# wuji3/visiondk

Measured on AMD Instinct MI355X. Metric: images/sec fwd+bwd+optimizer step (ViT-B/16, bs=256 per GPU), higher is better.
Workload: dtype fp16; 1 GPU; ViT-B/16 ICT, synthetic ImageNet-1k 224x224, random-init weights (reference re-init), per-GPU batch 256, CE label_smoothing 0.05, SGD 0.006/0.937/5e-4, clip 10, EMA on rank 0; global_batch=256, parallelism=dp1

## Files before the change

visiondk_amd/csrc/attention.hip:

```cpp
#include <hip/hip_runtime.h>
#include <stdlib.h>
#include "vdk_device.h"
#include "vdk_host.h"

#define A_HD 64
#define A_RP 72
#define A_FWD_KC 256
#define A_BWD_QC 256

__device__ __forceinline__ void a_stage_rows(bf16_t* dst, const bf16_t* __restrict__ src, long ld, int row0, int nvalid_total,
                                             int ntile) {
  for (int id = threadIdx.x; id < ntile * 8; id += 256) {
    int r = id >> 3, ch = id & 7;
    u32x4 v = {0u, 0u, 0u, 0u};
    if (row0 + r < nvalid_total) v = *(const u32x4*)(src + (long)(row0 + r) * ld + ch * 8);
    *(u32x4*)(dst + r * A_RP + ch * 8) = v;
  }
}
__device__ __forceinline__ void a_load_frags(s16x8 (&f)[4], const bf16_t* __restrict__ src, long ld, int row, int nvalid, int hi) {
#pragma unroll
  for (int ks = 0; ks < 4; ++ks) {
    s16x8 v = {0, 0, 0, 0, 0, 0, 0, 0};
    if (row < nvalid) v = *(const s16x8*)(src + (long)row * ld + ks * 16 + hi * 8);
    f[ks] = v;
// ... 182 lines not shown
    for (int r = 0; r < 16; ++r) { g0[r] = 0.f; g1[r] = 0.f; }
    for (int c = 0; c < nchunk; ++c) {
      const int key0 = c * A_FWD_KC;
      int nk = N - key0; if (nk > A_FWD_KC) nk = A_FWD_KC;
      const int nkp = (nk + 31) / 32 * 32;
      if (nchunk > 1 || rd == 0) {
        __syncthreads();
        a_stage_rows(Ks, kb, ld, key0, N, nkp);
        a_stage_rows(Vs, vb, ld, key0, N, nkp);
        __syncthreads();
      }
      if (active) {
        for (int kt = 0; kt < nkp / 32; ++kt) {
          f32x16 st = a_mma_rows(Ks + (kt * 32 + l31) * A_RP + hi * 8, qf);
          f32x16 dp = a_mma_rows(Vs + (kt * 32 + l31) * A_RP + hi * 8, dof);
          float ds[16];
#pragma unroll
          for (int r = 0; r < 16; ++r) {
            const int key = key0 + kt * 32 + (r & 3) + 8 * (r >> 2) + 4 * hi;
            const float p = (key < N && qrow < N) ? fast_exp2(fmaf(st[r], scale2, -mylse2)) : 0.f;
            ds[r] = p * (dp[r] - dsum);
          }
          s16x8 df[2];
          a_pack_b(ds, df);
#pragma unroll
          for (int s = 0; s < 2; ++s) {
            s16x8 a0 = a_load_T(Ks, kt * 32, 0, s, hi, lane);
            s16x8 a1 = a_load_T(Ks, kt * 32, 32, s, hi, lane);
            g0 = __builtin_amdgcn_mfma_f32_32x32x16_bf16(a0, df[s], g0, 0, 0, 0);
            g1 = __builtin_amdgcn_mfma_f32_32x32x16_bf16(a1, df[s], g1, 0, 0, 0);
          }
        }
      }
    }
    if (active && qrow < N) {
      bf16_t* drow = dq + ((long)b * N + qrow) * lddq + h * A_HD;
#pragma unroll
      for (int g = 0; g < 4; ++g) {
        const int d = 8 * g + 4 * hi;
        *(u32x2*)(drow + d) = (u32x2){pack_bf2(g0[4 * g] * scale, g0[4 * g + 1] * scale), pack_bf2(g0[4 * g + 2] * scale, g0[4 * g + 3] * scale)};
        *(u32x2*)(drow + 32 + d) = (u32x2){pack_bf2(g1[4 * g] * scale, g1[4 * g + 1] * scale), pack_bf2(g1[4 * g + 2] * scale, g1[4 * g + 3] * scale)};
      }
    }
  }
}

__global__ __launch_bounds__(256) void attn_bwd_dkv_kernel(const bf16_t* __restrict__ q, const bf16_t* __restrict__ k,
                                                           const bf16_t* __restrict__ v, long ld, const bf16_t* __restrict__ dout,
                                                           long ldo, const float* __restrict__ lse, const float* __restrict__ dvec,
                                                           bf16_t* __restrict__ dk, bf16_t* __restrict__ dv, long lddkv, int N, int H,
                                                           float scale) {
  __shared__ __attribute__((aligned(16))) bf16_t Qs[A_BWD_QC * A_RP];
  __shared__ __attribute__((aligned(16))) bf16_t Os[A_BWD_QC * A_RP];
  __shared__ __attribute__((aligned(16))) float lse_s[A_BWD_QC];
  __shared__ __attribute__((aligned(16))) float dv_s[A_BWD_QC];
  const int b = blockIdx.x / H, h = blockIdx.x % H;
  const int lane = threadIdx.x & 63, w = threadIdx.x >> 6, hi = lane >> 5, l31 = lane & 31;
  const bf16_t* qb = q + (long)b * N * ld + h * A_HD;
  const bf16_t* kb = k + (long)b * N * ld + h * A_HD;
  const bf16_t* vb = v + (long)b * N * ld + h * A_HD;
  const bf16_t* dob = dout + (long)b * N * ldo + h * A_HD;
  const float* lse_b = lse + ((long)b * H + h) * N;
  const float* dvec_b = dvec + ((long)b * H + h) * N;
  const int nkt = (N + 31) / 32, nchunk = (N + A_BWD_QC - 1) / A_BWD_QC, rounds = (nkt + 3) / 4;
  for (int rd = 0; rd < rounds; ++rd) {
    const int kt = rd * 4 + w;
    const bool active = kt < nkt;
    const int krow = kt * 32 + l31;
    s16x8 kf[4], vf[4];
    a_load_frags(kf, kb, ld, active ? krow : N, N, hi);
    a_load_frags(vf, vb, ld, active ? krow : N, N, hi);
    f32x16 gk0, gk1, gv0, gv1;
#pragma unroll
    for (int r = 0; r < 16; ++r) { gk0[r] = 0.f; gk1[r] = 0.f; gv0[r] = 0.f; gv1[r] = 0.f; }
    for (int c = 0; c < nchunk; ++c) {
      const int q0 = c * A_BWD_QC;
      int nq = N - q0; if (nq > A_BWD_QC) nq = A_BWD_QC;
      const int nqp = (nq + 31) / 32 * 32;
      if (nchunk > 1 || rd == 0) {
        __syncthreads();
        a_stage_rows(Qs, qb, ld, q0, N, nqp);
        a_stage_rows(Os, dob, ldo, q0, N, nqp);
        for (int i = threadIdx.x; i < nqp; i += 256) {
          lse_s[i] = (q0 + i < N) ? lse_b[q0 + i] * VDK_LOG2E : 0.f;
          dv_s[i] = (q0 + i < N) ? dvec_b[q0 + i] : 0.f;
        }
        __syncthreads();
      }
      if (active) {
        for (int qt = 0; qt < nqp / 32; ++qt) {
          f32x16 st = a_mma_rows(Qs + (qt * 32 + l31) * A_RP + hi * 8, kf);
          f32x16 dp = a_mma_rows(Os + (qt * 32 + l31) * A_RP + hi * 8, vf);
          float p[16], ds[16];
#pragma unroll
          for (int g = 0; g < 4; ++g) {
            f32x4 lv = *(const f32x4*)(lse_s + qt * 32 + 8 * g + 4 * hi);
            f32x4 dvv = *(const f32x4*)(dv_s + qt * 32 + 8 * g + 4 * hi);
#pragma unroll
            for (int e = 0; e < 4; ++e) {
              const int r = 4 * g + e;
              const int qq = q0 + qt * 32 + 8 * g + 4 * hi + e;
              const float pv = (qq < N && krow < N) ? fast_exp2(fmaf(st[r], scale * VDK_LOG2E, -lv[e])) : 0.f;
              p[r] = pv;
              ds[r] = pv * (dp[r] - dvv[e]);
            }
          }
          s16x8 pf[2], df[2];
          a_pack_b(p, pf);
          a_pack_b(ds, df);
#pragma unroll
          for (int s = 0; s < 2; ++s) {
            s16x8 ao0 = a_load_T(Os, qt * 32, 0, s, hi, lane);
            s16x8 ao1 = a_load_T(Os, qt * 32, 32, s, hi, lane);
            gv0 = __builtin_amdgcn_mfma_f32_32x32x16_bf16(ao0, pf[s], gv0, 0, 0, 0);
            gv1 = __builtin_amdgcn_mfma_f32_32x32x16_bf16(ao1, pf[s], gv1, 0, 0, 0);
            s16x8 aq0 = a_load_T(Qs, qt * 32, 0, s, hi, lane);
            s16x8 aq1 = a_load_T(Qs, qt * 32, 32, s, hi, lane);
            gk0 = __builtin_amdgcn_mfma_f32_32x32x16_bf16(aq0, df[s], gk0, 0, 0, 0);
            gk1 = __builtin_amdgcn_mfma_f32_32x32x16_bf16(aq1, df[s], gk1, 0, 0, 0);
          }
        }
      }
    }
    if (active && krow < N) {
      bf16_t* krow_p = dk + ((long)b * N + krow) * lddkv + h * A_HD;
      bf16_t* vrow_p = dv + ((long)b * N + krow) * lddkv + h * A_HD;
#pragma unroll
      for (int g = 0; g < 4; ++g) {
        const int d = 8 * g + 4 * hi;
        *(u32x2*)(krow_p + d) = (u32x2){pack_bf2(gk0[4 * g] * scale, gk0[4 * g + 1] * scale), pack_bf2(gk0[4 * g + 2] * scale, gk0[4 * g + 3] * scale)};
        *(u32x2*)(krow_p + 32 + d) = (u32x2){pack_bf2(gk1[4 * g] * scale, gk1[4 * g + 1] * scale), pack_bf2(gk1[4 * g + 2] * scale, gk1[4 * g + 3] * scale)};
        *(u32x2*)(vrow_p + d) = (u32x2){pack_bf2(gv0[4 * g], gv0[4 * g + 1]), pack_bf2(gv0[4 * g + 2], gv0[4 * g + 3])};
        *(u32x2*)(vrow_p + 32 + d) = (u32x2){pack_bf2(gv1[4 * g], gv1[4 * g + 1]), pack_bf2(gv1[4 * g + 2], gv1[4 * g + 3])};
      }
    }
  }
}

int vdk_attention_small_fwd(const void* qkv, int64_t ld, void* o, int64_t ldo, float* lse, int32_t B, int32_t N, int32_t H, float scale, int opf, void* stream);
int vdk_attention_small_bwd(const void* qkv, int64_t ld, const void* o, const void* dout, int64_t ldo, const float* lse, void* dqkv, int64_t ldd, float* dvec, int32_t B, int32_t N,
                            int32_t H, float scale, int opf, void* stream);
int vdk_attention_long_fwd(const void* qkv, int64_t ld, void* o, int64_t ldo, float* lse, int32_t B, int32_t N, int32_t H, float scale, int opf, void* stream);
int vdk_attention_long_bwd(const void* qkv, int64_t ld, const void* o, const void* dout, int64_t ldo, const float* lse, void* dqkv, int64_t ldd, float* dvec, int32_t B, int32_t N,
                           int32_t H, float scale, int opf, void* stream);
static thread_local int g_attn_legacy = -1;
static bool attn_legacy() {
  if (g_attn_legacy >= 0) return g_attn_legacy == 1;
  const char* e = getenv("VDK_ATTN_LEGACY");
  return e && e[0] == '1';
}

void vdk_attention_small_want_colsum(float*);
int vdk_attention_small_colsum_produced();
static int attn_long_min() {
  const char* e = getenv("VDK_ATTN_LONG_MIN");
  return e ? atoi(e) : 1 << 30;
}
static bool attn_long_bwd_off() {
  static const bool off = getenv("VDK_ATTN_LONG_BWD") && getenv("VDK_ATTN_LONG_BWD")[0] == '0';
  return off;
}

extern "C" {

int vdk_attention_fwd_dt(const void*, int64_t, void*, int64_t, float*, int32_t, int32_t, int32_t, int32_t, float, int32_t, void*);
int vdk_attention_bwd_dt(const void*, int64_t, const void*, const void*, int64_t, const float*, void*, int64_t, float*, int32_t, int32_t, int32_t, int32_t, float, int32_t, void*);
int vdk_attention_force_legacy(int32_t on) { g_attn_legacy = on < 0 ? -1 : (on ? 1 : 0); return VDK_OK; }

int vdk_attention_fwd(const void* qkv, int64_t ld, void* o, int64_t ldo, float* lse, int32_t B, int32_t N, int32_t H,
                      int32_t head_dim, float scale, void* stream) {
  return vdk_attention_fwd_dt(qkv, ld, o, ldo, lse, B, N, H, head_dim, scale, VDK_BF16, stream);
}
int vdk_attention_fwd_dt(const void* qkv, int64_t ld, void* o, int64_t ldo, float* lse, int32_t B, int32_t N, int32_t H,
                         int32_t head_dim, float scale, int32_t dtype, void* stream) {
  if (!qkv || !o || B <= 0 || N <= 0 || H <= 0 || (dtype != VDK_BF16 && dtype != VDK_F16)) return vdk_fail(VDK_EINVAL, "vdk_attention_fwd: bad argument");
  const int opf = dtype == VDK_F16 ? VDK_OPF_F16 : VDK_OPF_BF16;
  if (head_dim != A_HD) return vdk_fail(VDK_EUNSUPPORTED, "vdk_attention_fwd: head_dim must be 64");
  if ((ld & 7) || (ldo & 7)) return vdk_fail(VDK_EINVAL, "vdk_attention_fwd: ld % 8");
  if (N <= 256 && N < attn_long_min() && !attn_legacy()) {
    const int rc = vdk_attention_small_fwd(qkv, ld, o, ldo, lse, B, N, H, scale, opf, stream);
    if (rc != VDK_EUNSUPPORTED) return rc ? rc : vdk_check_launch("vdk_attention_fwd");
  }
  if ((N > 256 || N >= attn_long_min()) && !attn_legacy()) {
    const int rc = vdk_attention_long_fwd(qkv, ld, o, ldo, lse, B, N, H, scale, opf, stream);
    return rc ? rc : vdk_check_launch("vdk_attention_fwd");
  }
  if (opf) return vdk_fail(VDK_EUNSUPPORTED, "vdk_attention_fwd: the flash-style kernels of round 1 (vdk_attention_force_legacy) are bf16 only");
  const bf16_t* base = (const bf16_t*)qkv;
  const long D = (long)H * A_HD;
  int grid = B * H;
  int cap = 512;
  if (const char* e = getenv("VDK_ATTN_GRID")) { const int v = atoi(e); if (v > 0) cap = v; }
  if (N <= A_FWD_KC && grid > cap) grid = cap;
  hipLaunchKernelGGL(attn_fwd_kernel, dim3((unsigned)grid), dim3(256), 0, (hipStream_t)stream, base, base + D, base + 2 * D,
                     (long)ld, (bf16_t*)o, (long)ldo, lse, (int)N, (int)H, scale, (int)(B * H));
  return vdk_check_launch("vdk_attention_fwd");
}

int vdk_attention_bwd_cs(const void* qkv, int64_t ld, const void* o, const void* dout, int64_t ldo, const float* lse, void* dqkv, int64_t lddqkv, float* dvec, int32_t B, int32_t N,
                         int32_t H, int32_t head_dim, float scale, int32_t dtype, float* cspart, int32_t* produced, void* stream_) {
  vdk_attention_small_want_colsum(cspart);
  const int rc = vdk_attention_bwd_dt(qkv, ld, o, dout, ldo, lse, dqkv, lddqkv, dvec, B, N, H, head_dim, scale, dtype, stream_);
  if (produced) *produced = rc == VDK_OK ? vdk_attention_small_colsum_produced() : 0;
  vdk_attention_small_want_colsum(nullptr);
  return rc;
}
int vdk_attention_bwd(const void* qkv, int64_t ld, const void* o, const void* dout, int64_t ldo, const float* lse, void* dqkv,
                      int64_t lddqkv, float* dvec, int32_t B, int32_t N, int32_t H, int32_t head_dim, float scale, void* stream_) {
  return vdk_attention_bwd_dt(qkv, ld, o, dout, ldo, lse, dqkv, lddqkv, dvec, B, N, H, head_dim, scale, VDK_BF16, stream_);
}
int vdk_attention_bwd_dt(const void* qkv, int64_t ld, const void* o, const void* dout, int64_t ldo, const float* lse, void* dqkv,
                         int64_t lddqkv, float* dvec, int32_t B, int32_t N, int32_t H, int32_t head_dim, float scale, int32_t dtype, void* stream_) {
  hipStream_t stream = (hipStream_t)stream_;
  if (!qkv || !o || !dout || !lse || !dqkv || !dvec || B <= 0 || N <= 0 || H <= 0 || (dtype != VDK_BF16 && dtype != VDK_F16)) return vdk_fail(VDK_EINVAL, "vdk_attention_bwd: bad argument");
  const int opf = dtype == VDK_F16 ? VDK_OPF_F16 : VDK_OPF_BF16;
  if (head_dim != A_HD) return vdk_fail(VDK_EUNSUPPORTED, "vdk_attention_bwd: head_dim must be 64");
  if ((ld & 7) || (ldo & 7) || (lddqkv & 7)) return vdk_fail(VDK_EINVAL, "vdk_attention_bwd: ld % 8");
  if (N <= 224 && N < attn_long_min() && !attn_legacy()) {
    const int rc = vdk_attention_small_bwd(qkv, ld, o, dout, ldo, lse, dqkv, lddqkv, dvec, B, N, H, scale, opf, stream_);
    if (rc != VDK_EUNSUPPORTED) return rc ? rc : vdk_check_launch("vdk_attention_bwd");
  }
  if ((N > 224 || N >= attn_long_min()) && !attn_legacy() && !attn_long_bwd_off()) {
    const int rc = vdk_attention_long_bwd(qkv, ld, o, dout, ldo, lse, dqkv, lddqkv, dvec, B, N, H, scale, opf, stream_);
    return rc ? rc : vdk_check_launch("vdk_attention_bwd");
  }
  if (opf) return vdk_fail(VDK_EUNSUPPORTED, "vdk_attention_bwd: the flash-style kernels of round 1 are bf16 only");
  const bf16_t* base = (const bf16_t*)qkv;
  bf16_t* dbase = (bf16_t*)dqkv;
  const long D = (long)H * A_HD;
  hipLaunchKernelGGL(attn_bwd_dq_kernel, dim3((unsigned)(B * H)), dim3(256), 0, stream, base, base + D, base + 2 * D, (long)ld,
                     (const bf16_t*)o, (const bf16_t*)dout, (long)ldo, lse, dbase, (long)lddqkv, dvec, (int)N, (int)H, scale);
  hipLaunchKernelGGL(attn_bwd_dkv_kernel, dim3((unsigned)(B * H)), dim3(256), 0, stream, base, base + D, base + 2 * D, (long)ld,
                     (const bf16_t*)dout, (long)ldo, lse, (const float*)dvec, dbase + D, dbase + 2 * D, (long)lddqkv, (int)N, (int)H,
                     scale);
  return vdk_check_launch("vdk_attention_bwd");
}

}
```

visiondk_amd/csrc/attention_small.hip:

```cpp
#include <hip/hip_runtime.h>
#include <stdlib.h>
#include "vdk_device.h"
#include "vdk_host.h"

#include "vdk_attn_tile.h"


template <int NKT, int OF = 0>
__global__ __launch_bounds__(256, (NKT <= 7 ? 2 : 1)) void attn_s_fwd_kernel(const bf16_t* __restrict__ q, const bf16_t* __restrict__ k, const bf16_t* __restrict__ v, long ld,
                                                                              bf16_t* __restrict__ o, long ldo, float* __restrict__ lse, int N, int H, float scale, int nitems) {
  VDK_DYN_LDS(smem);
  const int tid = threadIdx.x, lane = tid & 63, hi = lane >> 5, l31 = lane & 31;
  const int w = __builtin_amdgcn_readfirstlane(tid >> 6);
  const int R8 = (N + 7) & ~7;
  unsigned char* const Qs = smem;
  unsigned char* const Ks = smem + R8 * AS_ROW;
  unsigned char* const Vs = smem + 2 * R8 * AS_ROW;
  for (int i = tid * 16; i < (32 * NKT - R8) * AS_ROW; i += 256 * 16) *(u32x4*)(Vs + R8 * AS_ROW + i) = (u32x4){0u, 0u, 0u, 0u};
  const int nqt = (N + 31) >> 5;
  const float scale2 = scale * VDK_LOG2E;
  const AsLane al = as_lane(lane);
  for (int item = blockIdx.x; item < nitems; item += gridDim.x) {
    const int b = item / H, h = item - b * H;
    const long off = (long)b * N * ld + h * 64;
    __syncthreads();
    as_dma_rows(Qs, q + off, ld, N, R8, w, 4, lane);
    as_dma_rows(Ks, k + off, ld, N, R8, w, 4, lane);
    as_dma_rows(Vs, v + off, ld, N, R8, w, 4, lane);
    __builtin_amdgcn_s_waitcnt(0x0F70);
    __syncthreads();
    for (int qt = w; qt < nqt; qt += 4) {
      const int qrow = qt * 32 + l31;
      s16x8 qf[4];
#pragma unroll
      for (int ks = 0; ks < 4; ++ks) qf[ks] = as_row_frag(Qs, qrow, ks, hi);
      f32x16 st[NKT];
#pragma unroll
      for (int kt = 0; kt < NKT; ++kt) {
        st[kt] = as_zero16();
#pragma unroll
        for (int ks = 0; ks < 4; ++ks) st[kt] = vdk_mfma32<OF>(as_row_frag_l(Ks + kt * 32 * AS_ROW, al, ks), qf[ks], st[kt]);
      }
      if (N & 31) {
#pragma unroll
        for (int r = 0; r < 16; ++r)
          if ((NKT - 1) * 32 + (r & 3) + 8 * (r >> 2) + 4 * hi >= N) st[NKT - 1][r] = -INFINITY;
      }
      float m = -INFINITY;
#pragma unroll
      for (int kt = 0; kt < NKT; ++kt)
#pragma unroll
        for (int r = 0; r < 16; ++r) m = fmaxf(m, st[kt][r]);
      m = fmaxf(m, __shfl_xor(m, 32));
      const float m2 = m * scale2;
      float l = 0.f;
#pragma unroll
      for (int kt = 0; kt < NKT; ++kt)
#pragma unroll
        for (int r = 0; r < 16; ++r) { const float p = fast_exp2(fmaf(st[kt][r], scale2, -m2)); st[kt][r] = p; l += p; }
      l += __shfl_xor(l, 32);
      const float inv = 1.0f / l;
      f32x16 o0 = as_zero16(), o1 = as_zero16();
#pragma unroll
      for (int kt = 0; kt < NKT; ++kt) {
        f32x16 pn;
#pragma unroll
        for (int r = 0; r < 16; ++r) pn[r] = st[kt][r] * inv;
        s16x8 pf[2];
        as_pack_b<OF>(pn, pf);
#pragma unroll
        for (int s = 0; s < 2; ++s) {
          o0 = vdk_mfma32<OF>(as_tr_frag_l(Vs + (kt * 32 + 16 * s) * AS_ROW, al, 0), pf[s], o0);
          o1 = vdk_mfma32<OF>(as_tr_frag_l(Vs + (kt * 32 + 16 * s) * AS_ROW, al, 1), pf[s], o1);
        }
      }
      as_store_tile<OF>(Qs + qt * 32 * AS_ROW, o0, o1, 1.0f, o + (long)b * N * ldo + h * 64, ldo, qt * 32, N, lane);
      if (lse && hi == 0 && qrow < N) lse[((long)b * H + h) * N + qrow] = (m2 + log2f(l)) * 0.6931471805599453f;
    }
  }
}

#define A5_PITCH 72
#ifndef A5_KVREG
#define A5_KVREG 1
#endif
#ifndef A5_SWAP
#define A5_SWAP 1
#endif
#ifndef A5_KP
#define A5_KP 1
#endif
#define A5_QPITCH 144
template <int NKT, int OF>
__global__ __launch_bounds__(512) void attn_s_bwd5_kernel(const bf16_t* __restrict__ q, const bf16_t* __restrict__ k, const bf16_t* __restrict__ v, long ld,
                                                          const bf16_t* __restrict__ o, const bf16_t* __restrict__ dout, long ldo, const float* __restrict__ lse,
                                                          bf16_t* __restrict__ dq, bf16_t* __restrict__ dk, bf16_t* __restrict__ dv, long ldd, int N, int H, float scale,
                                                          int nitems, int dbg ,
                                                          float* __restrict__ cspart ) {
  VDK_DYN_LDS(smem);
  const int tid = threadIdx.x, lane = tid & 63, hi = lane >> 5, l31 = lane & 31;
  const int w = __builtin_amdgcn_readfirstlane(tid >> 6);
  constexpr int NP = 32 * NKT;
  constexpr int NPC = (NP * 8 + 511) / 512;
  constexpr int DSB = NP * A5_PITCH;
  unsigned char* const QO = smem;
  unsigned char* const Kall = smem + 3 * 8192;
  unsigned char* const Kt = Kall + w * 4096;
  unsigned char* const Vt = Kall + NKT * 4096 + w * 4096;
  unsigned char* const Ds = Kall + 2 * NKT * 4096;
  unsigned char* const DQs = Ds + 2 * DSB;
  float* const lse2 = (float*)(DQs + NP * A5_QPITCH);
  float* const Dv = lse2 + NP;
  float* const CSs = Dv + NP;
  constexpr int nt = NKT;
  const float scale2 = scale * VDK_LOG2E;
  const bool ragged = (N & 31) != 0;
  const AsLane al = as_lane(lane);
  const bool keyw = w < nt;
  const int db = w >> 1, qb = w & 1;
  const int a16 = lane & 15, g4 = lane >> 4;
  const int trow = 8 * g4 + (a16 >> 2);
  const int ds_off = trow * A5_PITCH + qb * 32 + 8 * (a16 & 3);
  int kt_off[2];
#pragma unroll
  for (int h2 = 0; h2 < 2; ++h2) {
    const int r = trow + 4 * h2, byte = 32 * db + 8 * (a16 & 3);
    kt_off[h2] = r * AS_ROW + (((byte >> 4) ^ as_f(r)) << 4) + (byte & 8);
  }
  auto request_tile = [&](int j, int buf, long off, long offo, int lane_) {
    const int q0 = j * 32, part = w & 3;
    if (w < 4) as_dma_rows_raw(QO + buf * 8192, q + off + (long)q0 * ld, ld, N - q0, 32, part, 4, lane_);
    else as_dma_rows_raw(QO + buf * 8192 + 4096, dout + offo + (long)q0 * ldo, ldo, N - q0, 32, part, 4, lane_);
  };
  auto request_item = [&](long off, long offo, int lane_) {
    request_tile(0, 0, off, offo, lane_);
    if (nt > 1) request_tile(1, 1, off, offo, lane_);
    if (keyw) {
      as_dma_rows_raw(Kt, k + off + (long)(w * 32) * ld, ld, N - w * 32, 32, 0, 1, lane_);
      as_dma_rows_raw(Vt, v + off + (long)(w * 32) * ld, ld, N - w * 32, 32, 0, 1, lane_);
    }
  };
  u32x4 d_a[NPC], d_c[NPC];
  float lse_r = 0.f;
  auto d_issue = [&](long offo, long lrow, int tid_) {
#pragma unroll
    for (int p = 0; p < NPC; ++p) {
      const int id = tid_ + 512 * p, row = id >> 3, cp = id & 7;
      d_a[p] = (u32x4){0u, 0u, 0u, 0u}; d_c[p] = (u32x4){0u, 0u, 0u, 0u};
      if (row < N && !(dbg & 4)) { d_a[p] = *(const u32x4*)(dout + offo + (long)row * ldo + cp * 8); d_c[p] = *(const u32x4*)(o + offo + (long)row * ldo + cp * 8); }
    }
    lse_r = tid_ < N ? lse[lrow + tid_] : 0.f;
  };
  auto d_finish = [&]() {
#pragma unroll
    for (int p = 0; p < NPC; ++p) {
      const int id = tid + 512 * p, row = id >> 3, cp = id & 7;
      float d = 0.f;
#pragma unroll
      for (int e = 0; e < 4; ++e) { d = fmaf(op_lo<OF>(d_a[p][e]), op_lo<OF>(d_c[p][e]), d); d = fmaf(op_hi<OF>(d_a[p][e]), op_hi<OF>(d_c[p][e]), d); }
      d += __shfl_xor(d, 1); d += __shfl_xor(d, 2); d += __shfl_xor(d, 4);
      if (row < NP && cp == 0) Dv[row] = row < N ? d : 0.f;
    }
    if (tid < NP) lse2[tid] = lse_r * VDK_LOG2E;
  };
  int pb = -1, ph = 0;
  auto cs_flush = [&]() {
    if (tid < 192) {
      const int which = tid >> 6, col = tid & 63, nw = which == 0 ? 8 : nt;
      float t = 0.f;
      for (int ww = 0; ww < nw; ++ww) t += CSs[(which * 8 + ww) * 64 + col];
      cspart[(((long)pb * 3 + which) * H + ph) * 64 + col] = t;
    }
  };
  unsigned char* const St = Ds + w * 4096;
  if ((int)blockIdx.x < nitems) {
    const int b0 = blockIdx.x / H, h0 = blockIdx.x - b0 * H;
    request_item((long)b0 * N * ld + h0 * 64, (long)b0 * N * ldo + h0 * 64, lane);
    d_issue((long)b0 * N * ldo + h0 * 64, ((long)b0 * H + h0) * N, tid);
  }
  for (int item = blockIdx.x; item < nitems; item += gridDim.x) {
    const int b = item / H, h = item - b * H;
    const long off = (long)b * N * ld + h * 64, offo = (long)b * N * ldo + h * 64;
    d_finish();
    f32x16 gk0 = as_zero16(), gk1 = as_zero16(), gv0 = as_zero16(), gv1 = as_zero16();
    __builtin_amdgcn_s_waitcnt(0x0F70);
    __syncthreads();
    if (cspart && pb >= 0) cs_flush();
    s16x8 kfr[4], vfr[4];
#if A5_KVREG
    if (keyw) {
#pragma unroll
      for (int ks = 0; ks < 4; ++ks) { kfr[ks] = as_row_frag_l(Kt, al, ks); vfr[ks] = as_row_frag_l(Vt, al, ks); }
    }
#endif
    auto key_phase = [&](int j) {
      const int q0 = j * 32, buf = j % 3, dbuf = j & 1;
      const unsigned char* Qs = QO + buf * 8192;
      const unsigned char* Os = Qs + 4096;
      unsigned char* const Dsj = Ds + dbuf * DSB;
      if (j + 2 < nt) request_tile(j + 2, (j + 2) % 3, off, offo, lane);
      if (keyw && !(dbg & 1)) {
        f32x16 st = as_zero16(), dp = as_zero16();
        f32x16 pv, ds;
        s16x8 pf[2], df[2];
        const bool edge = ragged && j == nt - 1;
#if A5_KP == 0
#pragma unroll
        for (int ks = 0; ks < 4; ++ks) {
          st = vdk_mfma32<OF>(as_row_frag_l(Qs, al, ks), as_row_frag_l(Kt, al, ks), st);
          dp = vdk_mfma32<OF>(as_row_frag_l(Os, al, ks), as_row_frag_l(Vt, al, ks), dp);
        }
#pragma unroll
        for (int g = 0; g < 4; ++g) {
          const f32x4 lv = *(const f32x4*)(lse2 + q0 + 8 * g + 4 * hi);
          const f32x4 dd = *(const f32x4*)(Dv + q0 + 8 * g + 4 * hi);
#pragma unroll
          for (int e = 0; e < 4; ++e) {
            const int r = 4 * g + e;
            float p = fast_exp2(fmaf(st[r], scale2, -lv[e]));
            if (edge && q0 + 8 * g + 4 * hi + e >= N) p = 0.f;
            pv[r] = p;
            ds[r] = p * (dp[r] - dd[e]);
          }
        }
        as_pack_b<OF>(pv, pf);
        as_pack_b<OF>(ds, df);
#pragma unroll
        for (int s2 = 0; s2 < 2; ++s2) {
          gv0 = vdk_mfma32<OF>(as_tr_frag_l(Os + 16 * s2 * AS_ROW, al, 0), pf[s2], gv0);
          gv1 = vdk_mfma32<OF>(as_tr_frag_l(Os + 16 * s2 * AS_ROW, al, 1), pf[s2], gv1);
          gk0 = vdk_mfma32<OF>(as_tr_frag_l(Qs + 16 * s2 * AS_ROW, al, 0), df[s2], gk0);
          gk1 = vdk_mfma32<OF>(as_tr_frag_l(Qs + 16 * s2 * AS_ROW, al, 1), df[s2], gk1);
        }
#else
#define A5_SB() __builtin_amdgcn_sched_barrier(0)
#ifdef VDK_EMU
#define A5_PIN(x) ((void)0)
#else
#define A5_PIN(x) asm volatile("" : "+v"(x))
#endif
        s16x8 qf[4], of_[4], kf[4], vf[4];
#pragma unroll
        for (int ks = 0; ks < 4; ++ks) { qf[ks] = as_row_frag_l(Qs, al, ks); kf[ks] = A5_KVREG ? kfr[ks] : as_row_frag_l(Kt, al, ks); }
#pragma unroll
        for (int ks = 0; ks < 4; ++ks) st = vdk_mfma32<OF>(qf[ks], kf[ks], st);
#pragma unroll
        for (int ks = 0; ks < 4; ++ks) { of_[ks] = as_row_frag_l(Os, al, ks); vf[ks] = A5_KVREG ? vfr[ks] : as_row_frag_l(Vt, al, ks); }
        A5_SB();
#pragma unroll
        for (int g = 0; g < 4; ++g) {
          dp = vdk_mfma32<OF>(of_[g], vf[g], dp);
          const f32x4 lv = *(const f32x4*)(lse2 + q0 + 8 * g + 4 * hi);
#pragma unroll
          for (int e = 0; e < 4; ++e) pv[4 * g + e] = fast_exp2(fmaf(st[4 * g + e], scale2, -lv[e]));
          A5_SB();
        }
        if (edge) {
#pragma unroll
          for (int r = 0; r < 16; ++r)
            if (q0 + 8 * (r >> 2) + 4 * hi + (r & 3) >= N) pv[r] = 0.f;
        }
        as_pack_b<OF>(pv, pf);
        A5_SB();
#pragma unroll
        for (int s2 = 0; s2 < 2; ++s2)
#pragma unroll
          for (int dh = 0; dh < 2; ++dh) {
            const s16x8 tf = as_tr_frag_l(Os + 16 * s2 * AS_ROW, al, dh);
            if (dh == 0) gv0 = vdk_mfma32<OF>(tf, pf[s2], gv0); else gv1 = vdk_mfma32<OF>(tf, pf[s2], gv1);
            const int g = 2 * s2 + dh;
            const f32x4 dd = *(const f32x4*)(Dv + q0 + 8 * g + 4 * hi);
#pragma unroll
            for (int e = 0; e < 4; ++e) { ds[4 * g + e] = pv[4 * g + e] * (dp[4 * g + e] - dd[e]); A5_PIN(ds[4 * g + e]); }
            A5_SB();
          }
        as_pack_b<OF>(ds, df);
#pragma unroll
        for (int s2 = 0; s2 < 2; ++s2) {
          gk0 = vdk_mfma32<OF>(as_tr_frag_l(Qs + 16 * s2 * AS_ROW, al, 0), df[s2], gk0);
          gk1 = vdk_mfma32<OF>(as_tr_frag_l(Qs + 16 * s2 * AS_ROW, al, 1), df[s2], gk1);
        }
#undef A5_SB
#undef A5_PIN
#endif
        const bool kval = w * 32 + l31 < N;
        unsigned char* const drow = Dsj + (w * 32 + l31) * A5_PITCH + 8 * hi;
#pragma unroll
        for (int s2 = 0; s2 < 2; ++s2) {
          u32x4 u = *(const u32x4*)&df[s2];
          if (!kval) u = (u32x4){0u, 0u, 0u, 0u};
          *(u32x2*)(drow + 32 * s2) = (u32x2){u[0], u[1]};
          *(u32x2*)(drow + 32 * s2 + 16) = (u32x2){u[2], u[3]};
        }
      }
    };
    auto dq_phase = [&](int j) {
      const int q0 = j * 32, dbuf = j & 1;
      unsigned char* const Dsj = Ds + dbuf * DSB;
      f32x4 acc = {0.f, 0.f, 0.f, 0.f};
      if (!(dbg & 2))
#pragma unroll
      for (int t = 0; t < NKT; ++t) {
        const unsigned char* bp = Dsj + t * 32 * A5_PITCH + ds_off;
        const s16x4 lo = __builtin_amdgcn_ds_read_tr16_b64_v4i16(VDK_LDS_S16X4(bp));
        const s16x4 up = __builtin_amdgcn_ds_read_tr16_b64_v4i16(VDK_LDS_S16X4(bp + 4 * A5_PITCH));
        const s16x8 bfrag = {lo[0], lo[1], lo[2], lo[3], up[0], up[1], up[2], up[3]};
        const s16x4 klo = __builtin_amdgcn_ds_read_tr16_b64_v4i16(VDK_LDS_S16X4(Kall + t * 4096 + kt_off[0]));
        const s16x4 kup = __builtin_amdgcn_ds_read_tr16_b64_v4i16(VDK_LDS_S16X4(Kall + t * 4096 + kt_off[1]));
        acc = vdk_mfma16<OF>((s16x8){klo[0], klo[1], klo[2], klo[3], kup[0], kup[1], kup[2], kup[3]}, bfrag, acc);
      }
      *(u32x2*)(DQs + (q0 + 16 * qb + a16) * A5_QPITCH + 32 * db + 8 * g4) = (u32x2){pack_op2<OF>(acc[0] * scale, acc[1] * scale), pack_op2<OF>(acc[2] * scale, acc[3] * scale)};
    };
    key_phase(0);
#pragma unroll 1
    for (int j = 0; j < nt; ++j) {
      if (j + 2 < nt) __builtin_amdgcn_s_waitcnt(0x0F71); else __builtin_amdgcn_s_waitcnt(0x0F70);
      __syncthreads();
      const bool keyfirst = A5_SWAP && w < 4;
      if (keyfirst && j + 1 < nt) key_phase(j + 1);
      dq_phase(j);
      if (!keyfirst && j + 1 < nt) key_phase(j + 1);
    }
    __syncthreads();
    int ln = lane, td = tid;
#ifndef VDK_EMU
    asm volatile("" : "+v"(ln), "+v"(td));
#endif
    const int lane = ln, tid = td, l31 = ln & 31, hi = ln >> 5;
    if (item + (int)gridDim.x < nitems) {
      const int nb = (item + (int)gridDim.x) / H, nh = (item + (int)gridDim.x) - nb * H;
      request_item((long)nb * N * ld + nh * 64, (long)nb * N * ldo + nh * 64, lane);
      d_issue((long)nb * N * ldo + nh * 64, ((long)nb * H + nh) * N, tid);
    }
    if (dbg & 8) continue;
    if (!cspart) {
      if (keyw) {
        as_store_tile<OF>(St, gk0, gk1, scale, dk + (long)b * N * ldd + h * 64, ldd, w * 32, N, lane);
        as_store_tile<OF>(St, gv0, gv1, 1.0f, dv + (long)b * N * ldd + h * 64, ldd, w * 32, N, lane);
      }
#pragma unroll
      for (int p = 0; p < NPC; ++p) {
        const int id = tid + 512 * p, row = id >> 3, cp = id & 7;
        if (row < N) *(u32x4*)(dq + (long)b * N * ldd + h * 64 + (long)row * ldd + cp * 8) = *(const u32x4*)(DQs + row * A5_QPITCH + cp * 16);
      }
      continue;
    }
    auto cs_add = [&](float (&cs)[8], const u32x4& v) {
#pragma unroll
      for (int e = 0; e < 4; ++e) { cs[2 * e] += op_lo<OF>(v[e]); cs[2 * e + 1] += op_hi<OF>(v[e]); }
    };
    auto cs_put = [&](float (&cs)[8], int which) {
#pragma unroll
      for (int e = 0; e < 8; ++e) { float t = cs[e]; t += __shfl_xor(t, 8); t += __shfl_xor(t, 16); t += __shfl_xor(t, 32); cs[e] = t; }
      if (lane < 8) {
        float* dst = CSs + (which * 8 + w) * 64 + lane * 8;
        *(f32x4*)dst = (f32x4){cs[0], cs[1], cs[2], cs[3]}; *(f32x4*)(dst + 4) = (f32x4){cs[4], cs[5], cs[6], cs[7]};
      }
    };
    if (keyw) {
#pragma unroll
      for (int which = 1; which <= 2; ++which) {
        float cs[8] = {0.f, 0.f, 0.f, 0.f, 0.f, 0.f, 0.f, 0.f};
        bf16_t* const dst = (which == 1 ? dk : dv) + (long)b * N * ldd + h * 64;
        const f32x16& x0 = which == 1 ? gk0 : gv0; const f32x16& x1 = which == 1 ? gk1 : gv1;
        const float mul = which == 1 ? scale : 1.0f;
        const int row0 = w * 32;
        if (row0 + l31 < N) {
#pragma unroll
          for (int g = 0; g < 4; ++g) {
            const int ch = g ^ (l31 & 7), ch1 = (4 + g) ^ (l31 & 7);
            *(u32x2*)(St + l31 * AS_ROW + (ch << 4) + 8 * hi) = (u32x2){pack_op2<OF>(x0[4 * g] * mul, x0[4 * g + 1] * mul), pack_op2<OF>(x0[4 * g + 2] * mul, x0[4 * g + 3] * mul)};
            *(u32x2*)(St + l31 * AS_ROW + (ch1 << 4) + 8 * hi) = (u32x2){pack_op2<OF>(x1[4 * g] * mul, x1[4 * g + 1] * mul), pack_op2<OF>(x1[4 * g + 2] * mul, x1[4 * g + 3] * mul)};
          }
        }
        VDK_WAVE_LDS_SYNC();
#pragma unroll
        for (int p = 0; p < 4; ++p) {
          const int r = 8 * p + (lane >> 3), cp = lane & 7;
          if (row0 + r < N) {
            const u32x4 v = *(const u32x4*)(St + r * AS_ROW + ((cp ^ (r & 7)) << 4));
            *(u32x4*)(dst + (long)(row0 + r) * ldd + cp * 8) = v;
            cs_add(cs, v);
          }
        }
        VDK_WAVE_LDS_SYNC();
        cs_put(cs, which);
      }
    }
    {
      float cs[8] = {0.f, 0.f, 0.f, 0.f, 0.f, 0.f, 0.f, 0.f};
#pragma unroll
      for (int p = 0; p < NPC; ++p) {
        const int id = tid + 512 * p, row = id >> 3, cp = id & 7;
        if (row < N) {
          const u32x4 v = *(const u32x4*)(DQs + row * A5_QPITCH + cp * 16);
          *(u32x4*)(dq + (long)b * N * ldd + h * 64 + (long)row * ldd + cp * 8) = v;
          cs_add(cs, v);
        }
      }
      cs_put(cs, 0);
    }
    pb = b; ph = h;
  }
  if (cspart && pb >= 0) { __syncthreads(); cs_flush(); }
}

template <int NKT, int OF>
static int launch_fwd(const bf16_t* base, long D, long ld, bf16_t* o, long ldo, float* lse, int B, int N, int H, float scale, int grid, hipStream_t s) {
  const int R8 = (N + 7) & ~7;
  const size_t lds = (size_t)(2 * R8 + 32 * NKT) * AS_ROW;
  if (hipFuncSetAttribute((const void*)attn_s_fwd_kernel<NKT, OF>, hipFuncAttributeMaxDynamicSharedMemorySize, (int)lds) != hipSuccess)
    return vdk_fail(VDK_ELAUNCH, "vdk_attention_fwd: LDS attribute");
  hipLaunchKernelGGL((attn_s_fwd_kernel<NKT, OF>), dim3((unsigned)grid), dim3(256), lds, s, base, base + D, base + 2 * D, ld, o, ldo, lse, N, H, scale, B * H);
  return VDK_OK;
}
static thread_local float* t_cspart = nullptr;
static thread_local int t_cs_produced = 0;
void vdk_attention_small_want_colsum(float* cspart) { t_cspart = cspart; t_cs_produced = 0; }
int vdk_attention_small_colsum_produced() { return t_cs_produced; }
template <int NKT, int OF>
static int launch_bwd5(const bf16_t* base, long D, long ld, const bf16_t* o, const bf16_t* dout, long ldo, const float* lse, bf16_t* dbase, long ldd, int B, int N, int H,
                       float scale, int grid, hipStream_t s) {
  const size_t lds = 3 * 8192 + 2 * (size_t)NKT * 4096 + 2 * (size_t)(32 * NKT) * A5_PITCH + (size_t)(32 * NKT) * A5_QPITCH + (size_t)NKT * 32 * 8 + 3 * 8 * 64 * 4;
  float* const cspart = t_cspart;
  if (cspart) t_cs_produced = 1;
  const char* edbg = getenv("VDK_ATTN5_DBG");
  const int dbg = edbg ? atoi(edbg) : 0;
  if (hipFuncSetAttribute((const void*)attn_s_bwd5_kernel<NKT, OF>, hipFuncAttributeMaxDynamicSharedMemorySize, (int)lds) != hipSuccess)
    return vdk_fail(VDK_ELAUNCH, "vdk_attention_bwd: LDS attribute");
  hipLaunchKernelGGL((attn_s_bwd5_kernel<NKT, OF>), dim3((unsigned)grid), dim3(512), lds, s, base, base + D, base + 2 * D, ld, o, dout, ldo, lse, dbase, dbase + D, dbase + 2 * D,
                     ldd, N, H, scale, B * H, dbg, cspart);
  return VDK_OK;
}
static int grid_cap(int dflt) {
  if (const char* e = getenv("VDK_ATTN_GRID")) { const int v = atoi(e); if (v > 0) return v; }
  return dflt;
}

int vdk_attention_small_fwd(const void* qkv, int64_t ld, void* o, int64_t ldo, float* lse, int32_t B, int32_t N, int32_t H, float scale, int opf, void* stream) {
  const int nkt = (N + 31) / 32;
  if (nkt < 1 || nkt > 8) return VDK_EUNSUPPORTED;
  const bf16_t* base = (const bf16_t*)qkv;
  const long D = (long)H * 64;
  int grid = B * H;
  const int cap = grid_cap(512);
  if (grid > cap) grid = cap;
  hipStream_t s = (hipStream_t)stream;
  switch (nkt) {
#define FW(n) case n: return opf ? launch_fwd<n, VDK_OPF_F16>(base, D, ld, (bf16_t*)o, ldo, lse, B, N, H, scale, grid, s) : launch_fwd<n, 0>(base, D, ld, (bf16_t*)o, ldo, lse, B, N, H, scale, grid, s);
    FW(1) FW(2) FW(3) FW(4) FW(5) FW(6) FW(7)
    default: return opf ? launch_fwd<8, VDK_OPF_F16>(base, D, ld, (bf16_t*)o, ldo, lse, B, N, H, scale, grid, s) : launch_fwd<8, 0>(base, D, ld, (bf16_t*)o, ldo, lse, B, N, H, scale, grid, s);
#undef FW
  }
}

int vdk_attention_small_bwd(const void* qkv, int64_t ld, const void* o, const void* dout, int64_t ldo, const float* lse, void* dqkv, int64_t ldd, float* dvec, int32_t B, int32_t N,
                            int32_t H, float scale, int opf, void* stream) {
  const int nkt = (N + 31) / 32;
  if (nkt < 1 || nkt > 7) return VDK_EUNSUPPORTED;
  const bf16_t* base = (const bf16_t*)qkv;
  const long D = (long)H * 64;
  int grid = B * H;
  const int cap = grid_cap(256);
  if (grid > cap) grid = cap;
  hipStream_t s = (hipStream_t)stream;
  switch (nkt) {
#define B5(n) case n: return opf ? launch_bwd5<n, VDK_OPF_F16>(base, D, ld, (const bf16_t*)o, (const bf16_t*)dout, ldo, lse, (bf16_t*)dqkv, ldd, B, N, H, scale, grid, s) \
                                 : launch_bwd5<n, 0>(base, D, ld, (const bf16_t*)o, (const bf16_t*)dout, ldo, lse, (bf16_t*)dqkv, ldd, B, N, H, scale, grid, s);
    B5(1) B5(2) B5(3) B5(4) B5(5) B5(6)
    default: return opf ? launch_bwd5<7, VDK_OPF_F16>(base, D, ld, (const bf16_t*)o, (const bf16_t*)dout, ldo, lse, (bf16_t*)dqkv, ldd, B, N, H, scale, grid, s)
                        : launch_bwd5<7, 0>(base, D, ld, (const bf16_t*)o, (const bf16_t*)dout, ldo, lse, (bf16_t*)dqkv, ldd, B, N, H, scale, grid, s);
#undef B5
  }
}
```

visiondk_amd/csrc/gemm.hip:

```cpp
#include <hip/hip_runtime.h>
#ifndef VDK_EMU_NO_HIP_EXT
#include <hip/hip_ext.h>
#endif
#include <cstdlib>
#include "vdk_device.h"
#include "vdk_host.h"
#include "vdk_gemm.h"
#include "vdk_gemm_epilogue.h"

#define G_BM 128
#define G_BN 128
#define G_BK 64
#define G_PITCH 72
#define G_CP 132

__device__ __forceinline__ void g_load_tile(u32x4 (&r)[4], const bf16_t* __restrict__ base, long ld, int row0,
                                            int nrows, int k0, int kend) {
#pragma unroll
  for (int j = 0; j < 4; ++j) {
    int id = threadIdx.x + 256 * j;
    int row = id >> 3, ch = id & 7;
    int grow = row0 + row, k = k0 + ch * 8;
    u32x4 v = {0u, 0u, 0u, 0u};
    if (grow < nrows && k < kend) v = *(const u32x4*)(base + (long)grow * ld + k);
// ... 426 lines not shown
      if (cs_ >= te) break;
      if (ce_ == cs_) continue;
      if (ncontrib == 2 && pp == sk_pos) continue;
      const float* src = p.slabs + ((long)pp * 2 + (cs_ >= tb ? 0 : 1)) * WGF + w * 8192 + lane * 2;
#pragma unroll
      for (int i = 0; i < 4; ++i)
#pragma unroll
        for (int j = 0; j < 2; ++j)
#pragma unroll
          for (int g = 0; g < 8; ++g) {
            const unsigned long long v = VDK_AGENT_LD_U64(src + ((i * 2 + j) * 8 + g) * 128);
            acc[i][j][2 * g] += __uint_as_float((unsigned)v); acc[i][j][2 * g + 1] += __uint_as_float((unsigned)(v >> 32));
          }
    }
  } else if (SK) {
    if (tid == 0) {
      if (sk_st[2] < nwg / (int)gridDim.x) sk_st[2] += 1;
      else sk_st[0] += nk;
    }
  }

  float* slab = (float*)(smem + w * 16384);
  const int ncol = n0 + wc * 64 + (lane & 7) * 8;
  float bias8[8], ocs8[8];
#pragma unroll
  for (int e = 0; e < 8; ++e) { bias8[e] = 0.f; ocs8[e] = 0.f; }
  if ((E != E_GENERIC) && (E & E_BIAS) && ncol < p.N) {
    f32x4 b0v = *(const f32x4*)(p.bias + ncol), b1v = *(const f32x4*)(p.bias + ncol + 4);
#pragma unroll
    for (int e = 0; e < 4; ++e) { bias8[e] = b0v[e]; bias8[4 + e] = b1v[e]; }
  }
  float q8_unused = 0.f;
#pragma unroll
  for (int half = 0; half < 2; ++half) {
#pragma unroll
    for (int rt = 0; rt < 2; ++rt)
#pragma unroll
      for (int ct = 0; ct < 2; ++ct)
#pragma unroll
        for (int r = 0; r < 16; ++r)
          slab[(rt * 32 + (r & 3) + 8 * (r >> 2) + 4 * hi) * 64 + ct * 32 + l31] = acc[half * 2 + rt][ct][r];
    __builtin_amdgcn_wave_barrier();
    if (E != E_GENERIC) {
      h_epilogue_half<E>(p, slab, lane, (long)m0 + wr * 128 + half * 64, ncol, z, bias8, ocs8, q8_unused);
    } else {
#pragma unroll
      for (int pass = 0; pass < 8; ++pass) {
        const int row = pass * 8 + (lane >> 3), cc = (lane & 7) * 8;
        const long mi = (long)m0 + wr * 128 + half * 64 + row;
        const int n = n0 + wc * 64 + cc;
        if (mi < p.M && n < p.N) {
          float v[8];
          f32x4 x0 = *(const f32x4*)(slab + row * 64 + cc), x1 = *(const f32x4*)(slab + row * 64 + cc + 4);
#pragma unroll
          for (int e = 0; e < 4; ++e) { v[e] = x0[e]; v[4 + e] = x1[e]; }
          g_epilogue_store8(p, mi, n, v, z);
        }
      }
    }
    __builtin_amdgcn_wave_barrier();
  }
  if ((E != E_GENERIC) && (E & E_OCS)) {
#pragma unroll
    for (int e = 0; e < 8; ++e) {
      float v = ocs8[e];
      v += __shfl_xor(v, 8); v += __shfl_xor(v, 16); v += __shfl_xor(v, 32);
      ocs8[e] = v;
    }
    if (lane < 8 && ncol < p.N) {
      float* dst = p.ocs_part + ((long)tm * 2 + wr) * p.N + ncol;
      *(f32x4*)dst = (f32x4){ocs8[0], ocs8[1], ocs8[2], ocs8[3]};
      *(f32x4*)(dst + 4) = (f32x4){ocs8[4], ocs8[5], ocs8[6], ocs8[7]};
    }
  }
  if (!SK && p.dbg && tid == 0) {
    __builtin_amdgcn_s_waitcnt(0x0F70);
    unsigned long long* o = p.dbg + ((size_t)blockIdx.y * gridDim.x + blockIdx.x) * 4;
    o[0] = t_start; o[1] = t_landed; o[2] = t_main; o[3] = __builtin_readcyclecounter();
  }
  } while (SK);
#undef H_REG
#undef H_ISSUE_A
#undef H_ISSUE_B
#undef H_FRAG_A
#undef H_FRAG_B
}

template <int OF = 0>
__global__ __launch_bounds__(256) void splitk_reduce_kernel(const float* __restrict__ slabs, int S, long n4 ,
                                                            long mn, float alpha, float* __restrict__ outf,
                                                            bf16_t* __restrict__ outb) {
  long i = (long)blockIdx.x * 256 + threadIdx.x;
  if (i >= n4) return;
  f32x4 s = *(const f32x4*)(slabs + i * 4);
  for (int k = 1; k < S; ++k) {
    f32x4 t = *(const f32x4*)(slabs + (long)k * mn + i * 4);
    s += t;
  }
  s *= alpha;
  if (outf) *(f32x4*)(outf + i * 4) = s;
  if (outb) *(u32x2*)(outb + i * 4) = (u32x2){pack_op2<OF>(s[0], s[1]), pack_op2<OF>(s[2], s[3])};
}

template <int OF = 0>
__global__ __launch_bounds__(256) void transpose_bf16_kernel(const bf16_t* __restrict__ in, long ldi, int R, int Cc,
                                                             bf16_t* __restrict__ out, long ldo, int Rpad, int row_group,
                                                             float* __restrict__ colsum_partial) {
  __shared__ bf16_t tile[64][66];
  const int r0 = blockIdx.x * 64, c0 = blockIdx.y * 64;
  const int tid = threadIdx.x;
  for (int i = 0; i < 8; ++i) {
    int row = i * 8 + (tid >> 5), cw = (tid & 31) * 2;
    int gr = r0 + row, gc = c0 + cw;
    bf16_t v0 = 0, v1 = 0;
    if (gr < R) {
      const long sr = row_group > 0 ? (long)gr + gr / row_group + 1 : (long)gr;
      if (gc + 1 < Cc) { unsigned wv = *(const unsigned*)(in + sr * ldi + gc); v0 = (bf16_t)(wv & 0xffff); v1 = (bf16_t)(wv >> 16); }
      else if (gc < Cc) v0 = in[sr * ldi + gc];
    }
    tile[row][cw] = v0; tile[row][cw + 1] = v1;
  }
  __syncthreads();
  if (colsum_partial && tid < 64 && c0 + tid < Cc) {
    float sacc = 0.f;
    for (int r = 0; r < 64; ++r) sacc += op2f<OF>(tile[r][tid]);
    colsum_partial[(long)blockIdx.x * Cc + c0 + tid] = sacc;
  }
  for (int i = 0; i < 8; ++i) {
    int col = i * 8 + (tid >> 5), rw = (tid & 31) * 2;
    int gc = c0 + col, gr = r0 + rw;
    if (gc < Cc && gr < Rpad) {
      unsigned wv = (unsigned)tile[rw][col] | ((unsigned)tile[rw + 1][col] << 16);
      *(unsigned*)(out + (long)gc * ldo + gr) = wv;
    }
  }
}

#include <vector>
static thread_local std::vector<hipEvent_t> g_prof_ev;
static thread_local std::vector<double> g_prof_flops;
static thread_local double g_prof_bytes = 0.0;
static thread_local size_t g_prof_used = 0;
static thread_local bool g_prof_on = false;
static thread_local void* g_dbg_ptr = nullptr;
static thread_local int g_force_kernel = 0;
static thread_local int g_sk_grid = 0;
static thread_local int g_last_kernel = 0;
static bool w4_enabled_env() {
  static const bool on = !(getenv("VDK_GEMM_W4") && atoi(getenv("VDK_GEMM_W4")) == 0);
  return on;
}
static thread_local int t_tn_half = 0;
void vdk_gemm_tn_prefer_half(int on) { t_tn_half = on; }
static bool w4h_wanted(int E, bool trans, long M, long N, long K) {
  static const int mask = getenv("VDK_GEMM_W4H") ? atoi(getenv("VDK_GEMM_W4H")) : -1;
  if (g_force_kernel == 6) return true;
  if (g_force_kernel == 2 || g_force_kernel == 3 || g_force_kernel == 5 || !w4_enabled_env()) return false;
  if (mask >= 0) {
    if (trans) return (mask & 16) != 0;
    if (E == E_GENERIC) return false;
    if (E & E_GELU) return (mask & 1) != 0;
    if (E & E_DGELU) return (mask & 2) != 0;
    if (E & E_RES) return (mask & 4) != 0;
    return (mask & 8) != 0;
  }
  if (trans) return t_tn_half != 0;
  if (E == E_GENERIC) return false;
  const long tiles = ((M + 255) / 256) * ((N + 255) / 256);
  if (tiles < 128) return true;
  if ((E & E_DGELU) && (E & E_AUXD) && tiles > 256) return false;
  if (E & E_DGELU) return true;
  static const long gelu_k = getenv("VDK_GEMM_W4H_GELU_K") ? atol(getenv("VDK_GEMM_W4H_GELU_K")) : 768;
  if ((E & E_GELU) && gelu_k > 0 && K <= gelu_k) return true;
  if (E & E_GELU) return K <= 768 && (double)tiles / (double)((tiles + 255) / 256 * 256) < 0.8;
  if (E & E_RES) return K < 1536 && tiles <= 256;
  return K <= 1024 && tiles <= 3 * 256;
}
static long narrow_min_m() {
  static const long v = getenv("VDK_GEMM_NARROW_MIN_M") ? atol(getenv("VDK_GEMM_NARROW_MIN_M")) : 65536L;
  return v;
}
static bool w4_enabled() {
  return (w4_enabled_env() || g_force_kernel == 5) && g_force_kernel != 2 && g_force_kernel != 3 && g_force_kernel != 6;
}
#define SK_CNT_BYTES 65536
static int sk_grid() {
  if (g_sk_grid > 0) return g_sk_grid;
  static int cus = 0;
  if (cus == 0) {
    int dev = 0, n = 0;
    if (hipGetDevice(&dev) != hipSuccess || hipDeviceGetAttribute(&n, hipDeviceAttributeMultiprocessorCount, dev) != hipSuccess || n < 8) n = 256;
    cus = n & ~7;
  }
  return cus;
}

#define RC_MARGIN(x) do { int rc_ = (x); if (rc_) return rc_; } while (0)
extern "C" {

int vdk_gemm_a_colsum_rows(int32_t M, int32_t N, int32_t K) {
  const long tiles256 = (long)((M + 255) / 256) * ((N + 255) / 256);
  const bool big = g_force_kernel == 2 || g_force_kernel == 3 || g_force_kernel == 5 || g_force_kernel == 6 || ((g_force_kernel == 0 || g_force_kernel == 4) && (K % 64 == 0) && tiles256 >= 128 && M >= 256 && N >= 256);
  return (big && (K % 64 == 0) && (M % 256 == 0)) ? (M / 256) : 0;
}

int vdk_gemm_c_colsum_rows(int32_t M, int32_t N, int32_t K) {
  const long tiles256 = (long)((M + 255) / 256) * ((N + 255) / 256);
  const long tiles_h = w4_enabled_env() ? (long)((M + 255) / 256) * ((N + 127) / 128) : 0;
  const bool big = g_force_kernel == 2 || g_force_kernel == 3 || g_force_kernel == 5 || g_force_kernel == 6 || ((g_force_kernel == 0 || g_force_kernel == 4) && (K % 64 == 0) && (tiles256 >= 128 || tiles_h >= 128) && M >= 256 && N >= 256);
  return (big && (K % 64 == 0)) ? 2 * ((M + 255) / 256) : 0;
}

int vdk_gemm_force_kernel(int32_t which) { g_force_kernel = which; return VDK_OK; }
int vdk_gemm_last_kernel(void) { return g_last_kernel; }

int vdk_gemm_streamk_workspace_bytes(size_t* bytes) {
  if (!bytes) return vdk_fail(VDK_EINVAL, "vdk_gemm_streamk_workspace_bytes: null");
  *bytes = (size_t)SK_CNT_BYTES + (size_t)sk_grid() * 2 * 65536 * 4;
  return VDK_OK;
}
int vdk_gemm_streamk_grid(int32_t g) {
  if (g < 0 || (g & 7)) return vdk_fail(VDK_EINVAL, "vdk_gemm_streamk_grid: must be a multiple of 8");
  g_sk_grid = g;
  return VDK_OK;
}
int vdk_gemm_debug_stamps(void* device_u64_buffer) { g_dbg_ptr = device_u64_buffer; return VDK_OK; }

int vdk_prof_begin(int32_t max_launches) {
  if (max_launches < 0) return vdk_fail(VDK_EINVAL, "vdk_prof_begin: bad argument");
  while (g_prof_ev.size() < (size_t)max_launches * 2) {
    hipEvent_t e;
    if (hipEventCreate(&e) != hipSuccess) return vdk_fail(VDK_ELAUNCH, "vdk_prof_begin: hipEventCreate failed");
    g_prof_ev.push_back(e);
  }
  g_prof_flops.clear();
  g_prof_bytes = 0.0;
  g_prof_used = 0;
  g_prof_on = true;
  return VDK_OK;
}
int vdk_prof_pause(int32_t paused) { g_prof_on = !paused && !g_prof_ev.empty(); return VDK_OK; }
int vdk_prof_end(double* total_ms, int64_t* launches, double* total_flops) {
  g_prof_on = false;
  double ms = 0.0, fl = 0.0;
  for (size_t i = 0; i + 1 < g_prof_used; i += 2) {
    if (hipEventSynchronize(g_prof_ev[i + 1]) != hipSuccess) return vdk_fail(VDK_ELAUNCH, "vdk_prof_end: event sync failed");
    float t = 0.f;
    if (hipEventElapsedTime(&t, g_prof_ev[i], g_prof_ev[i + 1]) != hipSuccess) return vdk_fail(VDK_ELAUNCH, "vdk_prof_end: elapsed failed");
    ms += t; fl += g_prof_flops[i / 2];
  }
  if (total_ms) *total_ms = ms;
  if (launches) *launches = (int64_t)(g_prof_used / 2);
  if (total_flops) *total_flops = fl;
  return VDK_OK;
}

int vdk_prof_bytes(double* total_bytes) {
  if (!total_bytes) return vdk_fail(VDK_EINVAL, "vdk_prof_bytes: null");
  *total_bytes = g_prof_bytes;
  return VDK_OK;
}

int vdk_gemm_splitk_workspace_bytes(int32_t M, int32_t N, int32_t splitk, size_t* bytes) {
  if (!bytes || M <= 0 || N <= 0 || splitk < 1) return vdk_fail(VDK_EINVAL, "vdk_gemm_splitk_workspace_bytes: bad argument");
  *bytes = splitk > 1 ? (size_t)splitk * M * N * 4 : 0;
  return VDK_OK;
}

int vdk_gemm_bf16_nt(const GemmDesc* d, void* ws, size_t ws_bytes, void* stream_) {
  hipStream_t stream = (hipStream_t)stream_;
  if (!d || !d->A || !d->B || !d->C) return vdk_fail(VDK_EINVAL, "vdk_gemm_bf16_nt: null pointer");
  if (d->M <= 0 || d->N <= 0 || d->K <= 0) return vdk_fail(VDK_EINVAL, "vdk_gemm_bf16_nt: empty problem");
  if ((d->K & 7) || (d->N & 7) || (!d->conv && (d->lda & 7)) || (d->ldb & 7) || (d->ldc & 7))
    return vdk_fail(VDK_EINVAL, "vdk_gemm_bf16_nt: K, N, lda, ldb, ldc must be multiples of 8");
  if (d->ab_dtype == VDK_F16 && !d->conv && d->splitk <= 1 && d->splitk != -1 && d->row_group == 0 && !d->a_colsum && !d->c_colsum && d->a_row_group == 0) {
    double lim = 2147483648.0 - 65536.0;
    if (const char* e = getenv("VDK_GEMM_ROWBLOCK_LIMIT")) { const double v = atof(e); if (v > 0) lim = v; }
    double rowb = (double)d->ldc * (d->c_dtype == VDK_F32 ? 4.0 : 2.0);
    if (d->aux && (double)d->ldaux * 2.0 > rowb) rowb = (double)d->ldaux * 2.0;
    if (d->residual && (double)d->ldr * 4.0 > rowb) rowb = (double)d->ldr * 4.0;
    if (!d->trans && (double)d->lda * 2.0 > rowb) rowb = (double)d->lda * 2.0;
    if (((double)d->M + 256.0) * rowb >= lim) {
      long mb = (long)(lim / rowb) - 256;
      mb = mb / 256 * 256;
      if (mb >= 256) {
        for (long m0 = 0; m0 < d->M; m0 += mb) {
          GemmDesc sub = *d;
          sub.M = (int32_t)((d->M - m0) < mb ? (d->M - m0) : mb);
          sub.A = d->trans ? (const void*)((const bf16_t*)d->A + m0) : (const void*)((const bf16_t*)d->A + m0 * d->lda);
          sub.C = d->c_dtype == VDK_F32 ? (void*)((float*)d->C + m0 * d->ldc) : (void*)((bf16_t*)d->C + m0 * d->ldc);
          if (d->residual) sub.residual = d->residual + m0 * d->ldr;
          if (d->aux) sub.aux = (void*)((bf16_t*)d->aux + m0 * d->ldaux);
          if (d->row_scale) { if (m0 % d->rows_per_scale) return vdk_fail(VDK_EUNSUPPORTED, "vdk_gemm_bf16_nt: row blocks do not align with rows_per_scale"); sub.row_scale = d->row_scale + m0 / d->rows_per_scale; }
          const int rc = vdk_gemm_bf16_nt(&sub, ws, ws_bytes, stream_);
          if (rc) return rc;
        }
        return VDK_OK;
      }
    }
  }
  if (d->conv) {
    const VdkConvGeom* c = d->conv;
    if (c->Cin <= 0 || (c->Cin & 7) || c->KH <= 0 || c->KW <= 0 || c->stride <= 0 || c->pad < 0 || c->OH <= 0 || c->OW <= 0 || c->H <= 0 || c->W <= 0)
      return vdk_fail(VDK_EINVAL, "vdk_gemm_bf16_nt: bad convolution geometry (Cin % 8 == 0)");
    if (!d->trans && (d->K != c->KH * c->KW * c->Cin || (d->M % (c->OH * c->OW))))
      return vdk_fail(VDK_EINVAL, "vdk_gemm_bf16_nt: bad convolution geometry (K == KH*KW*Cin, M == B*OH*OW)");
    if (d->trans && (c->transposed || d->N != c->KH * c->KW * c->Cin || c->rows <= 0 || c->rows >= (1 << 24) || (c->rows % (c->OH * c->OW)) || d->K < c->rows || (d->K % 128) ||
                     d->K - c->rows >= 128 || d->a_row_group != 0))
      return vdk_fail(VDK_EINVAL, "vdk_gemm_bf16_nt: bad weight-gradient geometry (N == KH*KW*Cin, rows == B*OH*OW < 2^24, K == rows rounded up to 128)");
  }
  if (d->ab_dtype != VDK_BF16 && d->ab_dtype != VDK_F16) return vdk_fail(VDK_EINVAL, "vdk_gemm_bf16_nt: ab_dtype must be VDK_BF16 or VDK_F16");
  const int opf = d->ab_dtype == VDK_F16 ? VDK_OPF_F16 : VDK_OPF_BF16;
  if (d->c_dtype != VDK_F32 && d->c_dtype != (opf ? VDK_F16 : VDK_BF16)) return vdk_fail(VDK_EINVAL, "vdk_gemm_bf16_nt: bad c_dtype (VDK_F32, or the operand format)");
  if (opf && (d->a_colsum || d->splitk == -1))
    return vdk_fail(VDK_EUNSUPPORTED, "vdk_gemm_bf16_nt: fp16 operands are served by the four-wave and the 128x128 kernels (no a_colsum, no stream-K)");
  if (d->act < VDK_ACT_NONE || d->act > VDK_ACT_MUL_AUX) return vdk_fail(VDK_EINVAL, "vdk_gemm_bf16_nt: bad act");
  if (((d->act == VDK_ACT_DGELU || d->act == VDK_ACT_GELU_SAVE_GRAD || d->act == VDK_ACT_MUL_AUX) && !d->aux) || (d->aux && (d->ldaux & 7)))
    return vdk_fail(VDK_EINVAL, "vdk_gemm_bf16_nt: bad aux");
  int splitk = d->splitk < 1 ? 1 : d->splitk;
  GemmParams p = {};
  p.A = (const bf16_t*)d->A; p.B = (const bf16_t*)d->B; p.C = d->C;
  p.lda = d->lda; p.ldb = d->ldb; p.ldc = d->ldc;
  p.M = d->M; p.N = d->N; p.K = d->K;
  p.opf = opf;
  p.c_dtype = d->c_dtype == VDK_F32 ? VDK_F32 : VDK_BF16; p.bias = (const float*)d->bias; p.residual = (const float*)d->residual; p.ldr = d->ldr;
  p.act = d->act; p.aux = (bf16_t*)d->aux; p.ldaux = d->ldaux; p.alpha = d->alpha; p.row_group = d->row_group < 0 ? -d->row_group : d->row_group; p.row_shift = d->row_group > 0 ? 1 : 0; p.a_row_group = d->a_row_group;
  p.splitk = splitk; p.slabs = nullptr; p.sk_cnt = nullptr; p.dbg = (unsigned long long*)g_dbg_ptr;
  p.colsum_part = nullptr; p.ocs_part = nullptr;
  p.cscale = d->col_scale;
  p.rscale = d->row_scale; p.rps = d->rows_per_scale;
  if (d->row_scale && (d->rows_per_scale <= 0 || d->c_dtype != VDK_F32 || !d->bias || !d->residual || d->act != VDK_ACT_NONE || d->splitk > 1 || d->trans || d->row_group != 0))
    return vdk_fail(VDK_EUNSUPPORTED, "vdk_gemm_bf16_nt: row_scale goes with rows_per_scale > 0, an fp32 output, a bias, a residual, act NONE and neither split-K, TN nor a row remap");
  if (d->col_scale && (d->c_dtype != VDK_F32 || !d->bias || d->act != VDK_ACT_NONE || d->splitk > 1 || d->trans || d->row_group != 0 || (d->N & 7)))
    return vdk_fail(VDK_EUNSUPPORTED, "vdk_gemm_bf16_nt: col_scale goes with an fp32 output, a bias, act NONE, N % 8 == 0 and neither split-K, TN nor a row remap");
  p.conv_on = d->conv != nullptr;
  if (d->conv) {
    const VdkConvGeom* c = d->conv;
    p.cCin = c->Cin; p.cH = c->H; p.cW = c->W; p.cOH = c->OH; p.cOW = c->OW; p.cKH = c->KH; p.cKW = c->KW; p.cstride = c->stride; p.cpad = c->pad; p.ctrans = c->transposed;
    p.crows = c->rows;
  }
  int kps = d->K;
  if (splitk > 1) {
    if (d->bias || d->residual || d->act != VDK_ACT_NONE || d->row_group != 0) return vdk_fail(VDK_EINVAL, "vdk_gemm_bf16_nt: split-K excludes fused epilogues");
    if (d->ldc != d->N) return vdk_fail(VDK_EINVAL, "vdk_gemm_bf16_nt: split-K needs ldc == N");
    const int kq = (d->K % 128 == 0) ? 128 : G_BK;
    kps = ((d->K + splitk - 1) / splitk + kq - 1) / kq * kq;
    splitk = (d->K + kps - 1) / kps;
    p.splitk = splitk;
    if (splitk > 1) {
      size_t need = (size_t)splitk * d->M * d->N * 4;
      if (!ws || ws_bytes < need) return vdk_fail(VDK_EWORKSPACE, "vdk_gemm_bf16_nt: split-K workspace too small");
      p.slabs = (float*)ws;
    }
  }
  p.k_per_split = kps;
  const int ntn = (d->N + G_BN - 1) / G_BN, ntm = (d->M + G_BM - 1) / G_BM;
  const bool prof = g_prof_on && g_prof_used + 2 <= g_prof_ev.size();
  const long tiles256 = (long)((d->M + 255) / 256) * ((d->N + 255) / 256) * splitk;
  const long tiles_h = (!d->trans && splitk == 1 && !d->a_colsum && w4_enabled_env()) ? (long)((d->M + 255) / 256) * ((d->N + 127) / 128) : 0;
  const bool narrow = !d->conv && !d->trans && g_force_kernel == 0 && w4_enabled_env() && (d->K % 64 == 0) && (kps % 64 == 0) && d->N >= 128 && d->N < 256 && d->M >= narrow_min_m() &&
                      !d->a_colsum && !d->c_colsum && splitk == 1 && vdk_gemm_w4h_serves(p, false);
  const bool big = !d->conv && (narrow || g_force_kernel == 2 || g_force_kernel == 3 || g_force_kernel == 5 || g_force_kernel == 6 || ((g_force_kernel == 0 || g_force_kernel == 4) && (d->K % 64 == 0) && (kps % 64 == 0) && (tiles256 >= 128 || tiles_h >= 128) && d->M >= 256 && d->N >= 256));
  int E = E_GENERIC;
  {
    const bool bias = d->bias != nullptr, res = d->residual != nullptr, f32 = p.c_dtype == VDK_F32, rg = d->row_group != 0;
    const bool plain_alpha = d->alpha == 1.0f;
    if (splitk > 1) E = E_SPLITK;
    else if (plain_alpha && !rg && !res && d->act == VDK_ACT_NONE && !f32) E = bias ? E_BIAS : 0;
    else if (plain_alpha && !rg && !res && d->act == VDK_ACT_GELU && !f32 && bias && d->aux) E = E_BIAS | E_GELU;
    else if (plain_alpha && !rg && !res && d->act == VDK_ACT_DGELU && !f32 && !bias) E = E_DGELU;
    else if (plain_alpha && !rg && !res && d->act == VDK_ACT_GELU_SAVE_GRAD && !f32 && bias) E = E_BIAS | E_GELU | E_AUXD;
    else if (plain_alpha && !rg && !res && d->act == VDK_ACT_MUL_AUX && !f32 && !bias) E = E_DGELU | E_AUXD;
    else if (plain_alpha && !rg && res && d->act == VDK_ACT_NONE && f32 && bias) E = E_BIAS | E_RES | E_F32;
    else if (plain_alpha && rg && res && d->act == VDK_ACT_NONE && f32 && bias) E = E_BIAS | E_RES | E_F32 | E_ROWGRP;
    else if (plain_alpha && !rg && !res && d->act == VDK_ACT_NONE && f32 && !bias) E = E_F32;
    else if (plain_alpha && !rg && !res && d->act == VDK_ACT_NONE && f32 && bias) E = E_BIAS | E_F32;
  }
  dim3 grid256((unsigned)(((d->M + 255) / 256) * ((d->N + 255) / 256)), (unsigned)splitk);
  bool sk = false;
  if (d->splitk == -1 && !d->trans && !d->a_colsum && big && ws && g_force_kernel != 4) {
    const long T = (long)grid256.x, G = sk_grid();
    const long rounds = (T + G - 1) / G;
    static const bool optin = getenv("VDK_GEMM_STREAMK") && atoi(getenv("VDK_GEMM_STREAMK")) > 0;
    const bool worth = optin && T >= G && (double)T / (double)(rounds * G) < 0.94;
    if ((worth || g_force_kernel == 3) && T <= SK_CNT_BYTES / 4 && T * (d->K / 64) >= G && ws_bytes >= (size_t)SK_CNT_BYTES + (size_t)G * 2 * 65536 * 4) {
      sk = true;
      p.sk_cnt = (int*)ws; p.slabs = (float*)((char*)ws + SK_CNT_BYTES);
      grid256 = dim3((unsigned)G, 1u);
    }
  }
#define VDK_GEMM_LAUNCH(KERN, GRID, BLOCK)                                                                                                   \
  do {                                                                                                                                       \
    if (prof) hipExtLaunchKernelGGL(KERN, GRID, BLOCK, 0, stream, g_prof_ev[g_prof_used], g_prof_ev[g_prof_used + 1], 0, p);                 \
    else hipLaunchKernelGGL(KERN, GRID, BLOCK, 0, stream, p);                                                                                \
  } while (0)
#define LAUNCH256X(TNF, EE, CSF)                                                                                         \
  do {                                                                                                                   \
    if (opf) {                    \
      void* e0_ = prof ? (void*)g_prof_ev[g_prof_used] : nullptr; void* e1_ = prof ? (void*)g_prof_ev[g_prof_used + 1] : nullptr;                \
      const bool hfirst_ = narrow || w4h_wanted(EE, TNF, p.M, p.N, p.K) || !(w4_enabled() && vdk_gemm_w4_serves(p, TNF));                         \
      if (hfirst_ && vdk_gemm_w4h_serves(p, TNF) && vdk_gemm_w4h_launch_f16(p, TNF, EE, grid256.y, stream, e0_, e1_)) { g_last_kernel = 6; break; }   \
      if (vdk_gemm_w4_serves(p, TNF) && vdk_gemm_w4_launch_f16(p, TNF, EE, grid256.x, grid256.y, stream, e0_, e1_)) { g_last_kernel = 5; break; }     \
      if (vdk_gemm_w4h_serves(p, TNF) && vdk_gemm_w4h_launch_f16(p, TNF, EE, grid256.y, stream, e0_, e1_)) { g_last_kernel = 6; break; }          \
      fp16_unserved = true; break;                                                                                        \
    }                                                                                                                    \
    if (!sk && !(CSF) && (narrow || w4h_wanted(EE, TNF, p.M, p.N, p.K)) && vdk_gemm_w4h_serves(p, TNF) &&                                           \
        vdk_gemm_w4h_launch(p, TNF, EE, grid256.y, stream, prof ? (void*)g_prof_ev[g_prof_used] : nullptr,               \
                            prof ? (void*)g_prof_ev[g_prof_used + 1] : nullptr)) { g_last_kernel = 6; break; }           \
    if (!sk && !(CSF) && w4_enabled() && vdk_gemm_w4_serves(p, TNF) &&                                                   \
        vdk_gemm_w4_launch(p, TNF, EE, grid256.x, grid256.y, stream, prof ? (void*)g_prof_ev[g_prof_used] : nullptr,     \
                           prof ? (void*)g_prof_ev[g_prof_used + 1] : nullptr)) { g_last_kernel = 5; break; }            \
    g_last_kernel = sk ? 3 : 2;                                                                                          \
    if (sk) VDK_GEMM_LAUNCH((gemm256_bf16_kernel<TNF, EE, !TNF, CSF>), grid256, dim3(512));                               \
    else VDK_GEMM_LAUNCH((gemm256_bf16_kernel<TNF, EE, false, CSF>), grid256, dim3(512));                                 \
  } while (0)
#define LAUNCH256(TNF, EE) LAUNCH256X(TNF, EE, false)
#define LAUNCH256CS(EE)                                                                                                  \
  do {                                                                                                                   \
    if (p.colsum_part) VDK_GEMM_LAUNCH((gemm256_bf16_kernel<false, EE, false, true>), grid256, dim3(512));                \
    else LAUNCH256X(false, EE, false);                                                                                   \
  } while (0)
  bool fp16_unserved = false;
  if (d->trans && d->conv) {
    if ((kps % 128) || (d->M & 7) || d->M < 8 || !vdk_gemm_w4_serves(p, true)) return vdk_fail(VDK_EUNSUPPORTED, "vdk_gemm_bf16_nt: this implicit weight gradient is outside the four-wave TN kernel's range");
    void* e0_ = prof ? (void*)g_prof_ev[g_prof_used] : nullptr; void* e1_ = prof ? (void*)g_prof_ev[g_prof_used + 1] : nullptr;
    const int ew_ = E == E_SPLITK ? E_SPLITK : (E == E_F32 ? E_F32 : E_GENERIC);
    if (!(opf ? vdk_gemm_w4_launch_f16(p, true, ew_, grid256.x, grid256.y, stream, e0_, e1_) : vdk_gemm_w4_launch(p, true, ew_, grid256.x, grid256.y, stream, e0_, e1_)))
      return vdk_fail(VDK_EUNSUPPORTED, "vdk_gemm_bf16_nt: implicit weight gradient: no kernel");
    g_last_kernel = 5;
  } else if (d->trans) {
    if ((d->K % 64) || (kps % 64) || (d->M & 7) || d->M < 8 || d->N < 8)
      return vdk_fail(VDK_EUNSUPPORTED, "vdk_gemm_bf16_nt: trans=1 needs K and the split size to be multiples of 64 and M % 8 == 0");
    switch (E) {
      case E_SPLITK: LAUNCH256(true, E_SPLITK); break;
      case E_F32: LAUNCH256(true, E_F32); break;
      case 0: LAUNCH256(true, 0); break;
      default: LAUNCH256(true, E_GENERIC); break;
    }
  } else if (big && (d->K % 64 == 0) && (kps % 64 == 0)) {
    if (d->a_colsum) {
      if (d->M % 256) return vdk_fail(VDK_EUNSUPPORTED, "vdk_gemm_bf16_nt: a_colsum needs M % 256 == 0");
      p.colsum_part = d->a_colsum;
      if (E != 0 && E != E_DGELU && E != E_F32) E = E_GENERIC;
    }
    if (d->c_colsum) {
      if ((E != E_DGELU && E != (E_DGELU | E_AUXD) && E != 0) || d->a_colsum) return vdk_fail(VDK_EUNSUPPORTED, "vdk_gemm_bf16_nt: c_colsum goes with a plain or dGELU bf16 epilogue and without a_colsum");
      p.ocs_part = d->c_colsum;
      E |= E_OCS;
    }
    switch (E) {
      case E_OCS: LAUNCH256(false, E_OCS); break;
      case E_DGELU | E_OCS: LAUNCH256(false, E_DGELU | E_OCS); break;
      case 0: LAUNCH256CS(0); break;
      case E_BIAS: LAUNCH256(false, E_BIAS); break;
      case E_BIAS | E_GELU: LAUNCH256(false, E_BIAS | E_GELU); break;
      case E_DGELU: LAUNCH256CS(E_DGELU); break;
      case E_BIAS | E_GELU | E_AUXD: LAUNCH256(false, E_BIAS | E_GELU | E_AUXD); break;
      case E_DGELU | E_AUXD: LAUNCH256(false, E_DGELU | E_AUXD); break;
      case E_DGELU | E_OCS | E_AUXD: LAUNCH256(false, E_DGELU | E_OCS | E_AUXD); break;
      case E_BIAS | E_RES | E_F32: LAUNCH256(false, E_BIAS | E_RES | E_F32); break;
      case E_BIAS | E_F32: LAUNCH256(false, E_BIAS | E_F32); break;
      case E_BIAS | E_RES | E_F32 | E_ROWGRP: LAUNCH256(false, E_BIAS | E_RES | E_F32 | E_ROWGRP); break;
      case E_SPLITK: LAUNCH256(false, E_SPLITK); break;
      case E_F32: LAUNCH256CS(E_F32); break;
      default: LAUNCH256CS(E_GENERIC); break;
    }
  }
#undef LAUNCH256CS
#undef LAUNCH256X
#undef LAUNCH256
  else if (d->a_colsum || d->c_colsum)
    return vdk_fail(VDK_EUNSUPPORTED, "vdk_gemm_bf16_nt: a_colsum / c_colsum are by-products of the 256x256 NT kernel only (see vdk_gemm_a_colsum_rows)");
  else if (d->conv) {
    g_last_kernel = 1;
    if (opf) VDK_GEMM_LAUNCH((gemm_bf16_nt_kernel<true, VDK_OPF_F16>), dim3((unsigned)(ntn * ntm), (unsigned)splitk), dim3(256));
    else VDK_GEMM_LAUNCH(gemm_bf16_nt_kernel<true>, dim3((unsigned)(ntn * ntm), (unsigned)splitk), dim3(256));
  } else {
    g_last_kernel = 1;
    if (opf) VDK_GEMM_LAUNCH((gemm_bf16_nt_kernel<false, VDK_OPF_F16>), dim3((unsigned)(ntn * ntm), (unsigned)splitk), dim3(256));
    else VDK_GEMM_LAUNCH(gemm_bf16_nt_kernel<false>, dim3((unsigned)(ntn * ntm), (unsigned)splitk), dim3(256));
  }
  if (fp16_unserved) {
    if (d->trans) return vdk_fail(VDK_EUNSUPPORTED, "vdk_gemm_bf16_nt: this fp16 TN problem is outside the four-wave kernels' range");
    g_last_kernel = 1;
    VDK_GEMM_LAUNCH((gemm_bf16_nt_kernel<false, VDK_OPF_F16>), dim3((unsigned)(ntn * ntm), (unsigned)splitk), dim3(256));
  }
  if (prof) {
    g_prof_flops.push_back(2.0 * d->M * d->N * d->K);
    {
      const double mn = (double)d->M * d->N;
      double b = ((double)d->M * d->K + (double)d->N * d->K) * 2.0 + mn * (p.c_dtype == VDK_F32 ? 4.0 : 2.0);
      if (d->residual) b += mn * 4.0;
      if (d->aux) b += mn * 2.0;
      if (d->bias) b += d->N * 4.0;
      if (d->splitk > 1) b += 2.0 * d->splitk * mn * 4.0;
      g_prof_bytes += b;
    }
    g_prof_used += 2;
  }
  if (splitk > 1) {
    long mn = (long)d->M * d->N, n4 = mn / 4;
    if (opf) hipLaunchKernelGGL(splitk_reduce_kernel<VDK_OPF_F16>, dim3((unsigned)((n4 + 255) / 256)), dim3(256), 0, stream, (const float*)p.slabs, splitk, n4, mn, d->alpha,
                                p.c_dtype == VDK_F32 ? (float*)d->C : (float*)nullptr, p.c_dtype == VDK_BF16 ? (bf16_t*)d->C : (bf16_t*)nullptr);
    else
    hipLaunchKernelGGL(splitk_reduce_kernel<0>, dim3((unsigned)((n4 + 255) / 256)), dim3(256), 0, stream,
                       (const float*)p.slabs, splitk, n4, mn, d->alpha,
                       p.c_dtype == VDK_F32 ? (float*)d->C : (float*)nullptr,
                       p.c_dtype == VDK_BF16 ? (bf16_t*)d->C : (bf16_t*)nullptr);
  }
  return vdk_check_launch("vdk_gemm_bf16_nt");
}

int vdk_margin_cos_pass(const VdkMarginHead* h, int32_t pass, const void* fbt, int64_t ld_f, const void* wb, int64_t ld_w, int32_t B, int32_t Bp, int32_t C, int32_t Cp, int32_t K,
                        const int64_t* labels, const float* gt, float* stats, float* tlogit, const float* rowstat, float label_smoothing, float grad_scale, void* dcos,
                        int64_t lddc, void* stream_) {
  hipStream_t stream = (hipStream_t)stream_;
  if (!h || !fbt || !wb || !labels || B <= 0 || Bp < B || C <= 0 || Cp < C || (pass != 1 && pass != 2)) return vdk_fail(VDK_EINVAL, "vdk_margin_cos_pass: bad argument");
  if ((pass == 1 && (!stats || !tlogit)) || (pass == 2 && (!rowstat || !dcos))) return vdk_fail(VDK_EINVAL, "vdk_margin_cos_pass: missing buffer for this pass");
  if ((K % 64) || (Bp & 7) || (Cp & 7) || (ld_f & 7) || (ld_w & 7) || (pass == 2 && (lddc & 7)) || Bp < 8 || Cp < 256)
    return VDK_EUNSUPPORTED;
  GemmParams p = {};
  p.A = (const bf16_t*)fbt; p.B = (const bf16_t*)wb; p.C = dcos; p.lda = ld_f; p.ldb = ld_w; p.ldc = lddc; p.M = Bp; p.N = Cp; p.K = K; p.c_dtype = VDK_BF16;
  p.alpha = 1.0f; p.splitk = 1; p.k_per_split = K;
  RC_MARGIN(fill_params(h, &p.me.P));
  p.me.labels = (const long long*)labels; p.me.gt = gt; p.me.stats = stats; p.me.nslice = (Cp + 63) / 64; p.me.tlogit = tlogit; p.me.rowstat = rowstat;
  p.me.smoothing = label_smoothing; p.me.gscale = grad_scale; p.me.epsc = label_smoothing / (float)C; p.me.B = B; p.me.C = C;
  const dim3 grid((unsigned)(((Bp + 255) / 256) * ((Cp + 255) / 256)), 1u);
  g_last_kernel = 2;
  if (w4_enabled() && vdk_gemm_w4_serves(p, true) && vdk_gemm_w4_launch(p, true, pass == 1 ? E_MSTAT : E_MGRAD, grid.x, 1u, stream, nullptr, nullptr)) g_last_kernel = 5;
  else if (pass == 1) hipLaunchKernelGGL((gemm256_bf16_kernel<true, E_MSTAT, false, false>), grid, dim3(512), 0, stream, p);
  else hipLaunchKernelGGL((gemm256_bf16_kernel<true, E_MGRAD, false, false>), grid, dim3(512), 0, stream, p);
  return vdk_check_launch("vdk_margin_cos_pass");
}

int vdk_transpose_bf16(const void* in, int64_t ldi, int32_t R, int32_t Cc, void* out, int64_t ldo, int32_t Rpad,
                       int32_t in_row_group, float* colsum_partial, void* stream) {
  return vdk_transpose_16(in, ldi, R, Cc, out, ldo, Rpad, in_row_group, colsum_partial, VDK_OPF_BF16, stream);
}

}

int vdk_transpose_16(const void* in, int64_t ldi, int32_t R, int32_t Cc, void* out, int64_t ldo, int32_t Rpad, int32_t in_row_group, float* colsum_partial, int opf,
                     void* stream) {
  if (!in || !out || R < 0 || Cc <= 0 || Rpad < R || (Rpad & 1) || ldo < Rpad || (ldi & 1) || (ldo & 1))
    return vdk_fail(VDK_EINVAL, "vdk_transpose_bf16: bad argument");
  if (Rpad == 0) return VDK_OK;
  const dim3 grid((unsigned)((Rpad + 63) / 64), (unsigned)((Cc + 63) / 64));
  if (opf) hipLaunchKernelGGL(transpose_bf16_kernel<VDK_OPF_F16>, grid, dim3(256), 0, (hipStream_t)stream, (const bf16_t*)in, (long)ldi, (int)R, (int)Cc, (bf16_t*)out,
                              (long)ldo, (int)Rpad, (int)in_row_group, colsum_partial);
  else hipLaunchKernelGGL(transpose_bf16_kernel<0>, grid, dim3(256), 0, (hipStream_t)stream, (const bf16_t*)in, (long)ldi, (int)R, (int)Cc, (bf16_t*)out, (long)ldo,
                          (int)Rpad, (int)in_row_group, colsum_partial);
  return vdk_check_launch("vdk_transpose_bf16");
}
```

visiondk_amd/csrc/gemm_w4.hip:

```cpp
#include <hip/hip_runtime.h>
#ifndef VDK_EMU_NO_HIP_EXT
#include <hip/hip_ext.h>
#endif
#include "vdk_device.h"
#include "vdk_host.h"
#include <atomic>
#include <string.h>
#include <stdlib.h>
#include "vdk_gemm.h"
#include "vdk_gemm_epilogue.h"

#ifndef VDK_W4_OF
#define VDK_W4_OF 0
#endif
#if VDK_W4_OF == 0
#define W4_SYM(name) name
#else
#define W4_SYM(name) name##_f16
#endif

#define W4_REGION 16384
#define W4_TILEBUF 65536
#define W4_STAGE 131072
#define W4_SMEM 163840
// ... 72 lines not shown
  d.ldb = ldb;
  d.conv = 0;
  if (!TN) {
    d.rs = w4_make_rsrc(base, (unsigned)extent * ldb);
    const unsigned i = (unsigned)lane >> 3, cp = (unsigned)lane & 7u;
    d.voff0 = i * ldb + ((cp ^ (i >> 1)) << 4);
    d.voff1 = i * ldb + ((cp ^ (4u + (i >> 1))) << 4);
    d.wave_off = (unsigned)__builtin_amdgcn_readfirstlane((int)(((unsigned)(w >> 1) * blk + (unsigned)(w & 1) * 32u) * ldb));
    d.sub_stride = 64u * ldb;
    d.piece_stride = 8u * ldb;
    d.kbeg = (unsigned)kbeg * 2u;
    d.kstep = 128u;
  } else {
    d.rs = w4_make_rsrc(base, (unsigned)K * ldb);
    const unsigned kr = (unsigned)lane >> 4, cp = (unsigned)lane & 15u, c = cp ^ (4u * (kr & 3u));
    d.voff0 = d.voff1 = kr * ldb + ((c >> 3) * blk + (c & 7u) * 8u) * 2u;
    d.wave_off = (unsigned)__builtin_amdgcn_readfirstlane((int)((unsigned)w * 16u * ldb));
    d.sub_stride = 128u;
    d.piece_stride = 4u * ldb;
    d.kbeg = (unsigned)kbeg * ldb;
    d.kstep = 64u * ldb;
  }
}
template <bool TN>
__device__ __forceinline__ unsigned w4_tile_base(const W4Dma& d, int origin) {
  return (TN ? (unsigned)origin * 2u : (unsigned)origin * d.ldb) + d.wave_off;
}
__device__ __forceinline__ void w4_piece(const W4Dma& d, unsigned char* dst, int sub, int j, unsigned so0) {
  if (d.conv) {
    const unsigned rr = so0 + d.w16 + 4u * (unsigned)j + d.kr;
    unsigned voff = W4_OOB;
    if (rr < (unsigned)d.crows && d.cok[sub]) {
      int b, rem, oy, ox;
      w4_divmod(rr, d.cHW, d.inv_hw, b, rem);
      w4_divmod((unsigned)rem, d.cOW, d.inv_w, oy, ox);
      const int iy = oy * d.cstride + d.cy[sub], ix = ox * d.cstride + d.cx[sub];
      if ((unsigned)iy < (unsigned)d.cH && (unsigned)ix < (unsigned)d.cW) voff = (unsigned)(((b * d.cH + iy) * d.cW + ix) * d.cCin) * 2u + d.cib[sub];
    }
    W4_DMA16(d.rs, voff, dst, 0u);
    return;
  }
  const unsigned so = so0 + (unsigned)sub * d.sub_stride + (unsigned)j * d.piece_stride;
  W4_DMA16(d.rs, (j & 1) ? d.voff1 : d.voff0, dst, so);
}
__device__ __forceinline__ void w4_region(const W4Dma& d, unsigned char* region, int sub, int w, unsigned so0) {
#pragma unroll
  for (int j = 0; j < 4; ++j) w4_piece(d, region + (4 * w + j) * 1024, sub, j, so0);
}

template <bool TN>
struct W4Frag { unsigned a[TN ? 2 : 4], b[TN ? 2 : 4]; };

template <bool TN>
__device__ __forceinline__ void w4_frag_init(W4Frag<TN>& f, int wr, int wc, int lane) {
  const unsigned l31 = lane & 31, hi = lane >> 5;
  if (!TN) {
#pragma unroll
    for (int ks = 0; ks < 4; ++ks) {
      const unsigned ch = ((unsigned)(ks * 2) + hi) ^ ((l31 >> 1) & 7u);
      f.a[ks] = ((unsigned)wr * 64u + l31) * 128u + ch * 16u;
      f.b[ks] = ((unsigned)wc * 64u + l31) * 128u + ch * 16u;
    }
  } else {
    const unsigned s = lane & 15, chalf = (lane >> 4) & 1, t1 = hi * 8u + (s >> 2);
#pragma unroll
    for (int rt = 0; rt < 2; ++rt) {
      const unsigned ca = (unsigned)wr * 64u + (unsigned)rt * 32u + 16u * chalf + 4u * (s & 3u);
      const unsigned cb = (unsigned)wc * 64u + (unsigned)rt * 32u + 16u * chalf + 4u * (s & 3u);
      f.a[rt] = t1 * 256u + (((ca >> 3) ^ (4u * (t1 & 3u))) * 16u) + ((ca >> 2) & 1u) * 8u;
      f.b[rt] = t1 * 256u + (((cb >> 3) ^ (4u * (t1 & 3u))) * 16u) + ((cb >> 2) & 1u) * 8u;
    }
  }
}
template <bool TN>
__device__ __forceinline__ s16x8 w4_frag(const unsigned char* region, const unsigned* off, int rt, int ks) {
  if (!TN) {
    return *(const s16x8*)(region + off[ks] + rt * 4096);
  } else {
    const unsigned char* p1 = region + off[rt] + ks * 4096;
    s16x4 lo = __builtin_amdgcn_ds_read_tr16_b64_v4i16(VDK_LDS_S16X4(p1));
    s16x4 up = __builtin_amdgcn_ds_read_tr16_b64_v4i16(VDK_LDS_S16X4(p1 + 1024));
    s16x8 r = {lo[0], lo[1], lo[2], lo[3], up[0], up[1], up[2], up[3]};
    return r;
  }
}

template <bool TN, bool RD, bool FIRST, int OF>
__device__ __forceinline__ void w4_phase(f32x16 (&c00), f32x16 (&c01), f32x16 (&c10), f32x16 (&c11), const s16x8 (&X)[2][4], const s16x8 (&Y)[2][4],
                                         const unsigned char* rd_region, const unsigned* rd_off, s16x8 (&RDST)[2][4],
                                         const W4Dma& dma, unsigned char* is_region, int is_sub, unsigned so0, int w) {
  const f32x16 zero = {0.f, 0.f, 0.f, 0.f, 0.f, 0.f, 0.f, 0.f, 0.f, 0.f, 0.f, 0.f, 0.f, 0.f, 0.f, 0.f};
#pragma unroll
  for (int ks = 0; ks < 4; ++ks) {
    c00 = vdk_mfma32<OF>(Y[0][ks], X[0][ks], (FIRST && ks == 0) ? zero : c00);
    if (RD) RDST[0][ks] = w4_frag<TN>(rd_region, rd_off, 0, ks);
    c01 = vdk_mfma32<OF>(Y[1][ks], X[0][ks], (FIRST && ks == 0) ? zero : c01);
    if (RD) RDST[1][ks] = w4_frag<TN>(rd_region, rd_off, 1, ks);
    c10 = vdk_mfma32<OF>(Y[0][ks], X[1][ks], (FIRST && ks == 0) ? zero : c10);
    w4_piece(dma, is_region + (4 * w + ks) * 1024, is_sub, ks, so0);
    c11 = vdk_mfma32<OF>(Y[1][ks], X[1][ks], (FIRST && ks == 0) ? zero : c11);
  }
#ifndef VDK_EMU
#pragma unroll
  for (int ks = 0; ks < 4; ++ks) {
    __builtin_amdgcn_sched_group_barrier(0x008, 1, 0);
    if (RD) __builtin_amdgcn_sched_group_barrier(0x100, TN ? 2 : 1, 0);
    __builtin_amdgcn_sched_group_barrier(0x008, 1, 0);
    if (RD) __builtin_amdgcn_sched_group_barrier(0x100, TN ? 2 : 1, 0);
    __builtin_amdgcn_sched_group_barrier(0x008, 1, 0);
    __builtin_amdgcn_sched_group_barrier(0x004, 2, 0);
    __builtin_amdgcn_sched_group_barrier(0x008, 1, 0);
  }
#endif
}

template <int V>
__device__ __forceinline__ void w4_phase_end() {
  __builtin_amdgcn_sched_barrier(0);
  if constexpr (V >= 0) W4_WAIT_VM(V);
  W4_WAIT_LGKM0();
}
template <bool TN, int CUR, int VM, bool FIRST, bool NEXT, int OF>
__device__ __forceinline__ void w4_ktile(unsigned char* smem, const W4Frag<TN>& F, const W4Dma& da, const W4Dma& db, unsigned soa, unsigned sob, int w, f32x16 (&acc)[4][4],
                                         s16x8 (&A0)[2][4], s16x8 (&A1)[2][4], s16x8 (&B0)[2][4], s16x8 (&B1)[2][4], s16x8 (&B0N)[2][4]) {
  unsigned char* const buf = smem + CUR * W4_TILEBUF;
  unsigned char* const nbuf = smem + (CUR ^ 1) * W4_TILEBUF;
  W4_BAR();
  w4_phase<TN, true, FIRST, OF>(acc[0][0], acc[0][1], acc[1][0], acc[1][1], A0, B0, buf + W4_RB1, F.b, B1, da, buf + W4_RA0, 0, soa, w);
  w4_phase_end<VM>();
  W4_BAR();
  w4_phase<TN, true, FIRST, OF>(acc[0][2], acc[0][3], acc[1][2], acc[1][3], A0, B1, buf + W4_RA1, F.a, A1, db, buf + W4_RB0, 0, sob, w);
  w4_phase_end<VM>();
  W4_BAR();
  w4_phase<TN, NEXT, FIRST, OF>(acc[2][2], acc[2][3], acc[3][2], acc[3][3], A1, B1, nbuf + W4_RA0, F.a, A0, db, buf + W4_RB1, 1, sob, w);
  w4_phase_end<VM>();
  W4_BAR();
  w4_phase<TN, NEXT, FIRST, OF>(acc[2][0], acc[2][1], acc[3][0], acc[3][1], A1, B0, nbuf + W4_RB0, F.b, B0N, da, buf + W4_RA1, 1, soa, w);
  w4_phase_end<VM>();
}

#ifdef VDK_EMU
#define W4_EPI_SYNC() VDK_WAVE_LDS_SYNC()
#else
#define W4_EPI_SYNC() do { __builtin_amdgcn_s_waitcnt(0xC07F); VDK_WAVE_LDS_SYNC(); } while (0)
#endif
template <int E, int NCT, int DEEP, int OF>
__device__ __forceinline__ void w4_epilogue(const GemmParams& p, unsigned char* stage, f32x16 (&acc)[4][NCT], int lane, int wr, int wc, int m0, int n0, int z, int tm, unsigned long long (&ts)[5],
                                            const u32x4* auxpre = nullptr ) {
  constexpr int NCH = NCT * 4;
  constexpr int RPP = 64 / NCH;
  constexpr int NPS = 32 / RPP;
  constexpr int ROWB = NCT * 64;
  constexpr int EB = E & ~E_AUXD;
  constexpr bool FAST = (E == 0 || E == E_BIAS || EB == (E_BIAS | E_GELU) || EB == E_DGELU || EB == (E_DGELU | E_OCS) || E == E_OCS);
  const int l31 = lane & 31, hi = lane >> 5;
  const int mrow0 = m0 + wr * 128, ncol0 = n0 + wc * (NCT * 32);
  const int swz_w = NCT == 4 ? (l31 & 15) : ((l31 >> 1) & 7);
  if constexpr (FAST) {
    const int rrow = lane / NCH, rc = lane % NCH;
    const int ncol = ncol0 + rc * 8;
    const bool nok = ncol < p.N;
    float bias[NCT][4][4];
    if (E & E_BIAS) {
#pragma unroll
      for (int ct = 0; ct < NCT; ++ct)
#pragma unroll
        for (int g = 0; g < 4; ++g) {
          const int n = ncol0 + ct * 32 + 8 * g + 4 * hi;
          f32x4 b = {0.f, 0.f, 0.f, 0.f};
          if (n < p.N) b = *(const f32x4*)(p.bias + n);
#pragma unroll
          for (int e = 0; e < 4; ++e) bias[ct][g][e] = b[e];
        }
    }
    float ocs[8];
#pragma unroll
    for (int e = 0; e < 8; ++e) ocs[e] = 0.f;
    unsigned char* const wbase = stage + l31 * ROWB + hi * 8;
    const unsigned lane_out = nok ? (unsigned)rrow * (unsigned)p.ldc * 2u + (unsigned)ncol * 2u : W4_OOB;
    const unsigned lane_aux = nok ? (unsigned)rrow * (unsigned)p.ldaux * 2u + (unsigned)ncol * 2u : W4_OOB;
    const __amdgpu_buffer_rsrc_t rs_out = __builtin_amdgcn_make_buffer_rsrc(p.C, 0, (int)((unsigned)p.M * (unsigned)p.ldc * 2u), 0x00020000);
    const __amdgpu_buffer_rsrc_t rs_aux = __builtin_amdgcn_make_buffer_rsrc((E & (E_GELU | E_DGELU)) ? (void*)p.aux : p.C, 0,
                                                                            (int)((unsigned)p.M * (unsigned)((E & (E_GELU | E_DGELU)) ? p.ldaux : p.ldc) * 2u), 0x00020000);
    auto rows_out = [&](const __amdgpu_buffer_rsrc_t& rs, unsigned lane_off, unsigned ldbytes, int rt, bool with_ocs) {
      W4_EPI_SYNC();
      const unsigned srow = (unsigned)(mrow0 + rt * 32) * ldbytes;
      u32x4 d[NPS];
#pragma unroll
      for (int ps = 0; ps < NPS; ++ps) {
        const int row = ps * RPP + rrow;
        d[ps] = *(const u32x4*)(stage + row * ROWB + ((rc ^ (NCT == 4 ? (row & 15) : ((row >> 1) & 7))) << 4));
      }
      if (with_ocs) {
#pragma unroll
        for (int ps = 0; ps < NPS; ++ps)
#pragma unroll
          for (int e = 0; e < 4; ++e) { ocs[2 * e] += op_lo<OF>(d[ps][e]); ocs[2 * e + 1] += op_hi<OF>(d[ps][e]); }
      }
#pragma unroll
      for (int ps = 0; ps < NPS; ++ps)
        __builtin_amdgcn_raw_buffer_store_b128(d[ps], rs, lane_off + (srow + (unsigned)(ps * RPP) * ldbytes), 0, W4_STORE_POLICY);
      W4_EPI_SYNC();
    };
    if constexpr (DEEP >= 0) W4_WAIT_VM(DEEP);
    if (p.dbg) ts[0] = __builtin_readcyclecounter();
    u32x4 auxrows[NPS];
    auto aux_request = [&](int rt_) {
      const unsigned srow = (unsigned)(mrow0 + rt_ * 32) * (unsigned)p.ldaux * 2u;
#pragma unroll
      for (int ps = 0; ps < NPS; ++ps)
        auxrows[ps] = __builtin_amdgcn_raw_buffer_load_b128(rs_aux, lane_aux, srow + (unsigned)(ps * RPP) * (unsigned)p.ldaux * 2u, 0);
    };
    if (E & E_DGELU) {
      if (auxpre) {
#pragma unroll
        for (int ps = 0; ps < NPS; ++ps) auxrows[ps] = auxpre[ps];
      } else aux_request(0);
    }
#pragma unroll
    for (int rt = 0; rt < 4; ++rt) {
      if (p.dbg && rt > 0) ts[rt] = __builtin_readcyclecounter();
#ifndef VDK_EMU
      __builtin_amdgcn_sched_barrier(0);
#endif
      u32x2 held[NCT][4];
      if (E & E_DGELU) {
        if (!W4_EPI_AHEAD && rt > 0) aux_request(rt);
#pragma unroll
        for (int ps = 0; ps < NPS; ++ps) {
          const int row = ps * RPP + rrow;
          *(u32x4*)(stage + row * ROWB + ((rc ^ (NCT == 4 ? (row & 15) : ((row >> 1) & 7))) << 4)) = auxrows[ps];
        }
        if (W4_EPI_AHEAD && rt < 3) aux_request(rt + 1);
        W4_EPI_SYNC();
      }
#pragma unroll
      for (int ct = 0; ct < NCT; ++ct)
#pragma unroll
        for (int g = 0; g < 4; ++g) {
          unsigned char* const wp = wbase + (((ct * 4 + g) ^ swz_w) << 4);
          float v[4];
          if (E & E_DGELU) {
            const u32x2 u = *(const u32x2*)wp;
            if (E & E_AUXD) {
              v[0] = acc[rt][ct][4 * g + 0] * h_lo(u[0]); v[1] = acc[rt][ct][4 * g + 1] * h_hi(u[0]);
              v[2] = acc[rt][ct][4 * g + 2] * h_lo(u[1]); v[3] = acc[rt][ct][4 * g + 3] * h_hi(u[1]);
            } else {
              const vdk_f32x2 d0 = gelu_grad_f2((vdk_f32x2){op_lo<OF>(u[0]), op_hi<OF>(u[0])}), d1 = gelu_grad_f2((vdk_f32x2){op_lo<OF>(u[1]), op_hi<OF>(u[1])});
              v[0] = acc[rt][ct][4 * g + 0] * d0[0]; v[1] = acc[rt][ct][4 * g + 1] * d0[1];
              v[2] = acc[rt][ct][4 * g + 2] * d1[0]; v[3] = acc[rt][ct][4 * g + 3] * d1[1];
            }
          } else {
#pragma unroll
            for (int e = 0; e < 4; ++e) v[e] = (E & E_BIAS) ? acc[rt][ct][4 * g + e] + bias[ct][g][e] : acc[rt][ct][4 * g + e];
          }
          if ((E & E_GELU) && (E & E_AUXD)) {
            vdk_f32x2 g0, g1, d0, d1;
            gelu_both_f2((vdk_f32x2){v[0], v[1]}, g0, d0); gelu_both_f2((vdk_f32x2){v[2], v[3]}, g1, d1);
            *(u32x2*)wp = (u32x2){pack_h2(d0[0], d0[1]), pack_h2(d1[0], d1[1])};
            held[ct][g] = (u32x2){pack_op2<OF>(g0[0], g0[1]), pack_op2<OF>(g1[0], g1[1])};
          } else
          *(u32x2*)wp = (u32x2){pack_op2<OF>(v[0], v[1]), pack_op2<OF>(v[2], v[3])};
          if ((E & E_GELU) && !(E & E_AUXD)) {
            const vdk_f32x2 g0 = gelu_f2((vdk_f32x2){v[0], v[1]}), g1 = gelu_f2((vdk_f32x2){v[2], v[3]});
            held[ct][g] = (u32x2){pack_op2<OF>(g0[0], g0[1]), pack_op2<OF>(g1[0], g1[1])};
          }
#ifndef VDK_EMU
          if ((E & (E_GELU | E_DGELU)) && g == 3) __builtin_amdgcn_sched_barrier(0);
#endif
        }
      if (E & E_GELU) {
        rows_out(rs_aux, lane_aux, (unsigned)p.ldaux * 2u, rt, false);
#pragma unroll
        for (int ct = 0; ct < NCT; ++ct)
#pragma unroll
          for (int g = 0; g < 4; ++g) *(u32x2*)(wbase + (((ct * 4 + g) ^ swz_w) << 4)) = held[ct][g];
      }
      rows_out(rs_out, lane_out, (unsigned)p.ldc * 2u, rt, (E & E_OCS) != 0);
    }
    if (E & E_OCS) {
#pragma unroll
      for (int e = 0; e < 8; ++e) {
        float s = ocs[e];
        if (NCT == 2) s += __shfl_xor(s, 8);
        s += __shfl_xor(s, 16); s += __shfl_xor(s, 32);
        ocs[e] = s;
      }
      if (lane < NCH && nok) {
        float* dst = p.ocs_part + ((long)tm * 2 + wr) * p.N + ncol;
        *(f32x4*)dst = (f32x4){ocs[0], ocs[1], ocs[2], ocs[3]};
        *(f32x4*)(dst + 4) = (f32x4){ocs[4], ocs[5], ocs[6], ocs[7]};
      }
    }
  } else if constexpr (E == (E_BIAS | E_RES | E_F32) || E == (E_BIAS | E_F32)) {
    constexpr bool RES = (E & E_RES) != 0;
    float* const slab = (float*)stage;
    const int rrow = lane >> 4, rc = lane & 15;
    const __amdgpu_buffer_rsrc_t rs_out = __builtin_amdgcn_make_buffer_rsrc(p.C, 0, (int)((unsigned)p.M * (unsigned)p.ldc * 4u), 0x00020000);
    const __amdgpu_buffer_rsrc_t rs_res = __builtin_amdgcn_make_buffer_rsrc(RES ? (void*)p.residual : p.C, 0, (int)((unsigned)p.M * (unsigned)(RES ? p.ldr : p.ldc) * 4u), 0x00020000);
    if constexpr (DEEP >= 0) W4_WAIT_VM(DEEP);
    if (p.dbg) ts[0] = __builtin_readcyclecounter();
    constexpr int NCP = NCT / 2, NB = NCP * 4;
    unsigned lane_out[NCP], lane_res[NCP];
    f32x4 bias4[NCP], cs4[NCP];
    const bool csc = p.cscale != nullptr;
#pragma unroll
    for (int cp = 0; cp < NCP; ++cp) {
      const int ncol = ncol0 + cp * 64 + rc * 4;
      const bool nok = ncol < p.N;
      lane_out[cp] = nok ? (unsigned)rrow * (unsigned)p.ldc * 4u + (unsigned)ncol * 4u : W4_OOB;
      lane_res[cp] = (RES && nok) ? (unsigned)rrow * (unsigned)p.ldr * 4u + (unsigned)ncol * 4u : W4_OOB;
      bias4[cp] = (f32x4){0.f, 0.f, 0.f, 0.f};
      cs4[cp] = (f32x4){1.f, 1.f, 1.f, 1.f};
      if (nok) bias4[cp] = *(const f32x4*)(p.bias + ncol);
      if (nok && csc) cs4[cp] = *(const f32x4*)(p.cscale + ncol);
    }
    u32x4 rn[8];
    auto res_request = [&](int b) {
      const int cp_ = b >> 2, rt_ = b & 3;
      const unsigned srow_r = (unsigned)(mrow0 + rt_ * 32) * (unsigned)p.ldr * 4u;
#pragma unroll
      for (int ps = 0; ps < 8; ++ps) rn[ps] = __builtin_amdgcn_raw_buffer_load_b128(rs_res, lane_res[cp_], srow_r + (unsigned)(ps * 4) * (unsigned)p.ldr * 4u, 0);
    };
    if (RES) res_request(0);
#pragma unroll
    for (int b = 0; b < NB; ++b) {
      const int cp = b >> 2, rt = b & 3;
      const unsigned srow_o = (unsigned)(mrow0 + rt * 32) * (unsigned)p.ldc * 4u;
      if (RES && !W4_EPI_AHEAD && b > 0) res_request(b);
      f32x4 r[8];
#pragma unroll
      for (int ps = 0; ps < 8; ++ps)
        r[ps] = RES ? (f32x4){__uint_as_float(rn[ps][0]), __uint_as_float(rn[ps][1]), __uint_as_float(rn[ps][2]), __uint_as_float(rn[ps][3])} : (f32x4){0.f, 0.f, 0.f, 0.f};
      if (RES && W4_EPI_AHEAD && b + 1 < NB) res_request(b + 1);
#pragma unroll
      for (int ctl = 0; ctl < 2; ++ctl)
#pragma unroll
        for (int g = 0; g < 4; ++g) {
          const f32x16& a = acc[rt][cp * 2 + ctl];
          *(f32x4*)(slab + l31 * 64 + (((ctl * 8 + 2 * g + hi) ^ (l31 & 15)) << 2)) = (f32x4){a[4 * g], a[4 * g + 1], a[4 * g + 2], a[4 * g + 3]};
        }
      W4_EPI_SYNC();
      f32x4 d[8];
#pragma unroll
      for (int ps = 0; ps < 8; ++ps) {
        const int row = ps * 4 + rrow;
        d[ps] = *(const f32x4*)(slab + row * 64 + ((rc ^ (row & 15)) << 2));
      }
      if (csc) {
#pragma unroll
        for (int ps = 0; ps < 8; ++ps) d[ps] = d[ps] * cs4[cp];
      }
      if (RES && p.rscale) {
#pragma unroll
        for (int ps = 0; ps < 8; ++ps) {
          int row = mrow0 + rt * 32 + ps * 4 + rrow;
          row = row < p.M ? row : p.M - 1;
          const float f = p.rscale[row / p.rps];
          d[ps] = (d[ps] + bias4[cp]) * f + r[ps];
        }
      } else
#pragma unroll
      for (int ps = 0; ps < 8; ++ps) d[ps] = RES ? (d[ps] + bias4[cp]) + r[ps] : d[ps] + bias4[cp];
#pragma unroll
      for (int ps = 0; ps < 8; ++ps) {
        const u32x4 o = {__float_as_uint(d[ps][0]), __float_as_uint(d[ps][1]), __float_as_uint(d[ps][2]), __float_as_uint(d[ps][3])};
// ... 413 lines not shown
}
int g_w4_force_band_cw = -1;
extern "C" int vdk_gemm_force_band_cw(int32_t cw) { g_w4_force_band_cw = cw; return VDK_OK; }
#else
extern int g_w4_force_band_cw;
#endif
static int w4_cus() { return vdk_gemm_w4_cus(); }

#define W4_LAUNCH(TNF, EE)                                                                                                                    \
  do {                                                                                                                                        \
    if (persist) {                                                                                                                            \
      if (ev0 || ev1) hipExtLaunchKernelGGL((gemm_w4_kernel<TNF, EE, true, VDK_W4_OF>), pgrid, dim3(256), 0, stream, (hipEvent_t)ev0, (hipEvent_t)ev1, 0, p);   \
      else hipLaunchKernelGGL((gemm_w4_kernel<TNF, EE, true, VDK_W4_OF>), pgrid, dim3(256), 0, stream, p);                                               \
    } else {                                                                                                                                  \
      if (ev0 || ev1) hipExtLaunchKernelGGL((gemm_w4_kernel<TNF, EE, false, VDK_W4_OF>), grid, dim3(256), 0, stream, (hipEvent_t)ev0, (hipEvent_t)ev1, 0, p);   \
      else hipLaunchKernelGGL((gemm_w4_kernel<TNF, EE, false, VDK_W4_OF>), grid, dim3(256), 0, stream, p);                                               \
    }                                                                                                                                         \
    return true;                                                                                                                              \
  } while (0)

static bool w4_launch_one(const GemmParams& p, bool trans, int E, unsigned tiles, unsigned splitk, hipStream_t stream, void* ev0, void* ev1);

bool W4_SYM(vdk_gemm_w4_launch)(const GemmParams& p, bool trans, int E, unsigned tiles, unsigned splitk, void* stream_, void* ev0, void* ev1) {
  hipStream_t stream = (hipStream_t)stream_;
  const unsigned G = (unsigned)w4_cus();
  const bool split_on = getenv("VDK_GEMM_W4_SPLIT") && atoi(getenv("VDK_GEMM_W4_SPLIT")) == 1;
  const int split_min_k = getenv("VDK_GEMM_W4_SPLIT_K") ? atoi(getenv("VDK_GEMM_W4_SPLIT_K")) : 1536;
  if (split_on && !trans && splitk == 1 && tiles > G && p.K >= split_min_k && E != E_GENERIC && !(E & (E_ROWGRP | E_MSTAT | E_MGRAD | E_SPLITK))) {
    const unsigned ntn = (unsigned)((p.N + 255) / 256), ntm = (unsigned)((p.M + 255) / 256);
    const unsigned rows1 = (tiles / G) * G / ntn;
    const unsigned rem_tiles = (ntm - rows1) * ntn;
    if (rows1 > 0 && rem_tiles > 0 && 2 * rem_tiles <= G) {
      GemmParams p1 = p, p2 = p;
      const long m1 = (long)rows1 * 256;
      p1.M = (int)m1;
      p2.M = p.M - (int)m1;
      p2.A = p.A + m1 * p.lda;
      p2.C = (char*)p.C + m1 * p.ldc * ((E & E_F32) ? 4 : 2);
      if (p.residual) p2.residual = p.residual + m1 * p.ldr;
      if (p.aux) p2.aux = p.aux + m1 * p.ldaux;
      if (p.ocs_part) p2.ocs_part = p.ocs_part + (size_t)rows1 * 2 * p.N;
      if (vdk_gemm_w4h_serves(p2, false)) {
        w4_launch_one(p1, false, E, rows1 * ntn, 1u, stream, ev0, nullptr);
        return W4_SYM(vdk_gemm_w4h_launch)(p2, false, E, 1u, stream_, nullptr, ev1);
      }
    }
  }
  return w4_launch_one(p, trans, E, tiles, splitk, stream, ev0, ev1);
}

static int w4_band_cw(const GemmParams& p, bool trans, unsigned tiles, unsigned G, int tile_n) {
  if (g_w4_force_band_cw >= 0) return (trans || p.conv_on) ? 0 : g_w4_force_band_cw;
  static const bool on = [] { const char* e = getenv("VDK_GEMM_BANDS"); return !(e && e[0] == '0'); }();
  if (!on || trans || p.conv_on) return 0;
  const double bbytes = (double)p.N * p.K * 2.0, abytes = (double)p.M * p.K * 2.0;
  if (bbytes <= 2.0e6) return 0;
  const int ntn = (p.N + tile_n - 1) / tile_n;
  int nb = (int)((bbytes + 2.0e6 - 1.0) / 2.0e6); if (nb > ntn) nb = ntn;
  const double rounds = (double)tiles / (double)G;
  if (nb < 2 || 8.0 * bbytes * (rounds - 1.0) <= (nb - 1) * abytes) return 0;
  return (ntn + nb - 1) / nb;
}
static bool w4_sk_xcd() { static const bool v = [] { const char* e = getenv("VDK_GEMM_SK_XCD"); return !(e && e[0] == '0'); }(); return v; }
static bool w4_launch_one(const GemmParams& p_, bool trans, int E, unsigned tiles, unsigned splitk, hipStream_t stream, void* ev0, void* ev1) {
  GemmParams p = p_;
  p.sk_xcd = (splitk > 1 && E == E_SPLITK && w4_sk_xcd()) ? 1 : 0;
  p.band_cw = splitk == 1 ? w4_band_cw(p, trans, tiles, (unsigned)w4_cus(), 256) : 0;
  const unsigned items = tiles * splitk;
  const dim3 grid = p.sk_xcd ? dim3(8u * ((items + 7u) / 8u), 1u) : dim3(tiles, splitk);
  const unsigned G = (unsigned)w4_cus();
  const bool persist = splitk == 1 && tiles > G;
  const dim3 pgrid(G, 1u);
  p.stagger = 0; p.stagger_lo = 0;
  if (persist) {
    int pct = 75, all = 0;
    if (const char* e = getenv("VDK_GEMM_W4_STAGGER")) { pct = atoi(e); all = strstr(e, "all") != nullptr; }
    if (pct > 0) {
      const int nk = p.K / 64;
      int epi = 6000;
      if (E != E_GENERIC && (E & E_GELU)) epi = 20000; else if (E != E_GENERIC && (E & E_DGELU)) epi = 20000; else if (E == E_GENERIC || (E & (E_RES | E_F32))) epi = 25000;
      p.stagger = (int)((long)(nk * 2300 + epi) * pct / 100);
      p.stagger_lo = all;
    }
  }
  if (trans) {
    switch (E) {
      case E_SPLITK: W4_LAUNCH(true, E_SPLITK);
      case E_F32: W4_LAUNCH(true, E_F32);
      case 0: W4_LAUNCH(true, 0);
      case E_MSTAT: W4_LAUNCH(true, E_MSTAT);
      case E_MGRAD: W4_LAUNCH(true, E_MGRAD);
      default: W4_LAUNCH(true, E_GENERIC);
    }
  }
  switch (E) {
    case 0: W4_LAUNCH(false, 0);
    case E_OCS: W4_LAUNCH(false, E_OCS);
    case E_DGELU | E_OCS: W4_LAUNCH(false, E_DGELU | E_OCS);
    case E_BIAS: W4_LAUNCH(false, E_BIAS);
    case E_BIAS | E_GELU: W4_LAUNCH(false, E_BIAS | E_GELU);
    case E_DGELU: W4_LAUNCH(false, E_DGELU);
    case E_BIAS | E_GELU | E_AUXD: W4_LAUNCH(false, E_BIAS | E_GELU | E_AUXD);
    case E_DGELU | E_AUXD: W4_LAUNCH(false, E_DGELU | E_AUXD);
    case E_DGELU | E_OCS | E_AUXD: W4_LAUNCH(false, E_DGELU | E_OCS | E_AUXD);
    case E_BIAS | E_RES | E_F32: W4_LAUNCH(false, E_BIAS | E_RES | E_F32);
    case E_BIAS | E_F32: W4_LAUNCH(false, E_BIAS | E_F32);
    case E_BIAS | E_RES | E_F32 | E_ROWGRP: W4_LAUNCH(false, E_BIAS | E_RES | E_F32 | E_ROWGRP);
    case E_SPLITK: W4_LAUNCH(false, E_SPLITK);
    case E_F32: W4_LAUNCH(false, E_F32);
    default: W4_LAUNCH(false, E_GENERIC);
  }
  return false;
}

#define W4H_LAUNCH(TNF, EE)                                                                                                             \
  do {                                                                                                                                  \
    if (ev0 || ev1) hipExtLaunchKernelGGL((gemm_w4h_kernel<TNF, EE, VDK_W4_OF>), grid, dim3(256), 0, stream, (hipEvent_t)ev0, (hipEvent_t)ev1, 0, p);     \
    else hipLaunchKernelGGL((gemm_w4h_kernel<TNF, EE, VDK_W4_OF>), grid, dim3(256), 0, stream, p);                                                 \
    return true;                                                                                                                        \
  } while (0)

bool W4_SYM(vdk_gemm_w4h_launch)(const GemmParams& p_, bool trans, int E, unsigned splitk, void* stream_, void* ev0, void* ev1) {
  hipStream_t stream = (hipStream_t)stream_;
  GemmParams p = p_;
  const dim3 grid((unsigned)(((p.M + 255) / 256) * ((p.N + 127) / 128)), splitk);
  p.band_cw = splitk == 1 ? w4_band_cw(p, trans, grid.x, 2u * (unsigned)w4_cus(), 128) : 0;
  {
    static const int stag_pct = getenv("VDK_GEMM_W4H_STAGGER") ? atoi(getenv("VDK_GEMM_W4H_STAGGER")) : 0;
    const int cus = w4_cus();
    const int nk = (p.k_per_split < p.K ? p.k_per_split : p.K) / 64;
    int epi = 7000;
    if (E != E_GENERIC && (E & E_GELU)) epi = 20000; else if (E != E_GENERIC && (E & E_DGELU)) epi = 30000; else if (E == E_GENERIC || (E & (E_RES | E_F32 | E_SPLITK))) epi = 30000;
    p.stagger_lo = cus;
    p.stagger = ((int)grid.x >= 2 * cus && splitk == 1) ? (int)((long)(4000 + nk * 2400 + epi) / 2 * stag_pct / 100) : 0;
  }
  if (trans) {
    switch (E) {
      case E_SPLITK: W4H_LAUNCH(true, E_SPLITK);
      case E_F32: W4H_LAUNCH(true, E_F32);
      case 0: W4H_LAUNCH(true, 0);
      default: W4H_LAUNCH(true, E_GENERIC);
    }
  }
  switch (E) {
    case 0: W4H_LAUNCH(false, 0);
    case E_OCS: W4H_LAUNCH(false, E_OCS);
    case E_DGELU | E_OCS: W4H_LAUNCH(false, E_DGELU | E_OCS);
    case E_BIAS: W4H_LAUNCH(false, E_BIAS);
    case E_BIAS | E_GELU: W4H_LAUNCH(false, E_BIAS | E_GELU);
    case E_DGELU: W4H_LAUNCH(false, E_DGELU);
    case E_BIAS | E_GELU | E_AUXD: W4H_LAUNCH(false, E_BIAS | E_GELU | E_AUXD);
    case E_DGELU | E_AUXD: W4H_LAUNCH(false, E_DGELU | E_AUXD);
    case E_DGELU | E_OCS | E_AUXD: W4H_LAUNCH(false, E_DGELU | E_OCS | E_AUXD);
    case E_BIAS | E_RES | E_F32: W4H_LAUNCH(false, E_BIAS | E_RES | E_F32);
    case E_BIAS | E_F32: W4H_LAUNCH(false, E_BIAS | E_F32);
    case E_BIAS | E_RES | E_F32 | E_ROWGRP: W4H_LAUNCH(false, E_BIAS | E_RES | E_F32 | E_ROWGRP);
    case E_SPLITK: W4H_LAUNCH(false, E_SPLITK);
    case E_F32: W4H_LAUNCH(false, E_F32);
    default: W4H_LAUNCH(false, E_GENERIC);
  }
  return false;
}
```

visiondk_amd/csrc/vdk_attn_tile.h:

```cpp
#pragma once
#include <hip/hip_runtime.h>
#include "vdk_device.h"

#define AS_ROW 128

__device__ __forceinline__ int as_f(int r) { return (((r >> 1) & 1) << 2) | ((r >> 2) & 3); }

__device__ __forceinline__ void as_dma_rows(unsigned char* arr, const bf16_t* __restrict__ src, long ld, int N, int R8, int w, int nw, int lane) {
  for (int j = w; j < (R8 >> 3); j += nw) {
    const int row = 8 * j + (lane >> 3);
    const int c = (lane & 7) ^ as_f(row);
    const int srow = row < N ? row : N - 1;
    const bf16_t* g = src + (long)srow * ld + c * 8;
    __builtin_amdgcn_global_load_lds(VDK_GLOBAL_PTR(g), VDK_LDS_PTR(arr + j * 1024), 16, 0, 0);
  }
}
__device__ __forceinline__ void as_dma16_raw(const bf16_t* g, unsigned char* lds_dst) {
#ifdef VDK_EMU
  __builtin_amdgcn_global_load_lds(VDK_GLOBAL_PTR(g), VDK_LDS_PTR(lds_dst), 16, 0, 0);
#else
  const unsigned dst = (unsigned)__builtin_amdgcn_readfirstlane((int)(unsigned)(unsigned long long)VDK_LDS_PTR(lds_dst));
  asm volatile("s_mov_b32 m0, %1\n\ts_nop 0\n\tglobal_load_lds_dwordx4 %0, off" ::"v"(g), "s"(dst) : "memory");
#endif
}
__device__ __forceinline__ void as_dma_rows_raw(unsigned char* arr, const bf16_t* __restrict__ src, long ld, int N, int R8, int w, int nw, int lane) {
  for (int j = w; j < (R8 >> 3); j += nw) {
    const int row = 8 * j + (lane >> 3);
    const int c = (lane & 7) ^ as_f(row);
    const int srow = row < N ? row : N - 1;
    as_dma16_raw(src + (long)srow * ld + c * 8, arr + j * 1024);
  }
}
__device__ __forceinline__ s16x8 as_row_frag(const unsigned char* arr, int row, int ks, int hi) {
  return *(const s16x8*)(arr + row * AS_ROW + (((2 * ks + hi) ^ as_f(row)) << 4));
}
__device__ __forceinline__ s16x8 as_tr_frag(const unsigned char* arr, int t1, int d0, int lane) {
  const int s = lane & 15, chalf = (lane >> 4) & 1, hi = lane >> 5;
  const int r1 = t1 + 4 * hi + (s >> 2), r2 = r1 + 8;
  const int byte = 2 * d0 + 32 * chalf + 8 * (s & 3);
  const unsigned char* p1 = arr + r1 * AS_ROW + (((byte >> 4) ^ as_f(r1)) << 4) + (byte & 8);
  const unsigned char* p2 = arr + r2 * AS_ROW + (((byte >> 4) ^ as_f(r2)) << 4) + (byte & 8);
  s16x4 lo = __builtin_amdgcn_ds_read_tr16_b64_v4i16(VDK_LDS_S16X4(p1));
  s16x4 up = __builtin_amdgcn_ds_read_tr16_b64_v4i16(VDK_LDS_S16X4(p2));
  s16x8 r = {lo[0], lo[1], lo[2], lo[3], up[0], up[1], up[2], up[3]};
  return r;
}
struct AsLane { int row[4]; int tr[2][2]; };
__device__ __forceinline__ AsLane as_lane(int lane) {
  AsLane a;
  const int l31 = lane & 31, hi = lane >> 5;
#pragma unroll
  for (int ks = 0; ks < 4; ++ks) a.row[ks] = l31 * AS_ROW + (((2 * ks + hi) ^ as_f(l31)) << 4);
  const int s = lane & 15, chalf = (lane >> 4) & 1;
  const int r1 = 4 * hi + (s >> 2), r2 = r1 + 8;
#pragma unroll
  for (int dh = 0; dh < 2; ++dh) {
    const int byte = 64 * dh + 32 * chalf + 8 * (s & 3);
    a.tr[dh][0] = r1 * AS_ROW + (((byte >> 4) ^ as_f(r1)) << 4) + (byte & 8);
    a.tr[dh][1] = r2 * AS_ROW + (((byte >> 4) ^ as_f(r2)) << 4) + (byte & 8);
  }
  return a;
}
__device__ __forceinline__ s16x8 as_row_frag_l(const unsigned char* tile, const AsLane& a, int ks) { return *(const s16x8*)(tile + a.row[ks]); }
__device__ __forceinline__ s16x8 as_tr_frag_l(const unsigned char* tile, const AsLane& a, int dh) {
  s16x4 lo = __builtin_amdgcn_ds_read_tr16_b64_v4i16(VDK_LDS_S16X4(tile + a.tr[dh][0]));
  s16x4 up = __builtin_amdgcn_ds_read_tr16_b64_v4i16(VDK_LDS_S16X4(tile + a.tr[dh][1]));
  s16x8 r = {lo[0], lo[1], lo[2], lo[3], up[0], up[1], up[2], up[3]};
  return r;
}
__device__ __forceinline__ f32x16 as_zero16() {
  f32x16 z;
#pragma unroll
  for (int r = 0; r < 16; ++r) z[r] = 0.f;
  return z;
}
template <int OF = 0>
__device__ __forceinline__ void as_pack_b(const f32x16& p, s16x8 (&f)[2]) {
#pragma unroll
  for (int s = 0; s < 2; ++s) {
    u32x4 u = {pack_op2<OF>(p[8 * s + 0], p[8 * s + 1]), pack_op2<OF>(p[8 * s + 2], p[8 * s + 3]), pack_op2<OF>(p[8 * s + 4], p[8 * s + 5]), pack_op2<OF>(p[8 * s + 6], p[8 * s + 7])};
    f[s] = *(s16x8*)&u;
  }
}
template <int OF = 0>
__device__ __forceinline__ void as_store_tile(unsigned char* tile, const f32x16& x0, const f32x16& x1, float mul, bf16_t* __restrict__ dst, long ld, int row0, int N,
                                              int lane) {
  const int l31 = lane & 31, hi = lane >> 5;
  if (row0 + l31 < N) {
#pragma unroll
    for (int g = 0; g < 4; ++g) {
      const int ch = g ^ (l31 & 7), ch1 = (4 + g) ^ (l31 & 7);
      *(u32x2*)(tile + l31 * AS_ROW + (ch << 4) + 8 * hi) = (u32x2){pack_op2<OF>(x0[4 * g] * mul, x0[4 * g + 1] * mul), pack_op2<OF>(x0[4 * g + 2] * mul, x0[4 * g + 3] * mul)};
      *(u32x2*)(tile + l31 * AS_ROW + (ch1 << 4) + 8 * hi) = (u32x2){pack_op2<OF>(x1[4 * g] * mul, x1[4 * g + 1] * mul), pack_op2<OF>(x1[4 * g + 2] * mul, x1[4 * g + 3] * mul)};
    }
  }
  VDK_WAVE_LDS_SYNC();
#pragma unroll
  for (int p = 0; p < 4; ++p) {
    const int r = 8 * p + (lane >> 3), cp = lane & 7;
    if (row0 + r < N) {
      const u32x4 v = *(const u32x4*)(tile + r * AS_ROW + ((cp ^ (r & 7)) << 4));
      *(u32x4*)(dst + (long)(row0 + r) * ld + cp * 8) = v;
    }
  }
  VDK_WAVE_LDS_SYNC();
}
```

visiondk_amd/csrc/vdk_gemm.h:

```cpp
#pragma once
#include "visiondk.h"
#include "vdk_device.h"
#include "vdk_margin.h"

typedef VdkGemmDesc GemmDesc;

struct GemmParams {
  const bf16_t* A; const bf16_t* B; void* C;
  long lda, ldb, ldc;
  int M, N, K;
  int c_dtype;
  const float* bias;
  const float* residual; long ldr;
  int act;
  bf16_t* aux; long ldaux;
  float alpha;
  int row_group;
  int row_shift;
  int a_row_group;
  int splitk; int k_per_split;
  float* slabs;
  int* sk_cnt;
  float* ocs_part;
  float* colsum_part;
  int conv_on, cCin, cH, cW, cOH, cOW, cKH, cKW, cstride, cpad, ctrans;
  int crows;
  unsigned char* q8; long ldq8; const float* q8_scale; float* q8_amax; int q8_fmt;
  MarginEpi me;
  unsigned long long* dbg;
  int band_cw;
  int sk_xcd;
  int stagger, stagger_lo;
  int opf;
  const float* cscale;
  const float* rscale; int rps;
};

extern "C" int vdk_gemm_bf16_nt(const VdkGemmDesc* d, void* ws, size_t ws_bytes, void* stream);
extern "C" int vdk_transpose_bf16(const void* in, int64_t ldi, int32_t R, int32_t C, void* out, int64_t ldo, int32_t Rpad, int32_t in_row_group, float* colsum_partial, void* stream);
void vdk_gemm_tn_prefer_half(int on);
int vdk_transpose_16(const void* in, int64_t ldi, int32_t R, int32_t C, void* out, int64_t ldo, int32_t Rpad, int32_t in_row_group, float* colsum_partial, int opf, void* stream);

bool vdk_gemm_w4_serves(const GemmParams& p, bool trans);
bool vdk_gemm_w4_launch(const GemmParams& p, bool trans, int E, unsigned tiles, unsigned splitk, void* stream, void* ev0, void* ev1);
bool vdk_gemm_w4h_serves(const GemmParams& p, bool trans);
bool vdk_gemm_w4h_launch(const GemmParams& p, bool trans, int E, unsigned splitk, void* stream, void* ev0, void* ev1);
bool vdk_gemm_w4_launch_f16(const GemmParams& p, bool trans, int E, unsigned tiles, unsigned splitk, void* stream, void* ev0, void* ev1);
bool vdk_gemm_w4h_launch_f16(const GemmParams& p, bool trans, int E, unsigned splitk, void* stream, void* ev0, void* ev1);
int vdk_gemm_w4_cus();
```

visiondk_amd/csrc/vdk_gemm_epilogue.h:

```cpp
#pragma once
#include "vdk_gemm.h"

template <int OF = 0>
__device__ __forceinline__ void g_epilogue_store8(const GemmParams& p, long mi, int n, float (&v)[8], int z) {
    const long m = p.row_group > 0 ? mi + (mi / p.row_group + 1) * p.row_shift : mi;
    const long mr = p.row_group > 0 ? mi % p.row_group + p.row_shift : mi;
    if (p.splitk > 1) {
      float* dst = p.slabs + ((long)z * p.M + mi) * p.N + n;
      *(f32x4*)dst = (f32x4){v[0], v[1], v[2], v[3]};
      *(f32x4*)(dst + 4) = (f32x4){v[4], v[5], v[6], v[7]};
      return;
    }
    if (p.alpha != 1.0f) {
#pragma unroll
      for (int e = 0; e < 8; ++e) v[e] *= p.alpha;
    }
    if (p.cscale) {
      f32x4 c0 = *(const f32x4*)(p.cscale + n), c1 = *(const f32x4*)(p.cscale + n + 4);
#pragma unroll
      for (int e = 0; e < 4; ++e) { v[e] *= c0[e]; v[4 + e] *= c1[e]; }
    }
    if (p.bias) {
      f32x4 b0 = *(const f32x4*)(p.bias + n), b1 = *(const f32x4*)(p.bias + n + 4);
#pragma unroll
      for (int e = 0; e < 4; ++e) { v[e] += b0[e]; v[4 + e] += b1[e]; }
    }
    if (p.act == VDK_ACT_GELU) {
      if (p.aux) {
        u32x4 u = {pack_op2<OF>(v[0], v[1]), pack_op2<OF>(v[2], v[3]), pack_op2<OF>(v[4], v[5]), pack_op2<OF>(v[6], v[7])};
        *(u32x4*)(p.aux + m * p.ldaux + n) = u;
      }
#pragma unroll
      for (int e = 0; e < 4; ++e) { const vdk_f32x2 g2 = gelu_f2((vdk_f32x2){v[2 * e], v[2 * e + 1]}); v[2 * e] = g2[0]; v[2 * e + 1] = g2[1]; }
    } else if (p.act == VDK_ACT_DGELU) {
      u32x4 u = *(const u32x4*)(p.aux + m * p.ldaux + n);
#pragma unroll
      for (int e = 0; e < 4; ++e) {
        const vdk_f32x2 d2 = gelu_grad_f2((vdk_f32x2){op_lo<OF>(u[e]), op_hi<OF>(u[e])});
        v[2 * e] *= d2[0];
        v[2 * e + 1] *= d2[1];
      }
    } else if (p.act == VDK_ACT_GELU_SAVE_GRAD) {
      float d[8];
#pragma unroll
      for (int e = 0; e < 8; ++e) gelu_both_f(v[e], v[e], d[e]);
      *(u32x4*)(p.aux + m * p.ldaux + n) = (u32x4){pack_h2(d[0], d[1]), pack_h2(d[2], d[3]), pack_h2(d[4], d[5]), pack_h2(d[6], d[7])};
    } else if (p.act == VDK_ACT_MUL_AUX) {
      u32x4 u = *(const u32x4*)(p.aux + m * p.ldaux + n);
#pragma unroll
      for (int e = 0; e < 4; ++e) { v[2 * e] *= h_lo(u[e]); v[2 * e + 1] *= h_hi(u[e]); }
    }
    if (p.rscale) {
      const float f = p.rscale[mi / p.rps];
#pragma unroll
      for (int e = 0; e < 8; ++e) v[e] *= f;
    }
    if (p.residual) {
      const float* rs = p.residual + mr * p.ldr + n;
      f32x4 r0 = *(const f32x4*)rs, r1 = *(const f32x4*)(rs + 4);
#pragma unroll
      for (int e = 0; e < 4; ++e) { v[e] += r0[e]; v[4 + e] += r1[e]; }
    }
    if (p.c_dtype == VDK_F32) {
      float* dst = (float*)p.C + m * p.ldc + n;
      *(f32x4*)dst = (f32x4){v[0], v[1], v[2], v[3]};
      *(f32x4*)(dst + 4) = (f32x4){v[4], v[5], v[6], v[7]};
    } else {
      u32x4 o = {pack_op2<OF>(v[0], v[1]), pack_op2<OF>(v[2], v[3]), pack_op2<OF>(v[4], v[5]), pack_op2<OF>(v[6], v[7])};
      *(u32x4*)((bf16_t*)p.C + m * p.ldc + n) = o;
    }
}


#define E_BIAS 1
#define E_GELU 2
#define E_DGELU 4
#define E_RES 8
#define E_F32 16
#define E_SPLITK 32
#define E_ROWGRP 64
#define E_OCS 128
#define E_MSTAT 256
#define E_MGRAD 512
#define E_Q8 1024
#define E_AUXD 2048
#define E_GENERIC 0x1000

template <int E, int NPS = 8 , bool SWZ = false, int OF = 0 >
__device__ __forceinline__ void h_epilogue_half(const GemmParams& p, const float* slab, int lane, long mbase ,
                                                int n, int z, const float (&bias8)[8], float (&ocs)[8], float& q8am) {
  const int rsub = lane >> 3, cc = (lane & 7) * 8;
  if (E & E_MSTAT) {
    const MarginEpi& me = p.me;
#pragma unroll
    for (int ps = 0; ps < NPS; ++ps) {
      const long mi = mbase + ps * 8 + rsub;
      const bool rok = mi < me.B;
      const int row = ps * 8 + rsub, sw = SWZ ? (row & 15) : 0;
      f32x4 x0 = *(const f32x4*)(slab + row * 64 + (((cc >> 2) ^ sw) << 2)), x1 = *(const f32x4*)(slab + row * 64 + ((((cc >> 2) + 1) ^ sw) << 2));
      float v[8] = {x0[0], x0[1], x0[2], x0[3], x1[0], x1[1], x1[2], x1[3]};
      MarginP P = me.P;
      long yt = -1; RowCtx R; R.thr = 0.f; R.final_gt = 0.f; R.dfinal = 1.f;
      if (rok) { margin_row_params(P, (int)mi); yt = me.labels[mi]; R = margin_row_ctx(P, me.gt ? me.gt[mi] : 0.f); }
      float m = -3.0e38f, sl = 0.f, lg[8];
#pragma unroll
      for (int e = 0; e < 8; ++e) {
        lg[e] = -3.0e38f;
        if (rok && n + e < me.C) {
          float jc; margin_eval(P, R, v[e], (long)(n + e) == yt, lg[e], jc);
          sl += lg[e]; m = fmaxf(m, lg[e]);
          if ((long)(n + e) == yt) me.tlogit[mi] = lg[e];
        }
      }
      float se = 0.f;
#pragma unroll
      for (int e = 0; e < 8; ++e) se += (lg[e] > -1.0e38f) ? vdk_vexp(lg[e] - m) : 0.f;
#pragma unroll
      for (int off = 1; off < 8; off <<= 1) {
        const float m2 = __shfl_xor(m, off), s2 = __shfl_xor(se, off);
        sl += __shfl_xor(sl, off);
        const float M = fmaxf(m, m2);
        se = se * vdk_vexp(m - M) + s2 * vdk_vexp(m2 - M);
        m = M;
      }
      if (rok && (lane & 7) == 0 && n < p.N) *(f32x4*)(me.stats + ((long)mi * me.nslice + (n >> 6)) * 4) = (f32x4){m, se, sl, 0.f};
    }
    return;
  }
  if (n >= p.N) return;
  long mo[NPS], mr[NPS];
  bool ok[NPS];
#pragma unroll
  for (int ps = 0; ps < NPS; ++ps) {
    const long mi = mbase + ps * 8 + rsub;
    ok[ps] = mi < p.M;
    mo[ps] = (E & E_ROWGRP) ? mi + (mi / p.row_group + 1) * p.row_shift : mi;
    mr[ps] = (E & E_ROWGRP) ? mi % p.row_group + p.row_shift : mi;
  }
  f32x4 r0[NPS], r1[NPS];
  u32x4 ux[NPS];
  float q8s = 1.0f, q8lim = 448.0f;
  if (E & E_Q8) { q8s = p.q8_scale ? p.q8_scale[0] : 1.0f; q8lim = p.q8_fmt == 0 ? 448.0f : 57344.0f; }
  if (E & E_RES) {
#pragma unroll
    for (int ps = 0; ps < NPS; ++ps)
      if (ok[ps]) { const float* rs = p.residual + mr[ps] * p.ldr + n; r0[ps] = *(const f32x4*)rs; r1[ps] = *(const f32x4*)(rs + 4); }
  }
  if (E & E_DGELU) {
#pragma unroll
    for (int ps = 0; ps < NPS; ++ps)
      if (ok[ps]) ux[ps] = *(const u32x4*)(p.aux + mo[ps] * p.ldaux + n);
  }
#pragma unroll
  for (int ps = 0; ps < NPS; ++ps) {
    if (!ok[ps]) continue;
    const int row = ps * 8 + rsub, sw = SWZ ? (row & 15) : 0;
    float v[8];
    f32x4 x0 = *(const f32x4*)(slab + row * 64 + (((cc >> 2) ^ sw) << 2)), x1 = *(const f32x4*)(slab + row * 64 + ((((cc >> 2) + 1) ^ sw) << 2));
#pragma unroll
    for (int e = 0; e < 4; ++e) { v[e] = x0[e]; v[4 + e] = x1[e]; }
    if (E & E_SPLITK) {
      float* dst = p.slabs + ((long)z * p.M + (mbase + row)) * p.N + n;
      *(f32x4*)dst = x0; *(f32x4*)(dst + 4) = x1;
      continue;
    }
    if ((E & E_F32) && p.cscale) {
      const f32x4 c0 = *(const f32x4*)(p.cscale + n), c1 = *(const f32x4*)(p.cscale + n + 4);
#pragma unroll
      for (int e = 0; e < 4; ++e) { v[e] *= c0[e]; v[4 + e] *= c1[e]; }
    }
    if (E & E_BIAS) {
#pragma unroll
      for (int e = 0; e < 8; ++e) v[e] += bias8[e];
    }
    if ((E & E_GELU) && (E & E_AUXD)) {
      float dv[8];
#pragma unroll
      for (int e = 0; e < 8; ++e) gelu_both_f(v[e], v[e], dv[e]);
      *(u32x4*)(p.aux + mo[ps] * p.ldaux + n) = (u32x4){pack_h2(dv[0], dv[1]), pack_h2(dv[2], dv[3]), pack_h2(dv[4], dv[5]), pack_h2(dv[6], dv[7])};
    } else if (E & E_GELU) {
      *(u32x4*)(p.aux + mo[ps] * p.ldaux + n) = (u32x4){pack_op2<OF>(v[0], v[1]), pack_op2<OF>(v[2], v[3]), pack_op2<OF>(v[4], v[5]), pack_op2<OF>(v[6], v[7])};
#pragma unroll
      for (int e = 0; e < 4; ++e) { const vdk_f32x2 g2 = gelu_f2((vdk_f32x2){v[2 * e], v[2 * e + 1]}); v[2 * e] = g2[0]; v[2 * e + 1] = g2[1]; }
    }
    if ((E & E_DGELU) && (E & E_AUXD)) {
#pragma unroll
      for (int e = 0; e < 4; ++e) { v[2 * e] *= h_lo(ux[ps][e]); v[2 * e + 1] *= h_hi(ux[ps][e]); }
    } else if (E & E_DGELU) {
#pragma unroll
      for (int e = 0; e < 4; ++e) { const vdk_f32x2 d2 = gelu_grad_f2((vdk_f32x2){op_lo<OF>(ux[ps][e]), op_hi<OF>(ux[ps][e])}); v[2 * e] *= d2[0]; v[2 * e + 1] *= d2[1]; }
    }
    if (E & E_RES) {
      if (p.rscale) {
        const float f = p.rscale[(mbase + row) / p.rps];
#pragma unroll
        for (int e = 0; e < 8; ++e) v[e] *= f;
      }
#pragma unroll
      for (int e = 0; e < 4; ++e) { v[e] += r0[ps][e]; v[4 + e] += r1[ps][e]; }
    }
    if (E & E_MGRAD) {
      const MarginEpi& me = p.me;
      const long mi = mbase + row;
      if (mi < me.B) {
        MarginP P = me.P; margin_row_params(P, (int)mi);
        const long yt = me.labels[mi];
        const RowCtx R = margin_row_ctx(P, me.gt ? me.gt[mi] : 0.f);
        const float M = me.rowstat[2 * mi], inv = me.rowstat[2 * mi + 1];
#pragma unroll
        for (int e = 0; e < 8; ++e) {
          float lgv, jc; margin_eval(P, R, v[e], (long)(n + e) == yt, lgv, jc);
          float gd = vdk_vexp(lgv - M) * inv - me.epsc;
          if ((long)(n + e) == yt) gd -= (1.0f - me.smoothing);
          v[e] = (n + e < me.C) ? gd * me.gscale * jc : 0.f;
        }
      } else {
#pragma unroll
        for (int e = 0; e < 8; ++e) v[e] = 0.f;
      }
    }
    if (E & E_F32) {
      float* dst = (float*)p.C + mo[ps] * p.ldc + n;
      *(f32x4*)dst = (f32x4){v[0], v[1], v[2], v[3]};
      *(f32x4*)(dst + 4) = (f32x4){v[4], v[5], v[6], v[7]};
    } else {
      const u32x4 o = {pack_op2<OF>(v[0], v[1]), pack_op2<OF>(v[2], v[3]), pack_op2<OF>(v[4], v[5]), pack_op2<OF>(v[6], v[7])};
      *(u32x4*)((bf16_t*)p.C + mo[ps] * p.ldc + n) = o;
      if (E & E_OCS) {
#pragma unroll
        for (int e = 0; e < 4; ++e) { ocs[2 * e] += op_lo<OF>(o[e]); ocs[2 * e + 1] += op_hi<OF>(o[e]); }
      }
      if (E & E_Q8) {
        float c[8];
#pragma unroll
        for (int e = 0; e < 4; ++e) {
          const float a = op_lo<OF>(o[e]), b = op_hi<OF>(o[e]);
          q8am = fmaxf(q8am, fmaxf(fabsf(a), fabsf(b)));
          c[2 * e] = fminf(fmaxf(a * q8s, -q8lim), q8lim); c[2 * e + 1] = fminf(fmaxf(b * q8s, -q8lim), q8lim);
        }
// ... 14 lines not shown
```

visiondk_amd/csrc/vit_engine.hip:

```cpp
#include <hip/hip_runtime.h>
#include <stdlib.h>
#include <stdio.h>
#include <string.h>
#include "vdk_device.h"
#include "vdk_host.h"
#include "vdk_gemm.h"

extern "C" {
int vdk_layernorm_fwd(const float*, int64_t, int32_t, int32_t, const float*, const float*, float, void*, int64_t, int32_t, float*, float*, void*);
int vdk_layernorm_bwd_workspace_bytes(int32_t, int32_t, size_t*);
int vdk_layernorm_bwd(const void*, int64_t, int32_t, const float*, int64_t, const float*, const float*, const float*, const float*, int64_t,
                      int32_t, int32_t, float*, int64_t, void*, int64_t, float*, float*, void*, size_t, void*);
int vdk_reduce_rows_f32(const float*, int64_t, int32_t, int64_t, float*, float, void*);
int vdk_colsum_bf16_workspace_bytes(int32_t, int32_t, size_t*);
int vdk_colsum_bf16(const void*, int64_t, int32_t, int32_t, float*, void*, size_t, void*);
int vdk_attention_fwd(const void*, int64_t, void*, int64_t, float*, int32_t, int32_t, int32_t, int32_t, float, void*);
int vdk_attention_bwd(const void*, int64_t, const void*, const void*, int64_t, const float*, void*, int64_t, float*, int32_t, int32_t, int32_t,
                      int32_t, float, void*);
int vdk_attention_fwd_dt(const void*, int64_t, void*, int64_t, float*, int32_t, int32_t, int32_t, int32_t, float, int32_t, void*);
int vdk_attention_bwd_dt(const void*, int64_t, const void*, const void*, int64_t, const float*, void*, int64_t, float*, int32_t, int32_t, int32_t, int32_t, float, int32_t, void*);
int vdk_attention_bwd_cs(const void*, int64_t, const void*, const void*, int64_t, const float*, void*, int64_t, float*, int32_t, int32_t, int32_t, int32_t, float, int32_t, float*, int32_t*,
                         void*);
int vdk_patchify_bf16(const float*, int32_t, int32_t, int32_t, int32_t, int32_t, void*, int32_t, void*);
int vdk_cls_rows(float*, int64_t, int32_t, int32_t, const float*, const float*, void*);
int vdk_cast_f32_bf16(const float*, void*, int64_t, void*);
int vdk_transpose_cast_f32_bf16(const float*, int64_t, int32_t, int32_t, void*, int64_t, int32_t, void*);
int vdk_gemm_f32_nt(const VdkGemmF32Desc*, void*);
int vdk_gemm_a_colsum_rows(int32_t, int32_t, int32_t);
int vdk_softmax_rows_f32(float*, int64_t, int64_t, int32_t, float, void*);
int vdk_patchify_f32(const float*, int32_t, int32_t, int32_t, int32_t, int32_t, float*, void*);
int vdk_quant_fp8(const void*, int32_t, int64_t, const float*, void*, int32_t, float*, void*);
int vdk_fp8_scale_update(float*, float*, float*, int32_t, int32_t, float, void*);
int vdk_gemm_fp8_nt(const VdkGemmDesc*, int32_t, int32_t, const float*, const float*, void*);
int vdk_gemm_fp8_nt_q8(const VdkGemmDesc*, int32_t, int32_t, const float*, const float*, void*, int64_t, int32_t, const float*, float*, void*);
int vdk_layernorm_fwd_q8(const float*, int64_t, int32_t, int32_t, const float*, const float*, float, void*, int64_t, float*, float*, void*, int64_t, int32_t, const float*, float*, void*);
}


static thread_local int t_opf = VDK_OPF_BF16;
#define DT16 (t_opf ? VDK_F16 : VDK_BF16)
static bool gelu_saved_grad() {
  static const int v = [] { const char* e = getenv("VDK_VIT_GELU_SAVED_GRAD"); return e ? atoi(e) : -1; }();
  return v < 0 ? t_opf != 0 : v != 0;
}
#define ACT_FC1 (gelu_saved_grad() ? VDK_ACT_GELU_SAVE_GRAD : VDK_ACT_GELU)
#define ACT_DFC2 (gelu_saved_grad() ? VDK_ACT_MUL_AUX : VDK_ACT_DGELU)

static inline int64_t up(int64_t x, int64_t a) { return (x + a - 1) / a * a; }

struct VitDims {
  int B, img, ps, Cin, D, L, H, M, C, Cp, np, N, T, Kraw, Kpe, Tp, Bp, cls, pre , fp8, opf ;
  float eps;
};
static int vit_dims(const VdkVitConfig* c, VitDims* d) {
  if (!c) return vdk_fail(VDK_EINVAL, "vit: null config");
  d->B = c->batch; d->img = c->img_size; d->ps = c->patch_size; d->Cin = c->in_chans; d->D = c->dim; d->L = c->depth;
  d->H = c->heads; d->M = c->mlp_dim; d->C = c->num_classes; d->eps = c->ln_eps;
  if (d->B <= 0 || d->img <= 0 || d->ps <= 0 || d->img % d->ps || d->Cin <= 0 || d->D <= 0 || d->L <= 0 || d->H <= 0 || d->M <= 0 || d->C < 0)
    return vdk_fail(VDK_EINVAL, "vit: bad config value");
  if (d->D != d->H * 64) return vdk_fail(VDK_EUNSUPPORTED, "vit: head_dim must be 64 (dim == 64 * heads)");
  if ((d->D & 7) || (d->M & 7)) return vdk_fail(VDK_EUNSUPPORTED, "vit: dim and mlp_dim must be multiples of 8");
  d->Kraw = d->Cin * d->ps * d->ps;
  d->Kpe = (int)up(d->Kraw, 8);
  d->np = (d->img / d->ps) * (d->img / d->ps);
  d->cls = c->no_class_token ? 0 : 1;
  d->pre = c->pre_norm ? 1 : 0;
  if (d->pre && c->fp8) return vdk_fail(VDK_EUNSUPPORTED, "vit: pre_norm and the fp8 mode are not combined");
  if (!d->cls && d->C > 0) return vdk_fail(VDK_EUNSUPPORTED, "vit: no_class_token is feature mode only (num_classes == 0)");
  d->N = d->np + d->cls;
  d->T = d->B * d->N;
  d->Cp = (int)up(d->C, 8);
  d->Tp = (int)up(d->T, 64);
  d->Bp = (int)up(d->B, 64);
  d->fp8 = c->fp8;
  if (d->fp8 < 0 || d->fp8 > 2) return vdk_fail(VDK_EINVAL, "vit: fp8 must be 0, 1 or 2");
  if (c->operand != VDK_BF16 && c->operand != VDK_F16) return vdk_fail(VDK_EINVAL, "vit: operand must be VDK_BF16 or VDK_F16");
  d->opf = c->operand == VDK_F16 ? VDK_OPF_F16 : VDK_OPF_BF16;
  if (d->opf && d->fp8) return vdk_fail(VDK_EUNSUPPORTED, "vit: the fp8 mode goes with bf16 operands");
  if (d->fp8 && (d->D < 256 || (d->D % 128) || (d->M % 128))) return vdk_fail(VDK_EUNSUPPORTED, "vit: the fp8 mode needs dim >= 256, dim and mlp_dim % 128 == 0");
  return VDK_OK;
}

struct PEntry { char name[64]; int64_t off, numel; int64_t shape[4]; int ndim; };
struct PLayout {
  int64_t cls, pos, pe_w, pe_b, npre_w, npre_b, norm_w, norm_b, head_w, head_b, total;
  struct Blk { int64_t n1w, n1b, qkv_w, qkv_b, proj_w, proj_b, n2w, n2b, fc1_w, fc1_b, fc2_w, fc2_b; };
  Blk blk[64];
  struct BlkT { int64_t qkv, proj, fc1, fc2; } blkT[64];
  int64_t headT, totalT;
};
static int64_t p_take(int64_t& cur, int64_t n) { int64_t o = cur; cur = up(cur + n, 64); return o; }
static int vit_layout(const VitDims& d, PLayout* p) {
  if (d.L > 64) return vdk_fail(VDK_EUNSUPPORTED, "vit: depth > 64");
  int64_t cur = 0;
  p->cls = d.cls ? p_take(cur, d.D) : 0;
  p->pos = p_take(cur, (int64_t)d.N * d.D);
  p->pe_w = p_take(cur, (int64_t)d.D * d.Kraw);
  p->pe_b = p_take(cur, d.D);
  p->npre_w = p->npre_b = 0;
  if (d.pre) { p->npre_w = p_take(cur, d.D); p->npre_b = p_take(cur, d.D); }
  for (int l = 0; l < d.L; ++l) {
    PLayout::Blk& b = p->blk[l];
    b.n1w = p_take(cur, d.D); b.n1b = p_take(cur, d.D);
    b.qkv_w = p_take(cur, (int64_t)3 * d.D * d.D); b.qkv_b = p_take(cur, 3 * d.D);
    b.proj_w = p_take(cur, (int64_t)d.D * d.D); b.proj_b = p_take(cur, d.D);
    b.n2w = p_take(cur, d.D); b.n2b = p_take(cur, d.D);
    b.fc1_w = p_take(cur, (int64_t)d.M * d.D); b.fc1_b = p_take(cur, d.M);
    b.fc2_w = p_take(cur, (int64_t)d.D * d.M); b.fc2_b = p_take(cur, d.D);
  }
  p->norm_w = p_take(cur, d.D); p->norm_b = p_take(cur, d.D);
  p->head_w = p->head_b = cur;
  if (d.C > 0) {
    p->head_w = p_take(cur, (int64_t)d.Cp * d.D);
    p->head_b = p_take(cur, d.Cp);
  }
  p->total = cur;
  int64_t t = 0;
  for (int l = 0; l < d.L; ++l) {
    p->blkT[l].qkv = p_take(t, (int64_t)d.D * 3 * d.D);
    p->blkT[l].proj = p_take(t, (int64_t)d.D * d.D);
    p->blkT[l].fc1 = p_take(t, (int64_t)d.D * d.M);
    p->blkT[l].fc2 = p_take(t, (int64_t)d.M * d.D);
  }
  p->headT = t;
  if (d.C > 0) p->headT = p_take(t, (int64_t)d.D * d.Cp);
  p->totalT = t;
  return VDK_OK;
}

static void pe_set(PEntry* e, const char* name, int64_t off, int ndim, int64_t s0, int64_t s1 = 1, int64_t s2 = 1, int64_t s3 = 1) {
  snprintf(e->name, sizeof(e->name), "%s", name);
  e->off = off; e->ndim = ndim; e->shape[0] = s0; e->shape[1] = s1; e->shape[2] = s2; e->shape[3] = s3;
  e->numel = s0 * s1 * s2 * s3;
}
static int vit_entry(const VitDims& d, const PLayout& p, int idx, PEntry* e) {
  const int per = 12, nb0 = d.pre ? 5 : 4, ntens = nb0 + per * d.L + (d.C > 0 ? 4 : 2);
  if (!d.cls) { if (idx < 0) return -1; ++idx; }
  if (idx < 0 || idx >= ntens) return -1;
  char nm[64];
  if (idx == 0) { pe_set(e, "cls_token", p.cls, 3, 1, 1, d.D); return 0; }
  if (idx == 1) { pe_set(e, "pos_embed", p.pos, 3, 1, d.N, d.D); return 0; }
  if (idx == 2) { pe_set(e, "patch_embed.proj.weight", p.pe_w, 4, d.D, d.Cin, d.ps, d.ps); return 0; }
  if (idx == 3 && !d.pre) { pe_set(e, "patch_embed.proj.bias", p.pe_b, 1, d.D); return 0; }
  if (idx == 3) { pe_set(e, "norm_pre.weight", p.npre_w, 1, d.D); return 0; }
  if (idx == 4 && d.pre) { pe_set(e, "norm_pre.bias", p.npre_b, 1, d.D); return 0; }
  if (idx < nb0 + per * d.L) {
    int l = (idx - nb0) / per, k = (idx - nb0) % per;
    const PLayout::Blk& b = p.blk[l];
    static const char* suffix[12] = {"norm1.weight", "norm1.bias", "attn.qkv.weight", "attn.qkv.bias", "attn.proj.weight", "attn.proj.bias",
                                     "norm2.weight", "norm2.bias", "mlp.fc1.weight", "mlp.fc1.bias", "mlp.fc2.weight", "mlp.fc2.bias"};
    snprintf(nm, sizeof(nm), "blocks.%d.%s", l, suffix[k]);
    switch (k) {
      case 0: pe_set(e, nm, b.n1w, 1, d.D); break;
      case 1: pe_set(e, nm, b.n1b, 1, d.D); break;
      case 2: pe_set(e, nm, b.qkv_w, 2, 3 * d.D, d.D); break;
      case 3: pe_set(e, nm, b.qkv_b, 1, 3 * d.D); break;
      case 4: pe_set(e, nm, b.proj_w, 2, d.D, d.D); break;
      case 5: pe_set(e, nm, b.proj_b, 1, d.D); break;
      case 6: pe_set(e, nm, b.n2w, 1, d.D); break;
      case 7: pe_set(e, nm, b.n2b, 1, d.D); break;
      case 8: pe_set(e, nm, b.fc1_w, 2, d.M, d.D); break;
      case 9: pe_set(e, nm, b.fc1_b, 1, d.M); break;
      case 10: pe_set(e, nm, b.fc2_w, 2, d.D, d.M); break;
      default: pe_set(e, nm, b.fc2_b, 1, d.D); break;
    }
    return 0;
  }
  int k = idx - nb0 - per * d.L;
  if (k == 0) pe_set(e, "norm.weight", p.norm_w, 1, d.D);
  else if (k == 1) pe_set(e, "norm.bias", p.norm_b, 1, d.D);
  else if (k == 2) pe_set(e, "head.weight", p.head_w, 2, d.C, d.D);
  else pe_set(e, "head.bias", p.head_b, 1, d.C);
  return 0;
}

// ... 329 lines not shown
  RC(vdk_transpose_16(Xa, ldx, rows, in, tB, rows_pad, rows_pad, 0, nullptr, t_opf, s));
  const int sk = wgrad_splitk(out, in, rows_pad);
  RC(gemm(s, tA, rows_pad, tB, rows_pad, dW, in, out, in, rows_pad, VDK_F32, nullptr, nullptr, 0, VDK_ACT_NONE, nullptr, 0, sk, 0, base + w.slabs,
          w.slabs_bytes));
  if (csp) RC(vdk_reduce_rows_f32(csp, out, (rows_pad + 63) / 64, out, db, 1.0f, s));
  return VDK_OK;
}

static bool qkvb_pass(int T, int N, size_t csws_bytes) {
  static const int env = getenv("VDK_VIT_QKVB_PASS") ? atoi(getenv("VDK_VIT_QKVB_PASS")) : -1;
  if (env == 0) return false;
  size_t need = 0;
  if (vdk_colsum_bf16_workspace_bytes(T, N, &need) != VDK_OK || need > csws_bytes) return false;
  return true;
}

static int dgrad_with_bias(hipStream_t s, const WsPlan& w, char* base, const bf16_t* dY, int64_t lddy, const bf16_t* Wt, int64_t ldw, void* dX, int64_t lddx, int rows,
                           int in, int out, int act, void* aux, int64_t ldaux, float* db, int* fused, int slot, VdkReduceJob* jobs, int* njobs,
                           float* dbx = nullptr, int* fusedx = nullptr, int slotx = 0) {
  const int prow = db ? vdk_gemm_a_colsum_rows(rows, in, out) : 0;
  *fused = (db && !t_opf && prow > 0 && (size_t)prow * out * 4 <= w.csws_bytes) ? 1 : 0;
  const int xrow = dbx ? vdk_gemm_c_colsum_rows(rows, in, out) : 0;
  const int fx = (dbx && !*fused && xrow > 0 && (size_t)xrow * in * 4 <= w.csws_bytes) ? 1 : 0;
  if (fusedx) *fusedx = fx;
  float* const part = (float*)(base + w.csws + (size_t)slot * w.csws_bytes);
  float* const partx = (float*)(base + w.csws + (size_t)slotx * w.csws_bytes);
  VdkGemmDesc g = {};
  g.A = dY; g.lda = lddy; g.B = Wt; g.ldb = ldw; g.C = dX; g.ldc = lddx; g.M = rows; g.N = in; g.K = out; g.c_dtype = DT16; g.act = act; g.aux = aux;
  g.ldaux = ldaux; g.alpha = 1.0f; g.splitk = 1; g.ab_dtype = DT16;
  if (*fused) g.a_colsum = part;
  if (fx) g.c_colsum = partx;
  RC(vdk_gemm_bf16_nt(&g, nullptr, 0, s));
  if (*fused) jobs[(*njobs)++] = VdkReduceJob{part, (long)out, prow, (long)out, db, 1.0f};
  if (fx) jobs[(*njobs)++] = VdkReduceJob{partx, (long)in, xrow, (long)in, dbx, 1.0f};
  return VDK_OK;
}

int vdk_vit_backward(const VdkVitConfig* cfg, const void* dlogits, const float* params, const void* wb16, const void* wt16, void* ws,
                     size_t ws_bytes, float* grads, vdk_grad_ready_fn on_ready, void* user, void* stream_, void* side_stream_) {
  hipStream_t s = (hipStream_t)stream_;
  hipStream_t s2 = side_stream_ ? (hipStream_t)side_stream_ : s;
  VitDims d; RC(vit_dims(cfg, &d));
  PLayout p; RC(vit_layout(d, &p));
  WsPlan w; RC(vit_plan(d, &w));
  if (!dlogits || !params || !wb16 || !wt16 || !ws || !grads) return vdk_fail(VDK_EINVAL, "vdk_vit_backward: null pointer");
  if (ws_bytes < w.total) return vdk_fail(VDK_EWORKSPACE, "vdk_vit_backward: workspace too small");
  t_opf = d.opf;
  char* base = (char*)ws;
  const bf16_t* wt = (const bf16_t*)wt16;
  const int T = d.T, D = d.D, M = d.M;
  float* X = (float*)(base + w.X);
  float* stats = (float*)(base + w.stats);
  const size_t XS = (size_t)T * D;
  float* dxa = (float*)(base + w.dxa); float* dxm = (float*)(base + w.dxm);
#define DXAB(l) ((bf16_t*)(base + w.dxab[((l) + 3) % 3]))
#define DXMB(l) ((bf16_t*)(base + w.dxmb[((l) + 2) & 1]))
#define DU(l) ((bf16_t*)(base + w.du[((l) + 2) & 1]))
#define DQKV(l) ((bf16_t*)(base + w.dqkv[((l) + 2) & 1]))
  bf16_t* dsm = (bf16_t*)(base + w.dsm);
  float* dvec = (float*)(base + w.dvec);
  void* lnws = base + w.lnws;
  const size_t EV_SIDE_DONE = 8;
  size_t ev_p = EV_SIDE_DONE + d.L + 4;
  RC(ev_order(0, s, s2));

  bool last_fc2_bias_done = false;
  if (d.C == 0) {
    float* xl = X + (size_t)(2 * d.L) * XS;
    float* meanf = stats + (size_t)d.L * 4 * T; float* rstdf = meanf + T;
    RC(vdk_layernorm_bwd_deferred(dlogits, D, VDK_F32, xl, D, meanf, rstdf, params + p.norm_w, nullptr, 0, T, D, dxa, D, DXAB(d.L - 1), D, grads + p.norm_w,
                                  grads + p.norm_b, lnws, w.lnws_bytes, s, nullptr, nullptr, nullptr, nullptr, t_opf));
    if (on_ready) on_ready(user, p.norm_w, p.total - p.norm_w);
  } else {
    const bf16_t* dl = (const bf16_t*)dlogits;
    bf16_t* hf = (bf16_t*)(base + w.hf);
    RC(linear_wgrad(s, d, w, base, dl, d.Cp, hf, D, d.B, d.Bp, d.Cp, D, grads + p.head_w, grads + p.head_b, 0));
    bf16_t* dhf = (bf16_t*)(base + w.dhf);
    RC(gemm(s, dl, d.Cp, wt + p.headT, d.Cp, dhf, D, d.B, D, d.Cp, DT16, nullptr, nullptr, 0, VDK_ACT_NONE, nullptr, 0, 1, 0, nullptr, 0));
    if (hipMemsetAsync(dxa, 0, XS * 4, s) != hipSuccess || hipMemsetAsync(DXAB(d.L - 1), 0, XS * 2, s) != hipSuccess)
      return vdk_fail(VDK_ELAUNCH, "vdk_vit_backward: memset failed");
    float* xl = X + (size_t)(2 * d.L) * XS;
    float* meanf = stats + (size_t)d.L * 4 * T; float* rstdf = meanf + T;
    if (s2 == s && D <= 1024) {
      VdkReduceJob fj[2];
      RC(vdk_layernorm_bwd_deferred(dhf, D, DT16, xl, (int64_t)d.N * D, meanf, rstdf, params + p.norm_w, nullptr, 0, d.B, D, dxa, (int64_t)d.N * D, DXAB(d.L - 1),
                                    (int64_t)d.N * D, grads + p.norm_w, grads + p.norm_b, lnws, w.lnws_bytes, s, &fj[0], grads + p.blk[d.L - 1].fc2_b, &fj[1]));
      if (fj[0].in) RC(vdk_reduce_rows_batch(fj, 2, s)); else RC(vdk_reduce_rows_batch(fj + 1, 1, s));
      last_fc2_bias_done = true;
    } else
    RC(vdk_layernorm_bwd(dhf, D, DT16, xl, (int64_t)d.N * D, meanf, rstdf, params + p.norm_w, nullptr, 0, d.B, D, dxa, (int64_t)d.N * D, DXAB(d.L - 1),
                         (int64_t)d.N * D, grads + p.norm_w, grads + p.norm_b, lnws, w.lnws_bytes, s));
    if (on_ready) on_ready(user, p.norm_w, p.total - p.norm_w);
  }
  bool fc2_bias_from_norm1 = false, dxab8_ready = false;
  F8 f8; RC(f8_init(cfg, d, p, &f8, (unsigned char*)(base + w.a8), (unsigned char*)(base + w.a8b)));
  for (int l = d.L - 1; l >= 0; --l) {
    const PLayout::Blk& b = p.blk[l];
    float* xin = X + (size_t)(2 * l) * XS; float* xmid = xin + XS;
    float* mean1 = stats + (size_t)l * 4 * T; float* rstd1 = mean1 + T; float* mean2 = rstd1 + T; float* rstd2 = mean2 + T;
    bf16_t* h1 = (bf16_t*)(base + w.h1 + l * w.s_h); bf16_t* qkv = (bf16_t*)(base + w.qkv + l * w.s_qkv);
    float* lse = (float*)(base + w.lse + l * w.s_lse); bf16_t* o = (bf16_t*)(base + w.o + l * w.s_h);
    bf16_t* h2 = (bf16_t*)(base + w.h2 + l * w.s_h); bf16_t* u = (bf16_t*)(base + w.u + l * w.s_u); bf16_t* g = (bf16_t*)(base + w.g + l * w.s_u);
    bf16_t* dxab = DXAB(l); bf16_t* dxmb = DXMB(l); bf16_t* du = DU(l); bf16_t* dqkv = DQKV(l);
    if (s2 != s && l + 2 <= d.L - 1) { hipEvent_t e; RC(ev_get(EV_SIDE_DONE + l + 3, &e)); if (hipStreamWaitEvent(s, e, 0) != hipSuccess) return vdk_fail(VDK_ELAUNCH, "vit: wait failed"); }
    int fz = 0;
    const bool one_stream = (s2 == s);
    VdkReduceJob jobs[8]; int nj = 0;
    char* const lnws0 = base + w.lnws; char* const lnws1 = lnws0 + w.lnws_bytes;
    RC(ev_order(ev_p++, s, s2));
    if (f8.mode) {
      const int sl = 12 * l;
      const bool have_fc2b = one_stream && ((l == d.L - 1) ? last_fc2_bias_done : fc2_bias_from_norm1);
      const bool fq = f8_fused(f8) && (M % 64) == 0;
      const int xrow = one_stream ? 2 * ((T + 255) / 256) : 0;
      const bool fo = xrow > 0 && (size_t)xrow * M * 4 <= w.csws_bytes;
      float* const partx = (float*)(base + w.csws + (size_t)1 * w.csws_bytes);
      RC(gemm8(s, f8, dxab, sl + 8, 1, f8.wt8 + p.blkT[l].fc2, sl + 7, D, du, M, T, M, D, VDK_BF16, nullptr, nullptr, 0, VDK_ACT_DGELU, u, M, dxab8_ready ? f8.a8 : nullptr,
               fq ? sl + 9 : -1, 1, fo ? partx : nullptr));
      if (fo) jobs[nj++] = VdkReduceJob{partx, (long)M, xrow, (long)M, grads + b.fc1_b, 1.0f};
      RC(linear_wgrad(s2, d, w, base, dxab, D, g, M, T, d.Tp, D, M, grads + b.fc2_w, have_fc2b ? nullptr : grads + b.fc2_b, 0));
      RC(gemm8(s, f8, du, sl + 9, 1, f8.wt8 + p.blkT[l].fc1, sl + 6, M, dsm, D, T, D, M, VDK_BF16, nullptr, nullptr, 0, VDK_ACT_NONE, nullptr, 0, fq ? f8.a8b : nullptr));
      RC(linear_wgrad(s2, d, w, base, du, M, h2, D, T, d.Tp, M, D, grads + b.fc1_w, fo ? nullptr : grads + b.fc1_b, 0));
    } else if (one_stream) {
      int fx = 0;
      const bool have_fc2b = (l == d.L - 1) ? last_fc2_bias_done : fc2_bias_from_norm1;
      RC(dgrad_with_bias(s, w, base, dxab, D, wt + p.blkT[l].fc2, D, du, M, T, M, D, ACT_DFC2, u, M, have_fc2b ? nullptr : grads + b.fc2_b, &fz, 0, jobs, &nj,
                         grads + b.fc1_b, &fx, 1));
      RC(linear_wgrad(s2, d, w, base, dxab, D, g, M, T, d.Tp, D, M, grads + b.fc2_w, (fz || have_fc2b) ? nullptr : grads + b.fc2_b, 0));
      if (fx) {
        RC(gemm(s, du, M, wt + p.blkT[l].fc1, M, dsm, D, T, D, M, DT16, nullptr, nullptr, 0, VDK_ACT_NONE, nullptr, 0, 1, 0, nullptr, 0));
        fz = 1;
      } else {
        RC(dgrad_with_bias(s, w, base, du, M, wt + p.blkT[l].fc1, M, dsm, D, T, D, M, VDK_ACT_NONE, nullptr, 0, grads + b.fc1_b, &fz, 1, jobs, &nj));
      }
      RC(linear_wgrad(s2, d, w, base, du, M, h2, D, T, d.Tp, M, D, grads + b.fc1_w, fz ? nullptr : grads + b.fc1_b, 0));
    } else {
      RC(linear_wgrad(s2, d, w, base, dxab, D, g, M, T, d.Tp, D, M, grads + b.fc2_w, grads + b.fc2_b, 0));
      RC(gemm(s, dxab, D, wt + p.blkT[l].fc2, D, du, M, T, M, D, DT16, nullptr, nullptr, 0, ACT_DFC2, u, M, 1, 0, nullptr, 0));
      RC(ev_order(ev_p++, s, s2));
      RC(linear_wgrad(s2, d, w, base, du, M, h2, D, T, d.Tp, M, D, grads + b.fc1_w, grads + b.fc1_b, 0));
      RC(gemm(s, du, M, wt + p.blkT[l].fc1, M, dsm, D, T, D, M, DT16, nullptr, nullptr, 0, VDK_ACT_NONE, nullptr, 0, 1, 0, nullptr, 0));
    }
    const bool ocs_ln = one_stream && D <= 1024;
    static const bool g16_on = !(getenv("VDK_VIT_G16") && atoi(getenv("VDK_VIT_G16")) == 0);
    const bool g16 = g16_on && ocs_ln && !f8.mode && t_opf == VDK_OPF_F16 && D > 512 && D <= 1024;
    const bool lq = f8.mode && f8_fused(f8) && ocs_ln;
    const LnQ8 q8m = {f8.a8, (long)D, f8.sc + 12 * l + 10, f8.amax + 12 * l + 10, 1};
    if (g16) RC(vdk_layernorm_bwd_deferred(dsm, D, DT16, xmid, D, mean2, rstd2, params + b.n2w, nullptr, D, T, D, nullptr, D, dxmb, D, grads + b.n2w, grads + b.n2b, lnws0,
                                           w.lnws_bytes, s, &jobs[nj], grads + b.proj_b, &jobs[nj + 1], nullptr, 0, nullptr, nullptr, 1, dxab));
    else
    RC(vdk_layernorm_bwd_deferred(dsm, D, DT16, xmid, D, mean2, rstd2, params + b.n2w, dxa, D, T, D, dxm, D, dxmb, D, grads + b.n2w, grads + b.n2b, lnws0,
                                  w.lnws_bytes, s, &jobs[nj], ocs_ln ? grads + b.proj_b : nullptr, ocs_ln ? &jobs[nj + 1] : nullptr, lq ? &q8m : nullptr));
    nj += ocs_ln ? 2 : 1;
    RC(ev_order(ev_p++, s, s2));
    if (f8.mode) {
      RC(gemm8(s, f8, dxmb, 12 * l + 10, 1, f8.wt8 + p.blkT[l].proj, 12 * l + 5, D, dsm, D, T, D, D, VDK_BF16, nullptr, nullptr, 0, VDK_ACT_NONE, nullptr, 0, lq ? f8.a8 : nullptr));
      RC(linear_wgrad(s2, d, w, base, dxmb, D, o, D, T, d.Tp, D, D, grads + b.proj_w, ocs_ln ? nullptr : grads + b.proj_b, 0));
    } else if (one_stream && ocs_ln) {
      RC(gemm(s, dxmb, D, wt + p.blkT[l].proj, D, dsm, D, T, D, D, DT16, nullptr, nullptr, 0, VDK_ACT_NONE, nullptr, 0, 1, 0, nullptr, 0));
      RC(linear_wgrad(s2, d, w, base, dxmb, D, o, D, T, d.Tp, D, D, grads + b.proj_w, nullptr, 0));
    } else if (one_stream) {
      RC(dgrad_with_bias(s, w, base, dxmb, D, wt + p.blkT[l].proj, D, dsm, D, T, D, D, VDK_ACT_NONE, nullptr, 0, grads + b.proj_b, &fz, 2, jobs, &nj));
      RC(linear_wgrad(s2, d, w, base, dxmb, D, o, D, T, d.Tp, D, D, grads + b.proj_w, fz ? nullptr : grads + b.proj_b, 0));
    } else {
      RC(linear_wgrad(s2, d, w, base, dxmb, D, o, D, T, d.Tp, D, D, grads + b.proj_w, grads + b.proj_b, 0));
      RC(gemm(s, dxmb, D, wt + p.blkT[l].proj, D, dsm, D, T, D, D, DT16, nullptr, nullptr, 0, VDK_ACT_NONE, nullptr, 0, 1, 0, nullptr, 0));
    }
    int32_t qkvb_done = 0;
    {
      static const bool fuse_on = !(getenv("VDK_VIT_QKVB_ATTN") && atoi(getenv("VDK_VIT_QKVB_ATTN")) == 0);
      float* csp = (fuse_on && !f8.mode && one_stream && (size_t)d.B * 3 * D * 4 <= w.csws_bytes) ? (float*)(base + w.csws + (size_t)3 * w.csws_bytes) : nullptr;
      RC(vdk_attention_bwd_cs(qkv, 3 * D, o, dsm, D, lse, dqkv, 3 * D, dvec, d.B, d.N, d.H, 64, 0.125f, DT16, csp, &qkvb_done, s));
      if (qkvb_done) { jobs[nj] = VdkReduceJob{csp, (long)3 * D, d.B, (long)3 * D, grads + b.qkv_b, 1.0f}; ++nj; }
    }
    RC(ev_order(ev_p++, s, s2));
    if (f8.mode) {
      size_t csneed = 0; vdk_colsum_bf16_workspace_bytes(T, 3 * D, &csneed);
      const bool fcq = f8_fused(f8) && one_stream && csneed <= w.csws_bytes;
      if (fcq) {
        const LnQ8 q8d = {f8.a8, (long)3 * D, f8.sc + 12 * l + 11, f8.amax + 12 * l + 11, 1};
        RC(vdk_colsum_bf16_deferred(dqkv, 3 * D, T, 3 * D, grads + b.qkv_b, base + w.csws + (size_t)2 * w.csws_bytes, w.csws_bytes, s, &jobs[nj], &q8d)); ++nj;
      }
      RC(gemm8(s, f8, dqkv, 12 * l + 11, 1, f8.wt8 + p.blkT[l].qkv, 12 * l + 4, 3 * D, dsm, D, T, D, 3 * D, VDK_BF16, nullptr, nullptr, 0, VDK_ACT_NONE, nullptr, 0,
               fcq ? f8.a8 : nullptr));
      RC(linear_wgrad(s2, d, w, base, dqkv, 3 * D, h1, D, T, d.Tp, 3 * D, D, grads + b.qkv_w, fcq ? nullptr : grads + b.qkv_b, 0));
    } else if (one_stream && (qkvb_done || qkvb_pass(T, 3 * D, w.csws_bytes))) {
      if (!qkvb_done) { RC(vdk_colsum_bf16_deferred(dqkv, 3 * D, T, 3 * D, grads + b.qkv_b, base + w.csws + (size_t)3 * w.csws_bytes, w.csws_bytes, s, &jobs[nj], nullptr, t_opf)); ++nj; }
      RC(gemm(s, dqkv, 3 * D, wt + p.blkT[l].qkv, 3 * D, dsm, D, T, D, 3 * D, DT16, nullptr, nullptr, 0, VDK_ACT_NONE, nullptr, 0, 1, 0, nullptr, 0));
      RC(linear_wgrad(s2, d, w, base, dqkv, 3 * D, h1, D, T, d.Tp, 3 * D, D, grads + b.qkv_w, nullptr, 0));
    } else if (one_stream) {
      RC(dgrad_with_bias(s, w, base, dqkv, 3 * D, wt + p.blkT[l].qkv, 3 * D, dsm, D, T, D, 3 * D, VDK_ACT_NONE, nullptr, 0, grads + b.qkv_b, &fz, 3, jobs, &nj));
      RC(linear_wgrad(s2, d, w, base, dqkv, 3 * D, h1, D, T, d.Tp, 3 * D, D, grads + b.qkv_w, fz ? nullptr : grads + b.qkv_b, 0));
    } else {
      RC(linear_wgrad(s2, d, w, base, dqkv, 3 * D, h1, D, T, d.Tp, 3 * D, D, grads + b.qkv_w, grads + b.qkv_b, 0));
      RC(gemm(s, dqkv, 3 * D, wt + p.blkT[l].qkv, 3 * D, dsm, D, T, D, 3 * D, DT16, nullptr, nullptr, 0, VDK_ACT_NONE, nullptr, 0, 1, 0, nullptr, 0));
    }
    const bool ocs_n1 = ocs_ln && l > 0;
    const bool lq1 = lq && ocs_n1;
    const LnQ8 q8a = {f8.a8, (long)D, f8.sc + 12 * (l - 1) + 8, f8.amax + 12 * (l - 1) + 8, 1};
    if (g16 && l > 0) RC(vdk_layernorm_bwd_deferred(dsm, D, DT16, xin, D, mean1, rstd1, params + b.n1w, nullptr, D, T, D, nullptr, D, DXAB(l - 1), D, grads + b.n1w, grads + b.n1b, lnws1,
                                                    w.lnws_bytes, s, &jobs[nj], grads + p.blk[l - 1].fc2_b, &jobs[nj + 1], nullptr, 0, nullptr, nullptr, 1, dxmb));
    else if (g16) {
      float* const dummy_cs = (float*)(base + w.csws);
      RC(vdk_layernorm_bwd_deferred(dsm, D, DT16, xin, D, mean1, rstd1, params + b.n1w, nullptr, D, T, D, dxa, D, DXAB(l - 1), D, grads + b.n1w, grads + b.n1b, lnws1,
                                    w.lnws_bytes, s, &jobs[nj], dummy_cs, &jobs[nj + 1], nullptr, 0, nullptr, nullptr, 1, dxmb));
    } else
    RC(vdk_layernorm_bwd_deferred(dsm, D, DT16, xin, D, mean1, rstd1, params + b.n1w, dxm, D, T, D, dxa, D, DXAB(l - 1), D, grads + b.n1w, grads + b.n1b, lnws1,
                                  w.lnws_bytes, s, &jobs[nj], ocs_n1 ? grads + p.blk[l - 1].fc2_b : nullptr, ocs_n1 ? &jobs[nj + 1] : nullptr, lq1 ? &q8a : nullptr));
    dxab8_ready = lq1;
    nj += ocs_n1 ? 2 : 1;
    fc2_bias_from_norm1 = ocs_n1;
    RC(vdk_reduce_rows_batch(jobs, nj, s));
    if (s2 != s) { hipEvent_t e; RC(ev_get(EV_SIDE_DONE + l + 1, &e)); if (hipEventRecord(e, s2) != hipSuccess) return vdk_fail(VDK_ELAUNCH, "vit: record failed"); }
    if (on_ready) {
      if (s2 != s) { hipEvent_t e; RC(ev_get(EV_SIDE_DONE + l + 1, &e)); if (hipStreamWaitEvent(s, e, 0) != hipSuccess) return vdk_fail(VDK_ELAUNCH, "vit: wait failed"); }
      on_ready(user, b.n1w, (l + 1 < d.L ? p.blk[l + 1].n1w : p.norm_w) - b.n1w);
    }
  }
  {
    float* dposall = (float*)(base + w.dposall);
    const float* dx0 = dxa;
    if (d.pre) {
      const float* ps = (const float*)(base + w.pstats);
      RC(vdk_layernorm_bwd_deferred(dxa, D, VDK_F32, (const float*)(base + w.xe), D, ps, ps + T, params + p.npre_w, nullptr, 0, T, D, dxm, D, DXAB(-1), D, grads + p.npre_w,
                                    grads + p.npre_b, lnws, w.lnws_bytes, s, nullptr, nullptr, nullptr, nullptr, t_opf));
      dx0 = dxm;
    }
    RC(vdk_reduce_rows_f32(dx0, (int64_t)d.N * D, d.B, (int64_t)d.N * D, grads + p.pos, 1.0f, s));
    if (d.cls && hipMemcpyAsync(grads + p.cls, grads + p.pos, (size_t)D * 4, hipMemcpyDeviceToDevice, s) != hipSuccess)
      return vdk_fail(VDK_ELAUNCH, "vdk_vit_backward: memcpy failed");
    if (!d.pre) RC(vdk_reduce_rows_f32(grads + p.pos + (size_t)d.cls * D, D, d.np, D, grads + p.pe_b, 1.0f, s));
    else if (hipMemsetAsync(grads + p.pe_b, 0, (size_t)D * 4, s) != hipSuccess) return vdk_fail(VDK_ELAUNCH, "vdk_vit_backward: memset failed");
    (void)dposall;
    bf16_t* patches = (bf16_t*)(base + w.patches);
    const int rows = d.B * d.np, rows_pad = (int)up(rows, 64);
    RC(ev_order(ev_p++, s, s2));
    float* dwpe = d.Kraw != d.Kpe ? (float*)(base + w.dwpe) : grads + p.pe_w;
    RC(linear_wgrad(s2, d, w, base, DXAB(-1), D, patches, d.Kpe, rows, rows_pad, D, d.Kpe, dwpe, nullptr, d.cls ? d.np : 0));
    if (d.Kraw != d.Kpe && hipMemcpy2DAsync(grads + p.pe_w, (size_t)d.Kraw * 4, dwpe, (size_t)d.Kpe * 4, (size_t)d.Kraw * 4, D, hipMemcpyDeviceToDevice, s2) != hipSuccess)
      return vdk_fail(VDK_ELAUNCH, "vdk_vit_backward: memcpy2d failed");
    RC(ev_order(ev_p++, s2, s));
    if (on_ready) on_ready(user, 0, p.blk[0].n1w);
  }
#undef DXAB
#undef DXMB
#undef DU
#undef DQKV
  return vdk_check_launch("vdk_vit_backward");
}

}

struct WsF32 { size_t total, patches, xa, xb, h, qkv, S, o, u; int Np; };
static void vit_plan_f32(const VitDims& d, WsF32* w) {
  size_t cur = 0;
  const size_t T = d.T, D = d.D;
  w->Np = (int)up(d.N, 4);
  w->patches = w_take(cur, (size_t)d.B * d.np * d.Kpe * 4);
  w->xa = w_take(cur, T * D * 4); w->xb = w_take(cur, T * D * 4); w->h = w_take(cur, T * D * 4);
  w->qkv = w_take(cur, (T + 8) * 3 * D * 4);
  w->S = w_take(cur, (size_t)d.B * d.H * d.N * w->Np * 4);
  w->o = w_take(cur, T * D * 4);
  w->u = w_take(cur, T * (size_t)d.M * 4);
  w->total = cur;
}
static int gemm32(hipStream_t s, const float* A, int64_t lda, const float* B, int64_t ldb, float* C, int64_t ldc, int M, int N, int K, const float* bias,
                  const float* res, int64_t ldr, int act) {
  VdkGemmF32Desc g = {};
  g.A = A; g.lda = lda; g.B = B; g.ldb = ldb; g.C = C; g.ldc = ldc; g.M = M; g.N = N; g.K = K; g.bias = bias; g.residual = res; g.ldr = ldr; g.act = act;
  g.alpha = 1.0f;
  return vdk_gemm_f32_nt(&g, s);
}

extern "C" {

int vdk_vit_workspace_f32_bytes(const VdkVitConfig* cfg, size_t* bytes) {
  VitDims d; RC(vit_dims(cfg, &d));
  if (!bytes) return vdk_fail(VDK_EINVAL, "null");
  WsF32 w; vit_plan_f32(d, &w);
  *bytes = w.total;
  return VDK_OK;
}

int vdk_vit_forward_f32(const VdkVitConfig* cfg, const float* x, const float* params, void* ws, size_t ws_bytes, float* logits, void* stream_) {
  hipStream_t s = (hipStream_t)stream_;
  VitDims d; RC(vit_dims(cfg, &d));
  if (d.Kraw != d.Kpe) return vdk_fail(VDK_EUNSUPPORTED, "vdk_vit_forward_f32: in_chans*patch*patch must be a multiple of 8 on the fp32 path");
  PLayout p; RC(vit_layout(d, &p));
  WsF32 w; vit_plan_f32(d, &w);
  if (!x || !params || !ws || !logits) return vdk_fail(VDK_EINVAL, "vdk_vit_forward_f32: null pointer");
  if (ws_bytes < w.total) return vdk_fail(VDK_EWORKSPACE, "vdk_vit_forward_f32: workspace too small");
  if ((long)d.B * d.H > 65535) return vdk_fail(VDK_EUNSUPPORTED, "vdk_vit_forward_f32: batch * heads <= 65535");
  char* base = (char*)ws;
  const int T = d.T, D = d.D, M = d.M, N = d.N, Np = w.Np;
  float* patches = (float*)(base + w.patches);
  float* xa = (float*)(base + w.xa); float* xb = (float*)(base + w.xb); float* h = (float*)(base + w.h);
  float* qkv = (float*)(base + w.qkv); float* S = (float*)(base + w.S); float* o = (float*)(base + w.o); float* u = (float*)(base + w.u);
  if (hipMemsetAsync(qkv + (size_t)T * 3 * D, 0, (size_t)8 * 3 * D * 4, s) != hipSuccess) return vdk_fail(VDK_ELAUNCH, "vdk_vit_forward_f32: memset failed");
  RC(vdk_patchify_f32(x, d.B, d.Cin, d.img, d.img, d.ps, patches, s));
  {
    VdkGemmF32Desc g = {};
    g.A = patches; g.lda = d.Kpe; g.B = params + p.pe_w; g.ldb = d.Kpe; g.C = xa + (size_t)d.cls * D; g.ldc = D; g.M = d.np; g.N = D; g.K = d.Kpe;
    g.bias = params + p.pe_b; g.residual = params + p.pos + (size_t)d.cls * D; g.ldr = D; g.alpha = 1.0f;
    g.batch1 = d.B; g.batch2 = 1; g.sa1 = (int64_t)d.np * d.Kpe; g.sc1 = (int64_t)N * D;
    if (d.B > 65535) return vdk_fail(VDK_EUNSUPPORTED, "vdk_vit_forward_f32: batch <= 65535");
    RC(vdk_gemm_f32_nt(&g, s));
  }
  if (d.cls) RC(vdk_cls_rows(xa, (int64_t)N * D, d.B, D, params + p.cls, params + p.pos, s));
  if (d.pre) {
    RC(vdk_layernorm_fwd(xa, D, T, D, params + p.npre_w, params + p.npre_b, d.eps, xb, D, VDK_F32, nullptr, nullptr, s));
    float* t = xa; xa = xb; xb = t;
  }
  for (int l = 0; l < d.L; ++l) {
    const PLayout::Blk& b = p.blk[l];
    RC(vdk_layernorm_fwd(xa, D, T, D, params + b.n1w, params + b.n1b, d.eps, h, D, VDK_F32, nullptr, nullptr, s));
    RC(gemm32(s, h, D, params + b.qkv_w, D, qkv, 3 * D, T, 3 * D, D, params + b.qkv_b, nullptr, 0, VDK_ACT_NONE));
    {
      VdkGemmF32Desc g = {};
      g.A = qkv; g.lda = 3 * D; g.B = qkv + D; g.ldb = 3 * D; g.C = S; g.ldc = Np; g.M = N; g.N = N; g.K = 64; g.alpha = 1.0f;
      g.batch1 = d.B; g.batch2 = d.H; g.sa1 = (int64_t)N * 3 * D; g.sa2 = 64; g.sb1 = g.sa1; g.sb2 = 64; g.sc1 = (int64_t)d.H * N * Np; g.sc2 = (int64_t)N * Np;
      RC(vdk_gemm_f32_nt(&g, s));
      RC(vdk_softmax_rows_f32(S, Np, (int64_t)d.B * d.H * N, N, 0.125f, s));
      VdkGemmF32Desc v = {};
      v.A = S; v.lda = Np; v.B = qkv + 2 * D; v.ldb = 3 * D; v.b_kmajor = 1; v.C = o; v.ldc = D; v.M = N; v.N = 64; v.K = Np; v.alpha = 1.0f;
      v.batch1 = d.B; v.batch2 = d.H; v.sa1 = g.sc1; v.sa2 = g.sc2; v.sb1 = (int64_t)N * 3 * D; v.sb2 = 64; v.sc1 = (int64_t)N * D; v.sc2 = 64;
// ... 18 lines not shown
```

Baseline: 7206 images/sec.

## Fuse attention-backward D=rowsum(dO*O) into proj dgrad GEMM epilogue

```diff
diff --git a/visiondk_amd/csrc/attention.hip b/visiondk_amd/csrc/attention.hip
--- a/visiondk_amd/csrc/attention.hip
+++ b/visiondk_amd/csrc/attention.hip
@@ -358,6 +358,7 @@
 
 void vdk_attention_small_want_colsum(float*);
 int vdk_attention_small_colsum_produced();
+void vdk_attention_small_d_supplied(int);
 static int attn_long_min() {
   const char* e = getenv("VDK_ATTN_LONG_MIN");
   return e ? atoi(e) : 1 << 30;
@@ -403,13 +404,19 @@
   return vdk_check_launch("vdk_attention_fwd");
 }
 
-int vdk_attention_bwd_cs(const void* qkv, int64_t ld, const void* o, const void* dout, int64_t ldo, const float* lse, void* dqkv, int64_t lddqkv, float* dvec, int32_t B, int32_t N,
-                         int32_t H, int32_t head_dim, float scale, int32_t dtype, float* cspart, int32_t* produced, void* stream_) {
+int vdk_attention_bwd_cs_d(const void* qkv, int64_t ld, const void* o, const void* dout, int64_t ldo, const float* lse, void* dqkv, int64_t lddqkv, float* dvec, int32_t B, int32_t N,
+                           int32_t H, int32_t head_dim, float scale, int32_t dtype, float* cspart, int32_t* produced, int32_t d_supplied, void* stream_) {
   vdk_attention_small_want_colsum(cspart);
+  vdk_attention_small_d_supplied(d_supplied);
   const int rc = vdk_attention_bwd_dt(qkv, ld, o, dout, ldo, lse, dqkv, lddqkv, dvec, B, N, H, head_dim, scale, dtype, stream_);
   if (produced) *produced = rc == VDK_OK ? vdk_attention_small_colsum_produced() : 0;
   vdk_attention_small_want_colsum(nullptr);
+  vdk_attention_small_d_supplied(0);
   return rc;
+}
+int vdk_attention_bwd_cs(const void* qkv, int64_t ld, const void* o, const void* dout, int64_t ldo, const float* lse, void* dqkv, int64_t lddqkv, float* dvec, int32_t B, int32_t N,
+                         int32_t H, int32_t head_dim, float scale, int32_t dtype, float* cspart, int32_t* produced, void* stream_) {
+  return vdk_attention_bwd_cs_d(qkv, ld, o, dout, ldo, lse, dqkv, lddqkv, dvec, B, N, H, head_dim, scale, dtype, cspart, produced, 0, stream_);
 }
 int vdk_attention_bwd(const void* qkv, int64_t ld, const void* o, const void* dout, int64_t ldo, const float* lse, void* dqkv,
                       int64_t lddqkv, float* dvec, int32_t B, int32_t N, int32_t H, int32_t head_dim, float scale, void* stream_) {
diff --git a/visiondk_amd/csrc/attention_small.hip b/visiondk_amd/csrc/attention_small.hip
--- a/visiondk_amd/csrc/attention_small.hip
+++ b/visiondk_amd/csrc/attention_small.hip
@@ -91,12 +91,13 @@
 #define A5_KP 1
 #endif
 #define A5_QPITCH 144
-template <int NKT, int OF>
+template <int NKT, int OF, bool DIN>
 __global__ __launch_bounds__(512) void attn_s_bwd5_kernel(const bf16_t* __restrict__ q, const bf16_t* __restrict__ k, const bf16_t* __restrict__ v, long ld,
                                                           const bf16_t* __restrict__ o, const bf16_t* __restrict__ dout, long ldo, const float* __restrict__ lse,
                                                           bf16_t* __restrict__ dq, bf16_t* __restrict__ dk, bf16_t* __restrict__ dv, long ldd, int N, int H, float scale,
                                                           int nitems, int dbg ,
-                                                          float* __restrict__ cspart ) {
+                                                          float* __restrict__ cspart ,
+                                                          const float* __restrict__ dsup ) {
   VDK_DYN_LDS(smem);
   const int tid = threadIdx.x, lane = tid & 63, hi = lane >> 5, l31 = lane & 31;
   const int w = __builtin_amdgcn_readfirstlane(tid >> 6);
@@ -140,26 +141,35 @@
       as_dma_rows_raw(Vt, v + off + (long)(w * 32) * ld, ld, N - w * 32, 32, 0, 1, lane_);
     }
   };
-  u32x4 d_a[NPC], d_c[NPC];
-  float lse_r = 0.f;
+  constexpr int NPD = DIN ? 1 : NPC;
+  u32x4 d_a[NPD], d_c[NPD];
+  float lse_r = 0.f, dsup_r = 0.f;
   auto d_issue = [&](long offo, long lrow, int tid_) {
-#pragma unroll
-    for (int p = 0; p < NPC; ++p) {
-      const int id = tid_ + 512 * p, row = id >> 3, cp = id & 7;
-      d_a[p] = (u32x4){0u, 0u, 0u, 0u}; d_c[p] = (u32x4){0u, 0u, 0u, 0u};
-      if (row < N && !(dbg & 4)) { d_a[p] = *(const u32x4*)(dout + offo + (long)row * ldo + cp * 8); d_c[p] = *(const u32x4*)(o + offo + (long)row * ldo + cp * 8); }
+    if constexpr (DIN) {
+      dsup_r = (tid_ < N && !(dbg & 4)) ? dsup[lrow + tid_] : 0.f;
+    } else {
+#pragma unroll
+      for (int p = 0; p < NPC; ++p) {
+        const int id = tid_ + 512 * p, row = id >> 3, cp = id & 7;
+        d_a[p] = (u32x4){0u, 0u, 0u, 0u}; d_c[p] = (u32x4){0u, 0u, 0u, 0u};
+        if (row < N && !(dbg & 4)) { d_a[p] = *(const u32x4*)(dout + offo + (long)row * ldo + cp * 8); d_c[p] = *(const u32x4*)(o + offo + (long)row * ldo + cp * 8); }
+      }
     }
     lse_r = tid_ < N ? lse[lrow + tid_] : 0.f;
   };
   auto d_finish = [&]() {
-#pragma unroll
-    for (int p = 0; p < NPC; ++p) {
-      const int id = tid + 512 * p, row = id >> 3, cp = id & 7;
-      float d = 0.f;
-#pragma unroll
-      for (int e = 0; e < 4; ++e) { d = fmaf(op_lo<OF>(d_a[p][e]), op_lo<OF>(d_c[p][e]), d); d = fmaf(op_hi<OF>(d_a[p][e]), op_hi<OF>(d_c[p][e]), d); }
-      d += __shfl_xor(d, 1); d += __shfl_xor(d, 2); d += __shfl_xor(d, 4);
-      if (row < NP && cp == 0) Dv[row] = row < N ? d : 0.f;
+    if constexpr (DIN) {
+      if (tid < NP) Dv[tid] = dsup_r;
+    } else {
+#pragma unroll
+      for (int p = 0; p < NPC; ++p) {
+        const int id = tid + 512 * p, row = id >> 3, cp = id & 7;
+        float d = 0.f;
+#pragma unroll
+        for (int e = 0; e < 4; ++e) { d = fmaf(op_lo<OF>(d_a[p][e]), op_lo<OF>(d_c[p][e]), d); d = fmaf(op_hi<OF>(d_a[p][e]), op_hi<OF>(d_c[p][e]), d); }
+        d += __shfl_xor(d, 1); d += __shfl_xor(d, 2); d += __shfl_xor(d, 4);
+        if (row < NP && cp == 0) Dv[row] = row < N ? d : 0.f;
+      }
     }
     if (tid < NP) lse2[tid] = lse_r * VDK_LOG2E;
   };
@@ -418,19 +428,29 @@
 static thread_local int t_cs_produced = 0;
 void vdk_attention_small_want_colsum(float* cspart) { t_cspart = cspart; t_cs_produced = 0; }
 int vdk_attention_small_colsum_produced() { return t_cs_produced; }
-template <int NKT, int OF>
-static int launch_bwd5(const bf16_t* base, long D, long ld, const bf16_t* o, const bf16_t* dout, long ldo, const float* lse, bf16_t* dbase, long ldd, int B, int N, int H,
-                       float scale, int grid, hipStream_t s) {
+static thread_local int t_d_supplied = 0;
+void vdk_attention_small_d_supplied(int on) { t_d_supplied = on; }
+template <int NKT, int OF, bool DIN>
+static int launch_bwd5_t(const bf16_t* base, long D, long ld, const bf16_t* o, const bf16_t* dout, long ldo, const float* lse, bf16_t* dbase, long ldd, const float* dvec, int B,
+                         int N, int H, float scale, int grid, hipStream_t s) {
   const size_t lds = 3 * 8192 + 2 * (size_t)NKT * 4096 + 2 * (size_t)(32 * NKT) * A5_PITCH + (size_t)(32 * NKT) * A5_QPITCH + (size_t)NKT * 32 * 8 + 3 * 8 * 64 * 4;
   float* const cspart = t_cspart;
   if (cspart) t_cs_produced = 1;
   const char* edbg = getenv("VDK_ATTN5_DBG");
   const int dbg = edbg ? atoi(edbg) : 0;
-  if (hipFuncSetAttribute((const void*)attn_s_bwd5_kernel<NKT, OF>, hipFuncAttributeMaxDynamicSharedMemorySize, (int)lds) != hipSuccess)
+  if (hipFuncSetAttribute((const void*)attn_s_bwd5_kernel<NKT, OF, DIN>, hipFuncAttributeMaxDynamicSharedMemorySize, (int)lds) != hipSuccess)
     return vdk_fail(VDK_ELAUNCH, "vdk_attention_bwd: LDS attribute");
-  hipLaunchKernelGGL((attn_s_bwd5_kernel<NKT, OF>), dim3((unsigned)grid), dim3(512), lds, s, base, base + D, base + 2 * D, ld, o, dout, ldo, lse, dbase, dbase + D, dbase + 2 * D,
-                     ldd, N, H, scale, B * H, dbg, cspart);
+  hipLaunchKernelGGL((attn_s_bwd5_kernel<NKT, OF, DIN>), dim3((unsigned)grid), dim3(512), lds, s, base, base + D, base + 2 * D, ld, o, dout, ldo, lse, dbase, dbase + D,
+                     dbase + 2 * D, ldd, N, H, scale, B * H, dbg, cspart, dvec);
   return VDK_OK;
+}
+template <int NKT, int OF>
+static int launch_bwd5(const bf16_t* base, long D, long ld, const bf16_t* o, const bf16_t* dout, long ldo, const float* lse, bf16_t* dbase, long ldd, float* dvec, int B, int N,
+                       int H, float scale, int grid, hipStream_t s) {
+  const bool din = t_d_supplied != 0;
+  t_d_supplied = 0;
+  return din ? launch_bwd5_t<NKT, OF, true>(base, D, ld, o, dout, ldo, lse, dbase, ldd, dvec, B, N, H, scale, grid, s)
+             : launch_bwd5_t<NKT, OF, false>(base, D, ld, o, dout, ldo, lse, dbase, ldd, dvec, B, N, H, scale, grid, s);
 }
 static int grid_cap(int dflt) {
   if (const char* e = getenv("VDK_ATTN_GRID")) { const int v = atoi(e); if (v > 0) return v; }
@@ -465,11 +485,11 @@
   if (grid > cap) grid = cap;
   hipStream_t s = (hipStream_t)stream;
   switch (nkt) {
-#define B5(n) case n: return opf ? launch_bwd5<n, VDK_OPF_F16>(base, D, ld, (const bf16_t*)o, (const bf16_t*)dout, ldo, lse, (bf16_t*)dqkv, ldd, B, N, H, scale, grid, s) \
-                                 : launch_bwd5<n, 0>(base, D, ld, (const bf16_t*)o, (const bf16_t*)dout, ldo, lse, (bf16_t*)dqkv, ldd, B, N, H, scale, grid, s);
+#define B5(n) case n: return opf ? launch_bwd5<n, VDK_OPF_F16>(base, D, ld, (const bf16_t*)o, (const bf16_t*)dout, ldo, lse, (bf16_t*)dqkv, ldd, dvec, B, N, H, scale, grid, s) \
+                                 : launch_bwd5<n, 0>(base, D, ld, (const bf16_t*)o, (const bf16_t*)dout, ldo, lse, (bf16_t*)dqkv, ldd, dvec, B, N, H, scale, grid, s);
     B5(1) B5(2) B5(3) B5(4) B5(5) B5(6)
-    default: return opf ? launch_bwd5<7, VDK_OPF_F16>(base, D, ld, (const bf16_t*)o, (const bf16_t*)dout, ldo, lse, (bf16_t*)dqkv, ldd, B, N, H, scale, grid, s)
-                        : launch_bwd5<7, 0>(base, D, ld, (const bf16_t*)o, (const bf16_t*)dout, ldo, lse, (bf16_t*)dqkv, ldd, B, N, H, scale, grid, s);
+    default: return opf ? launch_bwd5<7, VDK_OPF_F16>(base, D, ld, (const bf16_t*)o, (const bf16_t*)dout, ldo, lse, (bf16_t*)dqkv, ldd, dvec, B, N, H, scale, grid, s)
+                        : launch_bwd5<7, 0>(base, D, ld, (const bf16_t*)o, (const bf16_t*)dout, ldo, lse, (bf16_t*)dqkv, ldd, dvec, B, N, H, scale, grid, s);
 #undef B5
   }
 }
diff --git a/visiondk_amd/csrc/gemm.hip b/visiondk_amd/csrc/gemm.hip
--- a/visiondk_amd/csrc/gemm.hip
+++ b/visiondk_amd/csrc/gemm.hip
@@ -602,6 +602,11 @@
 }
 static thread_local int t_tn_half = 0;
 void vdk_gemm_tn_prefer_half(int on) { t_tn_half = on; }
+struct RowDotReq { const void* o; int64_t ldo; float* out; int32_t tokens; };
+static thread_local RowDotReq t_rowdot = {nullptr, 0, nullptr, 0};
+static thread_local int t_rowdot_done = 0;
+void vdk_gemm_next_rowdot(const void* o, int64_t ldo, float* rowdot, int32_t tokens) { t_rowdot = RowDotReq{o, ldo, rowdot, tokens}; t_rowdot_done = 0; }
+int vdk_gemm_rowdot_produced() { return t_rowdot_done; }
 static bool w4h_wanted(int E, bool trans, long M, long N, long K) {
   static const int mask = getenv("VDK_GEMM_W4H") ? atoi(getenv("VDK_GEMM_W4H")) : -1;
   if (g_force_kernel == 6) return true;
@@ -662,6 +667,13 @@
 }
 
 int vdk_gemm_force_kernel(int32_t which) { g_force_kernel = which; return VDK_OK; }
+int vdk_gemm_rowdot_nt(const VdkGemmDesc* d, void* ws, size_t ws_bytes, const void* o, int64_t ldo, float* rowdot, int32_t tokens, int32_t* produced, void* stream) {
+  vdk_gemm_next_rowdot(o, ldo, rowdot, tokens);
+  const int rc = vdk_gemm_bf16_nt(d, ws, ws_bytes, stream);
+  if (produced) *produced = rc == VDK_OK ? vdk_gemm_rowdot_produced() : 0;
+  vdk_gemm_next_rowdot(nullptr, 0, nullptr, 0);
+  return rc;
+}
 int vdk_gemm_last_kernel(void) { return g_last_kernel; }
 
 int vdk_gemm_streamk_workspace_bytes(size_t* bytes) {
@@ -719,6 +731,9 @@
 
 int vdk_gemm_bf16_nt(const GemmDesc* d, void* ws, size_t ws_bytes, void* stream_) {
   hipStream_t stream = (hipStream_t)stream_;
+  const RowDotReq rd = t_rowdot;
+  t_rowdot = RowDotReq{nullptr, 0, nullptr, 0};
+  t_rowdot_done = 0;
   if (!d || !d->A || !d->B || !d->C) return vdk_fail(VDK_EINVAL, "vdk_gemm_bf16_nt: null pointer");
   if (d->M <= 0 || d->N <= 0 || d->K <= 0) return vdk_fail(VDK_EINVAL, "vdk_gemm_bf16_nt: empty problem");
   if ((d->K & 7) || (d->N & 7) || (!d->conv && (d->lda & 7)) || (d->ldb & 7) || (d->ldc & 7))
@@ -898,7 +913,19 @@
       p.ocs_part = d->c_colsum;
       E |= E_OCS;
     }
+    if (rd.out && rd.o && E == 0 && !sk && splitk == 1 && !d->a_colsum && !d->c_colsum && rd.tokens > 0 && (d->M % rd.tokens) == 0 && (d->N % 64) == 0 && !(rd.ldo & 7) &&
+        rd.ldo >= d->N) {
+      GemmParams pr = p;
+      pr.aux = (bf16_t*)rd.o; pr.ldaux = rd.ldo; pr.rowdot = rd.out; pr.rd_tokens = rd.tokens;
+      void* e0_ = prof ? (void*)g_prof_ev[g_prof_used] : nullptr; void* e1_ = prof ? (void*)g_prof_ev[g_prof_used + 1] : nullptr;
+      if (vdk_gemm_w4h_serves(pr, false) && (opf ? vdk_gemm_w4h_launch_f16(pr, false, E_ROWDOT, 1u, stream, e0_, e1_) : vdk_gemm_w4h_launch(pr, false, E_ROWDOT, 1u, stream, e0_, e1_))) {
+        g_last_kernel = 6;
+        t_rowdot_done = 1;
+        E = -1;
+      }
+    }
     switch (E) {
+      case -1: break;
       case E_OCS: LAUNCH256(false, E_OCS); break;
       case E_DGELU | E_OCS: LAUNCH256(false, E_DGELU | E_OCS); break;
       case 0: LAUNCH256CS(0); break;
diff --git a/visiondk_amd/csrc/gemm_w4.hip b/visiondk_amd/csrc/gemm_w4.hip
--- a/visiondk_amd/csrc/gemm_w4.hip
+++ b/visiondk_amd/csrc/gemm_w4.hip
@@ -248,7 +248,8 @@
   constexpr int NPS = 32 / RPP;
   constexpr int ROWB = NCT * 64;
   constexpr int EB = E & ~E_AUXD;
-  constexpr bool FAST = (E == 0 || E == E_BIAS || EB == (E_BIAS | E_GELU) || EB == E_DGELU || EB == (E_DGELU | E_OCS) || E == E_OCS);
+  constexpr bool FAST = (E == 0 || E == E_BIAS || EB == (E_BIAS | E_GELU) || EB == E_DGELU || EB == (E_DGELU | E_OCS) || E == E_OCS || E == E_ROWDOT);
+  static_assert(!(E & E_ROWDOT) || (E == E_ROWDOT && NCT == 2), "E_ROWDOT: the 256x128 kernel's plain 16-bit epilogue (a wave's 64 columns are one head)");
   const int l31 = lane & 31, hi = lane >> 5;
   const int mrow0 = m0 + wr * 128, ncol0 = n0 + wc * (NCT * 32);
   const int swz_w = NCT == 4 ? (l31 & 15) : ((l31 >> 1) & 7);
@@ -276,8 +277,15 @@
     const unsigned lane_out = nok ? (unsigned)rrow * (unsigned)p.ldc * 2u + (unsigned)ncol * 2u : W4_OOB;
     const unsigned lane_aux = nok ? (unsigned)rrow * (unsigned)p.ldaux * 2u + (unsigned)ncol * 2u : W4_OOB;
     const __amdgpu_buffer_rsrc_t rs_out = __builtin_amdgcn_make_buffer_rsrc(p.C, 0, (int)((unsigned)p.M * (unsigned)p.ldc * 2u), 0x00020000);
-    const __amdgpu_buffer_rsrc_t rs_aux = __builtin_amdgcn_make_buffer_rsrc((E & (E_GELU | E_DGELU)) ? (void*)p.aux : p.C, 0,
-                                                                            (int)((unsigned)p.M * (unsigned)((E & (E_GELU | E_DGELU)) ? p.ldaux : p.ldc) * 2u), 0x00020000);
+    constexpr bool AUXT = (E & (E_GELU | E_DGELU | E_ROWDOT)) != 0;
+    const __amdgpu_buffer_rsrc_t rs_aux = __builtin_amdgcn_make_buffer_rsrc(AUXT ? (void*)p.aux : p.C, 0, (int)((unsigned)p.M * (unsigned)(AUXT ? p.ldaux : p.ldc) * 2u), 0x00020000);
+    u32x4 auxrows[NPS];
+    auto aux_request = [&](int rt_) {
+      const unsigned srow = (unsigned)(mrow0 + rt_ * 32) * (unsigned)p.ldaux * 2u;
+#pragma unroll
+      for (int ps = 0; ps < NPS; ++ps)
+        auxrows[ps] = __builtin_amdgcn_raw_buffer_load_b128(rs_aux, lane_aux, srow + (unsigned)(ps * RPP) * (unsigned)p.ldaux * 2u, 0);
+    };
     auto rows_out = [&](const __amdgpu_buffer_rsrc_t& rs, unsigned lane_off, unsigned ldbytes, int rt, bool with_ocs) {
       W4_EPI_SYNC();
       const unsigned srow = (unsigned)(mrow0 + rt * 32) * ldbytes;
@@ -292,6 +300,28 @@
         for (int ps = 0; ps < NPS; ++ps)
 #pragma unroll
           for (int e = 0; e < 4; ++e) { ocs[2 * e] += op_lo<OF>(d[ps][e]); ocs[2 * e + 1] += op_hi<OF>(d[ps][e]); }
+      }
+      if constexpr ((E & E_ROWDOT) != 0) {
+        float dsum[NPS];
+#pragma unroll
+        for (int ps = 0; ps < NPS; ++ps) {
+          float t = 0.f;
+#pragma unroll
+          for (int e = 0; e < 4; ++e) { t = fmaf(op_lo<OF>(d[ps][e]), op_lo<OF>(auxrows[ps][e]), t); t = fmaf(op_hi<OF>(d[ps][e]), op_hi<OF>(auxrows[ps][e]), t); }
+          dsum[ps] = t;
+        }
+        if (rt < 3) aux_request(rt + 1);
+        const int H = p.N >> 6, head = ncol0 >> 6;
+#pragma unroll
+        for (int ps = 0; ps < NPS; ++ps) {
+          float t = dsum[ps];
+          t += __shfl_xor(t, 1); t += __shfl_xor(t, 2); t += __shfl_xor(t, 4);
+          const int mi = mrow0 + rt * 32 + ps * RPP + rrow;
+          if (rc == 0 && nok && mi < p.M) {
+            const int b = mi / p.rd_tokens, tk = mi - b * p.rd_tokens;
+            p.rowdot[((long)b * H + head) * p.rd_tokens + tk] = t;
+          }
+        }
       }
 #pragma unroll
       for (int ps = 0; ps < NPS; ++ps)
@@ -300,14 +330,7 @@
     };
     if constexpr (DEEP >= 0) W4_WAIT_VM(DEEP);
     if (p.dbg) ts[0] = __builtin_readcyclecounter();
-    u32x4 auxrows[NPS];
-    auto aux_request = [&](int rt_) {
-      const unsigned srow = (unsigned)(mrow0 + rt_ * 32) * (unsigned)p.ldaux * 2u;
-#pragma unroll
-      for (int ps = 0; ps < NPS; ++ps)
-        auxrows[ps] = __builtin_amdgcn_raw_buffer_load_b128(rs_aux, lane_aux, srow + (unsigned)(ps * RPP) * (unsigned)p.ldaux * 2u, 0);
-    };
-    if (E & E_DGELU) {
+    if (E & (E_DGELU | E_ROWDOT)) {
       if (auxpre) {
 #pragma unroll
         for (int ps = 0; ps < NPS; ++ps) auxrows[ps] = auxpre[ps];
@@ -1027,6 +1050,7 @@
     case E_BIAS | E_GELU | E_AUXD: W4H_LAUNCH(false, E_BIAS | E_GELU | E_AUXD);
     case E_DGELU | E_AUXD: W4H_LAUNCH(false, E_DGELU | E_AUXD);
     case E_DGELU | E_OCS | E_AUXD: W4H_LAUNCH(false, E_DGELU | E_OCS | E_AUXD);
+    case E_ROWDOT: W4H_LAUNCH(false, E_ROWDOT);
     case E_BIAS | E_RES | E_F32: W4H_LAUNCH(false, E_BIAS | E_RES | E_F32);
     case E_BIAS | E_F32: W4H_LAUNCH(false, E_BIAS | E_F32);
     case E_BIAS | E_RES | E_F32 | E_ROWGRP: W4H_LAUNCH(false, E_BIAS | E_RES | E_F32 | E_ROWGRP);
diff --git a/visiondk_amd/csrc/vdk_attn_tile.h b/visiondk_amd/csrc/vdk_attn_tile.h
--- a/visiondk_amd/csrc/vdk_attn_tile.h
+++ b/visiondk_amd/csrc/vdk_attn_tile.h
@@ -20,7 +20,7 @@
   __builtin_amdgcn_global_load_lds(VDK_GLOBAL_PTR(g), VDK_LDS_PTR(lds_dst), 16, 0, 0);
 #else
   const unsigned dst = (unsigned)__builtin_amdgcn_readfirstlane((int)(unsigned)(unsigned long long)VDK_LDS_PTR(lds_dst));
-  asm volatile("s_mov_b32 m0, %1\n\ts_nop 0\n\tglobal_load_lds_dwordx4 %0, off" ::"v"(g), "s"(dst) : "memory");
+  asm volatile("s_mov_b32 m0, %1\n\ts_nop 0\n\tglobal_load_lds_dwordx4 %0, off" ::"v"(g), "s"(dst) : "memory", "m0");
 #endif
 }
 __device__ __forceinline__ void as_dma_rows_raw(unsigned char* arr, const bf16_t* __restrict__ src, long ld, int N, int R8, int w, int nw, int lane) {
diff --git a/visiondk_amd/csrc/vdk_gemm.h b/visiondk_amd/csrc/vdk_gemm.h
--- a/visiondk_amd/csrc/vdk_gemm.h
+++ b/visiondk_amd/csrc/vdk_gemm.h
@@ -34,11 +34,14 @@
   int opf;
   const float* cscale;
   const float* rscale; int rps;
+  float* rowdot; int rd_tokens;
 };
 
 extern "C" int vdk_gemm_bf16_nt(const VdkGemmDesc* d, void* ws, size_t ws_bytes, void* stream);
 extern "C" int vdk_transpose_bf16(const void* in, int64_t ldi, int32_t R, int32_t C, void* out, int64_t ldo, int32_t Rpad, int32_t in_row_group, float* colsum_partial, void* stream);
 void vdk_gemm_tn_prefer_half(int on);
+void vdk_gemm_next_rowdot(const void* o, int64_t ldo, float* rowdot, int32_t tokens);
+int vdk_gemm_rowdot_produced();
 int vdk_transpose_16(const void* in, int64_t ldi, int32_t R, int32_t C, void* out, int64_t ldo, int32_t Rpad, int32_t in_row_group, float* colsum_partial, int opf, void* stream);
 
 bool vdk_gemm_w4_serves(const GemmParams& p, bool trans);
diff --git a/visiondk_amd/csrc/vdk_gemm_epilogue.h b/visiondk_amd/csrc/vdk_gemm_epilogue.h
--- a/visiondk_amd/csrc/vdk_gemm_epilogue.h
+++ b/visiondk_amd/csrc/vdk_gemm_epilogue.h
@@ -85,6 +85,7 @@
 #define E_Q8 1024
 #define E_AUXD 2048
 #define E_GENERIC 0x1000
+#define E_ROWDOT 0x2000
 
 template <int E, int NPS = 8 , bool SWZ = false, int OF = 0 >
 __device__ __forceinline__ void h_epilogue_half(const GemmParams& p, const float* slab, int lane, long mbase ,
diff --git a/visiondk_amd/csrc/vit_engine.hip b/visiondk_amd/csrc/vit_engine.hip
--- a/visiondk_amd/csrc/vit_engine.hip
+++ b/visiondk_amd/csrc/vit_engine.hip
@@ -19,8 +19,8 @@
                       int32_t, float, void*);
 int vdk_attention_fwd_dt(const void*, int64_t, void*, int64_t, float*, int32_t, int32_t, int32_t, int32_t, float, int32_t, void*);
 int vdk_attention_bwd_dt(const void*, int64_t, const void*, const void*, int64_t, const float*, void*, int64_t, float*, int32_t, int32_t, int32_t, int32_t, float, int32_t, void*);
-int vdk_attention_bwd_cs(const void*, int64_t, const void*, const void*, int64_t, const float*, void*, int64_t, float*, int32_t, int32_t, int32_t, int32_t, float, int32_t, float*, int32_t*,
-                         void*);
+int vdk_attention_bwd_cs_d(const void*, int64_t, const void*, const void*, int64_t, const float*, void*, int64_t, float*, int32_t, int32_t, int32_t, int32_t, float, int32_t, float*,
+                           int32_t*, int32_t, void*);
 int vdk_patchify_bf16(const float*, int32_t, int32_t, int32_t, int32_t, int32_t, void*, int32_t, void*);
 int vdk_cls_rows(float*, int64_t, int32_t, int32_t, const float*, const float*, void*);
 int vdk_cast_f32_bf16(const float*, void*, int64_t, void*);
@@ -656,12 +656,15 @@
     RC(vdk_layernorm_bwd_deferred(dsm, D, DT16, xmid, D, mean2, rstd2, params + b.n2w, dxa, D, T, D, dxm, D, dxmb, D, grads + b.n2w, grads + b.n2b, lnws0,
                                   w.lnws_bytes, s, &jobs[nj], ocs_ln ? grads + b.proj_b : nullptr, ocs_ln ? &jobs[nj + 1] : nullptr, lq ? &q8m : nullptr));
     nj += ocs_ln ? 2 : 1;
+    int32_t d_ready = 0;
     RC(ev_order(ev_p++, s, s2));
     if (f8.mode) {
       RC(gemm8(s, f8, dxmb, 12 * l + 10, 1, f8.wt8 + p.blkT[l].proj, 12 * l + 5, D, dsm, D, T, D, D, VDK_BF16, nullptr, nullptr, 0, VDK_ACT_NONE, nullptr, 0, lq ? f8.a8 : nullptr));
       RC(linear_wgrad(s2, d, w, base, dxmb, D, o, D, T, d.Tp, D, D, grads + b.proj_w, ocs_ln ? nullptr : grads + b.proj_b, 0));
     } else if (one_stream && ocs_ln) {
+      vdk_gemm_next_rowdot(o, D, dvec, d.N);
       RC(gemm(s, dxmb, D, wt + p.blkT[l].proj, D, dsm, D, T, D, D, DT16, nullptr, nullptr, 0, VDK_ACT_NONE, nullptr, 0, 1, 0, nullptr, 0));
+      d_ready = vdk_gemm_rowdot_produced();
       RC(linear_wgrad(s2, d, w, base, dxmb, D, o, D, T, d.Tp, D, D, grads + b.proj_w, nullptr, 0));
     } else if (one_stream) {
       RC(dgrad_with_bias(s, w, base, dxmb, D, wt + p.blkT[l].proj, D, dsm, D, T, D, D, VDK_ACT_NONE, nullptr, 0, grads + b.proj_b, &fz, 2, jobs, &nj));
@@ -674,7 +677,7 @@
     {
       static const bool fuse_on = !(getenv("VDK_VIT_QKVB_ATTN") && atoi(getenv("VDK_VIT_QKVB_ATTN")) == 0);
       float* csp = (fuse_on && !f8.mode && one_stream && (size_t)d.B * 3 * D * 4 <= w.csws_bytes) ? (float*)(base + w.csws + (size_t)3 * w.csws_bytes) : nullptr;
-      RC(vdk_attention_bwd_cs(qkv, 3 * D, o, dsm, D, lse, dqkv, 3 * D, dvec, d.B, d.N, d.H, 64, 0.125f, DT16, csp, &qkvb_done, s));
+      RC(vdk_attention_bwd_cs_d(qkv, 3 * D, o, dsm, D, lse, dqkv, 3 * D, dvec, d.B, d.N, d.H, 64, 0.125f, DT16, csp, &qkvb_done, d_ready, s));
       if (qkvb_done) { jobs[nj] = VdkReduceJob{csp, (long)3 * D, d.B, (long)3 * D, grads + b.qkv_b, 1.0f}; ++nj; }
     }
     RC(ev_order(ev_p++, s, s2));
```

Result: no change. 7255 images/sec, median of 6 (+0.7%).
